# penn-graphics-research/DOT

Measured on AMD Instinct MI355X. Metric: ms_per_time_step, lower is better.
Workload: dtype f64; 1 GPU; bar17K_twist; nV=17315, nT=86058, energy=SNH, subdomains=32, script=twist, parallelism=32 subdomains on 1 GPU

## Files before the change

dot_amd/csrc/dotmi_api.hip:

```cpp
#include "dotmi_handle.hpp"

extern "C" {

int dotmi_set_state(dotmi_handle *h, const double *x, const double *v, const double *x_n)
{
    if (!h || !x || !v) return DOTMI_E_INVALID;
    HIPCHECK(h, hipSetDevice(h->device));
    if (resolve_refresh(h) == DOTMI_E_DEVICE) return DOTMI_E_DEVICE;
    const size_t bytes = sizeof(double) * h->n;
    HIPCHECK(h, hipMemcpyAsync(h->x, x, bytes, hipMemcpyHostToDevice, h->st));
    HIPCHECK(h, hipMemcpyAsync(h->v, v, bytes, hipMemcpyHostToDevice, h->st));
    HIPCHECK(h, hipMemcpyAsync(h->xn, x_n ? x_n : x, bytes, hipMemcpyHostToDevice, h->st));
    HIPCHECK(h, hipStreamSynchronize(h->st));
    std::vector<double> xt(h->n);
    const double *xn_h = x_n ? x_n : x;
    for (int i = 0; i < h->nV; ++i)
        for (int d = 0; d < 3; ++d) {
            const int k = 3 * i + d;
            xt[k] = h->fixed[i] ? xn_h[k] : xn_h[k] + (v[k] * h->dt + h->gdtsq[d]);
        }
    HIPCHECK(h, hipMemcpy(h->xt, xt.data(), bytes, hipMemcpyHostToDevice));
    return 0;
}

int dotmi_get_state(dotmi_handle *h, double *x, double *v, double *x_tilde)
{
    if (!h) return DOTMI_E_INVALID;
    HIPCHECK(h, hipSetDevice(h->device));
    if (resolve_refresh(h) == DOTMI_E_DEVICE) return DOTMI_E_DEVICE;
    const size_t bytes = sizeof(double) * h->n;
    HIPCHECK(h, hipStreamSynchronize(h->st));
    if (x) HIPCHECK(h, hipMemcpy(x, h->x, bytes, hipMemcpyDeviceToHost));
    if (v) HIPCHECK(h, hipMemcpy(v, h->v, bytes, hipMemcpyDeviceToHost));
    if (x_tilde) HIPCHECK(h, hipMemcpy(x_tilde, h->xt, bytes, hipMemcpyDeviceToHost));
    return 0;
}

int dotmi_set_dirichlet(dotmi_handle *h, int32_t n, const int32_t *idx, const double *pos)
{
    if (!h || n < 0 || (n > 0 && (!idx || !pos))) return DOTMI_E_INVALID;
    if (n == 0) return 0;
    HIPCHECK(h, hipSetDevice(h->device));
    for (int i = 0; i < n; ++i)
        if (idx[i] < 0 || idx[i] >= h->nV) {
            h->err = "dirichlet index out of range";
            return DOTMI_E_INVALID;
        }
    if ((size_t)n > h->dcap) {
        if (int rc = dalloc(h, &h->didx, (size_t)n)) return rc;
        if (int rc = dalloc(h, &h->dpos, (size_t)3 * n)) return rc;
        h->dcap = n;
    }
    if (h->didxHost.size() != (size_t)n || memcmp(h->didxHost.data(), idx, sizeof(int32_t) * n) != 0) {
        HIPCHECK(h, hipStreamSynchronize(h->st));
        h->didxHost.assign(idx, idx + n);
        if (h->dposPinned) hipHostFree(h->dposPinned);
        h->dposPinned = nullptr;
        HIPCHECK(h, hipHostMalloc((void **)&h->dposPinned, sizeof(double) * 3 * n));
        HIPCHECK(h, hipMemcpyAsync(h->didx, h->didxHost.data(), sizeof(int) * n, hipMemcpyHostToDevice, h->st));
    }
    if (!h->evDir) HIPCHECK(h, hipEventCreateWithFlags(&h->evDir, hipEventDisableTiming));
    else HIPCHECK(h, hipEventSynchronize(h->evDir));
    memcpy(h->dposPinned, pos, sizeof(double) * 3 * n);
    HIPCHECK(h, hipMemcpyAsync(h->dpos, h->dposPinned, sizeof(double) * 3 * n, hipMemcpyHostToDevice, h->st));
    HIPCHECK(h, hipEventRecord(h->evDir, h->st));
    launch_scatter_rows(n, h->didx, h->dpos, h->x, h->st);
    return 0;
}

int dotmi_refix(dotmi_handle *h, const uint8_t *fixed)
{
    if (!h || !fixed) return DOTMI_E_INVALID;
    HIPCHECK(h, hipSetDevice(h->device));
    if (resolve_refresh(h) == DOTMI_E_DEVICE) return DOTMI_E_DEVICE;
    h->fixed.assign(fixed, fixed + h->nV);
    HIPCHECK(h, hipMemcpy(h->M.fixed, fixed, h->nV, hipMemcpyHostToDevice));
    if (h->VP.orec) {
        refix_vpatch_records(h->vpRecGid, fixed, h->vpRec);
        HIPCHECK(h, hipMemcpy(const_cast<VpOwnRec *>(h->VP.orec), h->vpRec.data(), sizeof(VpOwnRec) * h->vpRec.size(), hipMemcpyHostToDevice));
    }
    if (h->pd) return pd_factor(h);
    return refactor(h, h->x, nullptr, nullptr);
}

int dotmi_operand_records(const dotmi_handle *h) { return h && h->vpFits ? (h->VP.orec ? 1 : 0) : -1; }

int dotmi_loop_forms(const dotmi_handle *h)
{
    if (!h) return DOTMI_E_INVALID;
    const long long nv = h->owner ? h->nHeld : h->nV;
    int forms = 0;
    if (h->devLoop) {
        if (gather_is_wide(3 * nv, h->tune.wideForms)) forms |= FORM_WIDE_GATHER;
        if (h->earlyBs && merge_early_is_wide(3 * nv, h->tune.wideForms)) forms |= FORM_WIDE_MERGE;
        if (h->earlyBs && (h->owner || h->tune.fuseDir) && spmv_zp_is_wide(nv, h->tune.wideForms)) forms |= FORM_WIDE_SPMV;
    }
    if (h->P.splitMerge) forms |= FORM_SPLIT_MERGE;
    if (h->P.tl.on && h->P.tl.nPanels > 0) forms |= twolevel_backward_code(h->P.tl.maxCols) << FORM_TWOLEVEL_CW_SHIFT;
    return forms;
}

double dotmi_target_gres(const dotmi_handle *h) { return h ? h->targetGRes : 0.0; }

int dotmi_last_iter_log(const dotmi_handle *h, int32_t cap, double *alpha, double *E, double *g2)
{
    if (!h) return DOTMI_E_INVALID;
    if (h->logPending > 0) {
        dotmi_handle *hm = const_cast<dotmi_handle *>(h);
        const int nlog = h->logPending;
        hm->logPending = 0;
        hm->log_alpha.resize(nlog);
        hm->log_E.resize(nlog);
        hm->log_g2.resize(nlog);
        if (hipSetDevice(h->device) != hipSuccess ||
            hipMemcpy(hm->log_alpha.data(), h->dlog, sizeof(double) * nlog, hipMemcpyDeviceToHost) != hipSuccess ||
            hipMemcpy(hm->log_E.data(), h->dlog + h->logCap, sizeof(double) * nlog, hipMemcpyDeviceToHost) != hipSuccess ||
            hipMemcpy(hm->log_g2.data(), h->dlog + 2 * (size_t)h->logCap, sizeof(double) * nlog, hipMemcpyDeviceToHost) !=
                hipSuccess)
            return DOTMI_E_DEVICE;
    }
    const int n = std::min<int>(cap, (int)h->log_alpha.size());
    for (int i = 0; i < n; ++i) {
        if (alpha) alpha[i] = h->log_alpha[i];
        if (E) E[i] = h->log_E[i];
        if (g2) g2[i] = h->log_g2[i];
    }
    return (int)h->log_alpha.size();
}

static int upload_tmp(dotmi_handle *h, const double *x, double *dst)
{
    HIPCHECK(h, hipMemcpyAsync(dst, x, sizeof(double) * h->n, hipMemcpyHostToDevice, h->st));
    return 0;
}

int dotmi_eval_energy(dotmi_handle *h, const double *x, double *E)
{
    if (!h || !x || !E) return DOTMI_E_INVALID;
    HIPCHECK(h, hipSetDevice(h->device));
    if (resolve_refresh(h) == DOTMI_E_DEVICE) return DOTMI_E_DEVICE;
    if (int rc = upload_tmp(h, x, h->x_trial)) return rc;
    const int nb = eval_all_elements(h, h->x_trial, 0);
    HIPCHECK(h, hipMemcpyAsync(h->h_partE, h->partE, sizeof(double) * 2 * nb, hipMemcpyDeviceToHost, h->st));
    HIPCHECK(h, hipStreamSynchronize(h->st));
    double se = 0, si = 0;
    for (int b = 0; b < nb; ++b) {
        se += h->h_partE[2 * b];
        si += h->h_partE[2 * b + 1];
    }
    *E = h->dtSq * se + si;
    return 0;
}

int dotmi_eval_gradient(dotmi_handle *h, const double *x, double *g)
{
    if (!h || !x || !g) return DOTMI_E_INVALID;
    HIPCHECK(h, hipSetDevice(h->device));
    if (resolve_refresh(h) == DOTMI_E_DEVICE) return DOTMI_E_DEVICE;
    if (int rc = upload_tmp(h, x, h->x_trial)) return rc;
    eval_all_elements(h, h->x_trial, 1);
    HIPCHECK(h, hipMemcpyAsync(g, h->g_trial, sizeof(double) * h->n, hipMemcpyDeviceToHost, h->st));
    HIPCHECK(h, hipStreamSynchronize(h->st));
    return 0;
}

int dotmi_eval_elem_hessians(dotmi_handle *h, const double *x, double *H)
{
    if (!h || !x || !H) return DOTMI_E_INVALID;
    HIPCHECK(h, hipSetDevice(h->device));
    if (resolve_refresh(h) == DOTMI_E_DEVICE) return DOTMI_E_DEVICE;
    if (int rc = upload_tmp(h, x, h->x_trial)) return rc;
    double *tmp = nullptr;
    HIPCHECK(h, hipMalloc((void **)&tmp, sizeof(double) * 144 * (size_t)h->nT));
    launch_elem_hessians(h->M, h->mat, h->dtSq, h->x_trial, tmp, h->st);
    hipError_t e = hipMemcpyAsync(H, tmp, sizeof(double) * 144 * (size_t)h->nT, hipMemcpyDeviceToHost, h->st);
    hipStreamSynchronize(h->st);
    hipFree(tmp);
    HIPCHECK(h, e);
    return 0;
}

int dotmi_refactor(dotmi_handle *h, const double *x)
{
    if (!h) return DOTMI_E_INVALID;
    if (h->pd) {
        h->err = "dotmi_refactor: an LBFGS-PD handle has no Hessian block solve";
        return DOTMI_E_INVALID;
    }
    HIPCHECK(h, hipSetDevice(h->device));
    if (resolve_refresh(h) == DOTMI_E_DEVICE) return DOTMI_E_DEVICE;
    const double *xd = h->x;
    if (x) {
        if (int rc = upload_tmp(h, x, h->x_trial)) return rc;
        xd = h->x_trial;
    }
    return refactor(h, xd, nullptr, nullptr);
}

int dotmi_apply_precond(dotmi_handle *h, const double *r, double *p)
{
    if (!h || !r || !p) return DOTMI_E_INVALID;
    HIPCHECK(h, hipSetDevice(h->device));
    if (int rc = enter_with_factors(h)) return rc;
    if (int rc = dot_coarse_refresh(h)) return rc;
    if (int rc = upload_tmp(h, r, h->q)) return rc;
    if (h->pd) {
        if (int rc = pd_apply(h, h->q, h->z, NO_HISTORY)) return rc;
    } else if (h->hi) {
        if (int rc = ic_apply(h, h->q, h->z, NO_HISTORY)) return rc;
    } else if (int rc = apply_precond(h, h->q, h->z, NO_HISTORY)) return rc;
    HIPCHECK(h, hipMemcpyAsync(p, h->z, sizeof(double) * h->n, hipMemcpyDeviceToHost, h->st));
    HIPCHECK(h, hipStreamSynchronize(h->st));
    return 0;
}

int dotmi_probe_direction(dotmi_handle *h, const double *x, int32_t m, const double *S, const double *Y, double *g_out,
                          double *q_out, double *z_out, double *p_out, double *alpha0, double *E_trial)
{
    if (!h || !x || m < 0 || m > h->hist || (m > 0 && (!S || !Y))) return DOTMI_E_INVALID;
    if (h->pd) {
        h->err = "dotmi_probe_direction: an LBFGS-PD handle has no Hessian block solve";
        return DOTMI_E_INVALID;
    }
    if (h->hi) {
        h->err = "dotmi_probe_direction: an LBFGS-HI handle has no Hessian block solve";
        return DOTMI_E_INVALID;
    }
    if (h->dist) {
        h->err = "dotmi_probe_direction: single-GPU handles only";
        return DOTMI_E_INVALID;
    }
    HIPCHECK(h, hipSetDevice(h->device));
    if (int rc = enter_with_factors(h)) return rc;
    if (int rc = dot_coarse_refresh(h)) return rc;
    const int n = h->n;
    const size_t bytes = sizeof(double) * n;
    HIPCHECK(h, hipMemcpyAsync(h->tmpn, x, bytes, hipMemcpyHostToDevice, h->st));
    for (int i = 0; i < m; ++i) {
// ... 169 lines not shown
    for (int i = 0; i < reps; ++i) one();
    HIPCHECK(h, hipEventRecord(h->ev1, h->st));
    HIPCHECK(h, hipEventSynchronize(h->ev1));
    float ms = 0;
    HIPCHECK(h, hipEventElapsedTime(&ms, h->ev0, h->ev1));
    if (ms_per_launch) *ms_per_launch = ms / reps;
    if (bytes_per_launch) *bytes_per_launch = h->precond_bytes;
    return 0;
}

int dotmi_bench_kernel(dotmi_handle *h, int32_t kind, int32_t reps, double *ms_per_launch, int64_t *bytes_per_launch)
{
    if (!h || reps < 1) return DOTMI_E_INVALID;
    if (h->pd) {
        h->err = "dotmi_bench_kernel: an LBFGS-PD handle has no Hessian block solve";
        return DOTMI_E_INVALID;
    }
    if (h->hi) {
        switch (kind) {
        case DOTMI_BENCH_BACKSOLVE:
        case DOTMI_BENCH_MERGE:
        case DOTMI_BENCH_BUILD_QPAD:
        case DOTMI_BENCH_SPMV_ZP:
        case DOTMI_BENCH_MERGE_EARLY:
        case DOTMI_BENCH_ELEM_STEP:
        case DOTMI_BENCH_GATHER_EARLY:
        case DOTMI_BENCH_DIRSTEP:
        case DOTMI_BENCH_ELEM_VERTEX:
            h->err = "dotmi_bench_kernel: an LBFGS-HI handle has no Hessian block solve";
            return DOTMI_E_INVALID;
        default:
            break;
        }
    }
    HIPCHECK(h, hipSetDevice(h->device));
    if (int rc = enter_with_factors(h)) return rc;
    const int n = h->n, nV = h->nV;
    const int64_t nTo = h->PT.nElem, nVo = h->v1 - h->v0, m = h->m > 0 ? h->m : h->hist;
    LbfgsArgs L = lbfgs_args(h);
    L.m = (int)std::min<int64_t>(m, h->hist);
    for (int i = 0; i < L.m; ++i) {
        L.s[i] = h->S[i];
        L.y[i] = h->Y[i];
        if (L.ys[i] == 0.0) L.ys[i] = 1.0;
    }
    int64_t bytes = 0;
    bool live = false;
    std::function<void()> run;
    StepElemPass e = step_elem_pass(h, h->x, 1, false);
    const StepArgs sa{h->p, h->partS, h->alpha_dev, h->alphaMin};
    GatherArgs a = gather_args(h);
    a.x = h->x;
    a.g_old = h->g;
    a.p = h->p;
    a.alpha_dev = h->alpha_dev;
    a.g_new = h->g_trial;
    a.s_new = h->S[h->hist];
    a.y_new = h->Y[h->hist];
    a.make_pair = 1;
    double xi[HIST_MAX] = {0, 0, 0, 0, 0, 0};
    switch (kind) {
    case DOTMI_BENCH_ELEM_ENERGY_GRAD:
        bytes = 112 * nTo + 56 * nVo;
        run = [&] { launch_elem_pass(e.M, h->PT, h->mat, h->dtSq, e.a, h->st); };
        break;
    case DOTMI_BENCH_ELEM_ENERGY:
        bytes = 112 * nTo + 56 * nVo;
        e.a.grad = 0;
        run = [&] { launch_elem_pass(e.M, h->PT, h->mat, h->dtSq, e.a, h->st); };
        break;
    case DOTMI_BENCH_VERTEX_GATHER:
        bytes = 80 * (int64_t)nV + (int64_t)(4 + 2 * L.m) * 8 * n;
        run = [&] { launch_vertex_gather(h->M, h->PT, a, L, h->partR, h->st); };
        break;
    case DOTMI_BENCH_SPMV_DOTS:
        bytes = 72 * (int64_t)h->M.nnzb + 2 * 8 * (int64_t)n;
        run = [&] { launch_spmv_dots(h->M, h->Hval, h->p, h->g, nullptr, h->v0, h->v1, h->partS, h->st); };
        break;
    case DOTMI_BENCH_BACKSOLVE:
        bytes = h->precond_bytes;
        run = [&] { launch_gemv(h->P, h->q, h->st); };
        break;
    case DOTMI_BENCH_MERGE:
        bytes = 8 * (int64_t)n * (2 + L.m) + 8 * (int64_t)h->mergeEntries;
        run = [&] {
            if (!h->P.mt_ptr) launch_reduce_partial(h->P, h->st);
            launch_merge(h->M, h->P, L, {.z = h->z, .partials = h->partC, .dots = true, .divide = true}, h->st);
        };
        break;
    case DOTMI_BENCH_BUILD_QPAD:
        bytes = 8 * (int64_t)n * (1 + L.m) + 8 * (int64_t)h->P.nParts * h->P.nmax;
        run = [&] { launch_build_qpad(h->P, h->g, L, xi, h->st); };
        break;
    case DOTMI_BENCH_BUILD_P:
        bytes = 8 * (int64_t)n * (2 + L.m);
        run = [&] { launch_build_p(n, h->z, L, h->partC, xi, h->p, h->st); };
        break;
    case DOTMI_BENCH_STEP_FORWARD:
        bytes = 8 * (int64_t)n * 3;
        run = [&] { launch_step_forward(n, step_forward_args(h, h->partS), h->st); };
        break;
    case DOTMI_BENCH_ELEM_HESSIAN:
        if (h->world > 1) return DOTMI_E_INVALID;
        bytes = (int64_t)(112 + 1152) * h->nHessElems;
        run = [&] {
            if (h->shardHess) launch_elem_hessians(h->M, h->mat, h->dtSq, h->x, h->He, h->st, h->hessElems, h->nHessElems);
            else launch_elem_hessians(h->M, h->mat, h->dtSq, h->x, h->He, h->st);
        };
        break;
    case DOTMI_BENCH_ASSEMBLE:
        if (h->world > 1) return DOTMI_E_INVALID;
        bytes = (int64_t)1152 * h->nHessElems + 72 * (int64_t)(h->shardHess ? h->nHessBlk : h->M.nnzb);
        run = [&] {
            if (h->shardHess) launch_assemble(h->M, h->He, h->Hval, h->st, h->hessBlk, h->nHessBlk, h->hessBlkPtr, h->hessBlkEnt);
            else launch_assemble(h->M, h->He, h->Hval, h->st);
        };
        break;
    case DOTMI_BENCH_SPMV_ZP:
        bytes = 72 * (int64_t)h->M.nnzb + 8 * (int64_t)n * (4 + 2 * L.m);
        live = true;
        run = [&] { launch_spmv_zp(h->M, spmv_zp_args(h, false), h->st, h->ctl); };
        break;
    case DOTMI_BENCH_MERGE_EARLY:
        bytes = 8 * (int64_t)h->mergeEntries + 8 * (int64_t)n * (4 + 2 * L.m);
        live = true;
        run = [&] {
            if (!h->P.mt_ptr) launch_reduce_partial(h->P, h->st, h->ctl);
            launch_merge_early(h->M, h->P, {.z = h->z, .partials = h->partC, .partialsT = h->dist ? nullptr : h->partCT, .wide = h->tune.wideForms}, h->st, h->ctl);
        };
        break;
    case DOTMI_BENCH_ELEM_STEP: {
        bytes = 112 * nTo + 56 * nVo + 48 * (int64_t)nV;
        live = true;
        e.a.x = h->x_trial;
        if (h->tune.fuseStep) e.a.step = &sa;
        run = [&] { launch_elem_pass(e.M, h->PT, h->mat, h->dtSq, e.a, h->st, h->ctl); };
        break;
    }
    case DOTMI_BENCH_GATHER_EARLY: {
        long long held = 0;
        for (int v = 0; v < nV; ++v) held += h->dup[v];
        bytes = 80 * (int64_t)nV + (int64_t)(6 + 2 * L.m) * 8 * n + 24 * held;
        live = true;
        a = early_gather_args(h);
        run = [&] { launch_vertex_gather(h->M, h->PT, a, L, h->partR, h->st, h->ctl); };
        break;
    }
    case DOTMI_BENCH_ELEM_VERTEX: {
        if (!h->vpFits) return DOTMI_E_INVALID;
        long long held = 0;
        for (int v = 0; v < nV; ++v) held += h->dup[v];
        bytes = 112 * nTo + 56 * nVo + 48 * (int64_t)nV + 80 * (int64_t)nV + (int64_t)(6 + 2 * L.m) * 8 * n + 24 * held;
        live = true;
        run = [&] {
            launch_elem_vertex(h->VP, h->mat, elem_vertex_args(h), h->st, h->ctl);
        };
        break;
    }
    case DOTMI_BENCH_DIRSTEP: {
        if (h->dist || !h->specFits) return DOTMI_E_INVALID;
        bytes = 72 * (int64_t)h->M.nnzb + 8 * (int64_t)n * (4 + 2 * L.m) + 112 * nTo + 56 * nVo + 24 * (int64_t)nV;
        live = true;
        e.a.x = h->x_trial;
        e.a.step = &sa;
        run = [&] { launch_dirstep(e.M, h->PTspec, h->mat, h->dtSq, spmv_zp_args(h, false), e.a, h->st, h->ctl); };
        break;
    }
    default:
        return DOTMI_E_INVALID;
    }
    DevLoop saved;
    if (live) {
        if (!h->earlyBs || h->prevSlots < 0 || !h->P.vp_ptr) {
            h->err = "the in-loop kernel forms need a handle that has run a step of the device loop's early order";
            return DOTMI_E_INVALID;
        }
        HIPCHECK(h, hipMemcpy(&saved, h->ctl, sizeof(DevLoop), hipMemcpyDeviceToHost));
        DevLoop live_ctl = saved;
        live_ctl.status = 0;
        live_ctl.phase = 0;
        HIPCHECK(h, hipMemcpy(h->ctl, &live_ctl, sizeof(DevLoop), hipMemcpyHostToDevice));
    }
    run();
    HIPCHECK(h, hipEventRecord(h->ev0, h->st));
    for (int i = 0; i < reps; ++i) run();
    HIPCHECK(h, hipEventRecord(h->ev1, h->st));
    HIPCHECK(h, hipEventSynchronize(h->ev1));
    HIPCHECK(h, hipGetLastError());
    if (live) HIPCHECK(h, hipMemcpy(h->ctl, &saved, sizeof(DevLoop), hipMemcpyHostToDevice));
    float ms = 0;
    HIPCHECK(h, hipEventElapsedTime(&ms, h->ev0, h->ev1));
    if (kind == DOTMI_BENCH_ELEM_HESSIAN || kind == DOTMI_BENCH_ASSEMBLE) {
        if (int rc = refactor(h, h->x, nullptr, nullptr)) return rc;
    }
    if (ms_per_launch) *ms_per_launch = ms / reps;
    if (bytes_per_launch) *bytes_per_launch = bytes;
    return 0;
}

int dotmi_bench_energy(dotmi_handle *h, int32_t reps, double *ms_per_launch, int64_t *bytes_per_launch)
{
    if (!h || reps < 1) return DOTMI_E_INVALID;
    HIPCHECK(h, hipSetDevice(h->device));
    if (resolve_refresh(h) == DOTMI_E_DEVICE) return DOTMI_E_DEVICE;
    const StepElemPass e = step_elem_pass(h, h->x, 0, false);
    launch_elem_pass(e.M, h->PT, h->mat, h->dtSq, e.a, h->st);
    HIPCHECK(h, hipEventRecord(h->ev0, h->st));
    for (int i = 0; i < reps; ++i) launch_elem_pass(e.M, h->PT, h->mat, h->dtSq, e.a, h->st);
    HIPCHECK(h, hipEventRecord(h->ev1, h->st));
    HIPCHECK(h, hipEventSynchronize(h->ev1));
    float ms = 0;
    HIPCHECK(h, hipEventElapsedTime(&ms, h->ev0, h->ev1));
    if (ms_per_launch) *ms_per_launch = ms / reps;
    if (bytes_per_launch) *bytes_per_launch = (int64_t)112 * h->nOwnElem + (int64_t)56 * (h->v1 - h->v0);
    return 0;
}

int dotmi_comm_unique_id(void *out128)
{
    ncclUniqueId id;
    if (ncclGetUniqueId(&id) != ncclSuccess) return DOTMI_E_DEVICE;
    static_assert(sizeof(ncclUniqueId) == 128, "ncclUniqueId size");
    memcpy(out128, &id, 128);
    return 0;
}

int32_t dotmi_factor_kind(const dotmi_handle *h)
{
    if (!h) return DOTMI_E_INVALID;
    return h->tileFlow ? 2 : h->tileSplit ? 3 : 1;
}

int32_t dotmi_factor_groups(const dotmi_handle *h)
{
    if (!h) return DOTMI_E_INVALID;
    return h->tgroupLevel.size() > 2 ? (int32_t)h->tgroupLevel.size() - 1 : 1;
}

int32_t dotmi_backsolve_form(const dotmi_handle *h)
{
    if (!h) return DOTMI_E_INVALID;
    return h->twoLevel ? 1 : 0;
}

int32_t dotmi_comm_ranks(const dotmi_handle *h)
{
    if (!h) return DOTMI_E_INVALID;
    if (h->comm) {
        int n = 0;
        if (ncclCommCount(h->comm, &n) != ncclSuccess) return DOTMI_E_DEVICE;
        return n;
    }
    return h->arCb ? -h->world : 1;
}

}
```

dot_amd/csrc/dotmi_create.hip:

```cpp
#include "dotmi_handle.hpp"
#include "block_plan.hpp"

namespace dotmi {
std::string g_create_error;
}

namespace dotmi {

void host_features(dotmi_handle *h)
{
    const int nV = h->nV, nT = h->nT;
    h->A.assign((size_t)9 * nT, 0.0);
    h->vol.assign(nT, 0.0);
    h->mass.assign(nV, 0.0);
    for (int e = 0; e < nT; ++e) {
        const int *t = &h->T[4 * e];
        const double *p0 = &h->Xrest[3 * t[0]], *p1 = &h->Xrest[3 * t[1]], *p2 = &h->Xrest[3 * t[2]],
                     *p3 = &h->Xrest[3 * t[3]];
        Mat3 X0;
        for (int i = 0; i < 3; ++i) {
            X0.m[i][0] = p1[i] - p0[i];
            X0.m[i][1] = p2[i] - p0[i];
            X0.m[i][2] = p3[i] - p0[i];
        }
        const double d = det3(X0), id = 1.0 / d;
        const double(*m)[3] = X0.m;
        double *R = &h->A[(size_t)9 * e];
        R[0] = (m[1][1] * m[2][2] - m[1][2] * m[2][1]) * id;
        R[1] = (m[0][2] * m[2][1] - m[0][1] * m[2][2]) * id;
        R[2] = (m[0][1] * m[1][2] - m[0][2] * m[1][1]) * id;
        R[3] = (m[1][2] * m[2][0] - m[1][0] * m[2][2]) * id;
        R[4] = (m[0][0] * m[2][2] - m[0][2] * m[2][0]) * id;
        R[5] = (m[0][2] * m[1][0] - m[0][0] * m[1][2]) * id;
        R[6] = (m[1][0] * m[2][1] - m[1][1] * m[2][0]) * id;
        R[7] = (m[0][1] * m[2][0] - m[0][0] * m[2][1]) * id;
        R[8] = (m[0][0] * m[1][1] - m[0][1] * m[1][0]) * id;
        h->vol[e] = d / 3.0 / 2.0;
        double a[3], b[3], c[3];
        for (int i = 0; i < 3; ++i) {
            a[i] = p0[i] - p3[i];
            b[i] = p1[i] - p3[i];
            c[i] = p2[i] - p3[i];
        }
        const double vv = std::fabs(a[0] * (b[1] * c[2] - b[2] * c[1]) + a[1] * (b[2] * c[0] - b[0] * c[2]) +
                                    a[2] * (b[0] * c[1] - b[1] * c[0])) / 6.0;
        for (int k = 0; k < 4; ++k) h->mass[t[k]] += vv / 4.0;
    }
    for (int v = 0; v < nV; ++v) h->mass[v] *= h->density;
}

double host_target_gres(const dotmi_handle *h)
{
    Mat3 Aw;
    double Bw[3][4];
    const double S1[3] = {1, 1, 1};
#define TG_BLOCKS(MATV) spectral_blocks<MATV>(S1, h->mu[0], h->lam[0], 1.0, false, Aw, Bw)
    DM_DISPATCH_MAT(h->mat, TG_BLOCKS)
#undef TG_BLOCKS
    double sqH = 0;
    for (int i = 0; i < 3; ++i)
        for (int j = 0; j < 3; ++j) sqH += Aw.m[i][j] * Aw.m[i][j];
    for (int c = 0; c < 3; ++c)
        for (int k = 0; k < 4; ++k) sqH += Bw[c][k] * Bw[c][k];
    std::vector<double> ls(h->nV, 0.0);
    for (int e = 0; e < h->nT; ++e) {
        const int *t = &h->T[4 * e];
        for (int i = 0; i < 4; ++i) {
            const double *a = &h->Xrest[3 * t[(i + 1) % 4]], *b = &h->Xrest[3 * t[(i + 2) % 4]],
                         *c = &h->Xrest[3 * t[(i + 3) % 4]];
            const double u[3] = {b[0] - a[0], b[1] - a[1], b[2] - a[2]};
            const double w[3] = {c[0] - a[0], c[1] - a[1], c[2] - a[2]};
            const double cx = u[1] * w[2] - u[2] * w[1], cy = u[2] * w[0] - u[0] * w[2],
                         cz = u[0] * w[1] - u[1] * w[0];
            ls[t[i]] += 0.5 * std::sqrt(cx * cx + cy * cy + cz * cz);
        }
    }
    double sql = 0;
    for (int v = 0; v < h->nV; ++v) sql += ls[v] * ls[v];
    const double cn = h->relTol * h->relTol * sqH * sql * (double)(h->nV - 1) / (double)h->nV;
    return cn * h->dtSq * h->dtSq;
}

int upload_vpatches(dotmi_handle *h, const HostVPatches &H, DevVPatches &D, dotmi_handle::SlotMap &SM)
{
    D.nPatches = H.nPatches;
    D.PE = H.PE;
    D.PV = H.PV;
    D.PO = H.PO;
    D.RUN = H.RUN;
    const size_t ns = (size_t)H.nPatches * H.PE;
    std::vector<ushort4> tl(ns), ep(ns);
    std::vector<double> A(9 * ns, 0.0), mu(ns, 1.0), lam(ns, 1.0), vol(ns, 0.0), volE(ns, 0.0);
    D.nSlotsUsed = 0;
    for (size_t s = 0; s < ns; ++s) {
        tl[s] = make_ushort4(H.tl[4 * s], H.tl[4 * s + 1], H.tl[4 * s + 2], H.tl[4 * s + 3]);
        ep[s] = make_ushort4(H.epos[4 * s], H.epos[4 * s + 1], H.epos[4 * s + 2], H.epos[4 * s + 3]);
        const int e = H.elem[s];
        if (e < 0) continue;
        D.nSlotsUsed++;
        for (int k = 0; k < 9; ++k) A[(size_t)k * ns + s] = h->A[(size_t)9 * e + k];
        mu[s] = h->mu[e];
        lam[s] = h->lam[e];
        vol[s] = h->vol[e];
        volE[s] = H.eown[s] ? h->vol[e] : 0.0;
    }
    if (int rc = upload(h, &D.tl, tl)) return rc;
    if (int rc = upload(h, &D.epos, ep)) return rc;
    if (int rc = upload(h, &D.A, A)) return rc;
    bool uniform = !h->mu.empty();
    for (size_t e = 1; e < h->mu.size() && uniform; ++e) uniform = h->mu[e] == h->mu[0] && h->lam[e] == h->lam[0];
    D.mu = D.lam = nullptr;
    if (uniform) {
        D.mu0 = h->mu[0];
        D.lam0 = h->lam[0];
    } else {
        if (int rc = upload(h, &D.mu, mu)) return rc;
        if (int rc = upload(h, &D.lam, lam)) return rc;
    }
    if (int rc = upload(h, &SM.elem, H.elem)) return rc;
    SM.nSlots = ns;
    SM.mu = D.mu;
    SM.lam = D.lam;
    if (int rc = upload(h, &D.vol, vol)) return rc;
    if (int rc = upload(h, &D.volE, volE)) return rc;
    if (int rc = upload(h, &D.pv_gid, H.pv_gid)) return rc;
    if (int rc = upload(h, &D.pv_cnt, H.pv_cnt)) return rc;
    if (int rc = upload(h, &D.po_cnt, H.po_cnt)) return rc;
    if (int rc = upload(h, &D.c_ptr, H.c_ptr)) return rc;
    return 0;
}

int upload_patches(dotmi_handle *h, const HostPatches &H, DevPatches &D, dotmi_handle::SlotMap &SM)
{
    D.nPatches = H.nPatches;
    D.PE = H.PE;
    D.PV = H.PV;
    D.nSlots = H.nSlots;
    const size_t ns = (size_t)H.nPatches * H.PE;
    std::vector<ushort4> tl(ns);
    std::vector<double> A(9 * ns, 0.0), mu(ns, 1.0), lam(ns, 1.0), vol(ns, 0.0);
    D.nElem = 0;
    for (size_t s = 0; s < ns; ++s) {
        tl[s] = make_ushort4(H.tl[4 * s], H.tl[4 * s + 1], H.tl[4 * s + 2], H.tl[4 * s + 3]);
        const int e = H.elem[s];
        if (e < 0) continue;
        D.nElem++;
        for (int k = 0; k < 9; ++k) A[(size_t)k * ns + s] = h->A[(size_t)9 * e + k];
        mu[s] = h->mu[e];
        lam[s] = h->lam[e];
        vol[s] = h->vol[e];
    }
    if (int rc = upload(h, &D.tl, tl)) return rc;
    if (int rc = upload(h, &D.A, A)) return rc;
    bool uniform = !h->mu.empty();
    for (size_t e = 1; e < h->mu.size() && uniform; ++e) uniform = h->mu[e] == h->mu[0] && h->lam[e] == h->lam[0];
    D.mu = D.lam = nullptr;
    if (uniform) {
        D.mu0 = h->mu[0];
        D.lam0 = h->lam[0];
    } else {
        if (int rc = upload(h, &D.mu, mu)) return rc;
        if (int rc = upload(h, &D.lam, lam)) return rc;
    }
    if (int rc = upload(h, &SM.elem, H.elem)) return rc;
    SM.nSlots = ns;
    SM.mu = D.mu;
    SM.lam = D.lam;
    if (int rc = upload(h, &D.vol, vol)) return rc;
    if (int rc = upload(h, &D.pv_gid, H.pv_gid)) return rc;
    if (int rc = upload(h, &D.pv_slot, H.pv_slot)) return rc;
    if (int rc = upload(h, &D.pv_cnt, H.pv_cnt)) return rc;
    if (int rc = upload(h, &D.c_ptr, H.c_ptr)) return rc;
    {
        std::vector<ushort4> ep(ns);
        for (size_t s2 = 0; s2 < ns; ++s2) ep[s2] = make_ushort4(H.epos[4 * s2], H.epos[4 * s2 + 1], H.epos[4 * s2 + 2], H.epos[4 * s2 + 3]);
        if (int rc = upload(h, &D.epos, ep)) return rc;
    }
    {
        std::vector<int2> rng(H.pp_rng.size() / 2);
        for (size_t v = 0; v < rng.size(); ++v) rng[v] = make_int2(H.pp_rng[2 * v], H.pp_rng[2 * v + 1]);
        if (int rc = upload(h, &D.pp_rng, rng)) return rc;
    }
    if (int rc = dalloc(h, &D.gpart, (size_t)3 * std::max(H.nSlots, 1))) return rc;
    HIPCHECK(h, hipMemset(D.gpart, 0, sizeof(double) * 3 * (size_t)std::max(H.nSlots, 1)));
    return 0;
}

static int build_element_side(dotmi_handle *h, const std::vector<int> &adj_ptr, const std::vector<int> &blk_ptr,
                              const std::vector<int> &blk_ent)
{
    const int nV = h->nV, nT = h->nT;
    if (h->shardElems) {
        std::vector<int> el;
        for (int e = 0; e < nT; ++e)
            if (h->epart[e] >= h->p0 && h->epart[e] < h->p1) el.push_back(e);
        h->nOwnElem = (int)el.size();
        if (int rc = upload(h, &h->elist, el)) return rc;
        h->v0 = (int)((long long)nV * h->rank / h->world);
        h->v1 = (int)((long long)nV * (h->rank + 1) / h->world);
    } else {
        h->elist = nullptr;
        h->nOwnElem = nT;
        h->v0 = 0;
        h->v1 = nV;
    }
    h->shardHess = h->shardElems && (h->owner || (h->tune.shardHess >= 0 ? h->tune.shardHess != 0 : true));
    h->nHessElems = nT;
    if (h->shardHess) {
        std::vector<uint8_t> needV(nV, 0);
        for (int pI = h->p0; pI < h->p1; ++pI)
            for (int v : h->partVerts[pI]) needV[v] = 1;
        if (!h->owner)
            for (int v = h->v0; v < h->v1; ++v) needV[v] = 1;
        std::vector<int> el, e2c(nT, -1);
        for (int e = 0; e < nT; ++e)
            if (needV[h->T[4 * e]] || needV[h->T[4 * e + 1]] || needV[h->T[4 * e + 2]] || needV[h->T[4 * e + 3]]) {
                e2c[e] = (int)el.size();
                el.push_back(e);
            }
        std::vector<int> bl, bptr(1, 0), bent, optr(1, 0), oent;
        for (int v = 0; v < nV; ++v) {
            if (!needV[v]) continue;
            for (int k = adj_ptr[v]; k < adj_ptr[v + 1]; ++k) {
                bl.push_back(k);
                for (int i = blk_ptr[k]; i < blk_ptr[k + 1]; ++i) {
                    const int e = blk_ent[i] >> 4;
                    bent.push_back((e2c[e] << 4) | (blk_ent[i] & 15));
                    if (h->owner && h->epart[e] >= h->p0 && h->epart[e] < h->p1) oent.push_back(bent.back());
                }
                bptr.push_back((int)bent.size());
                optr.push_back((int)oent.size());
            }
        }
        if (h->owner) {
            if (oent.empty()) oent.push_back(-1);
            if (int rc = upload(h, &h->ownBlkPtr, optr)) return rc;
            if (int rc = upload(h, &h->ownBlkEnt, oent)) return rc;
        }
        h->nHessElems = (int)el.size();
        h->nHessBlk = (int)bl.size();
        if (int rc = upload(h, &h->hessElems, el)) return rc;
        if (int rc = upload(h, &h->hessBlk, bl)) return rc;
        if (int rc = upload(h, &h->hessBlkPtr, bptr)) return rc;
        if (int rc = upload(h, &h->hessBlkEnt, bent)) return rc;
    }
    {
        int PE = h->tune.patchElems > 0 ? (h->tune.patchElems <= 256 ? 256 : 512) : 256;
        std::vector<int> all(nT);
        for (int e = 0; e < nT; ++e) all[e] = e;
        if (int rc = upload_patches(h, build_patches(nV, h->T.data(), h->Xrest.data(), all, PE), h->PTall, h->smAll)) return rc;
        if (h->shardElems) {
            std::vector<int> own;
            for (int e = 0; e < nT; ++e)
                if (h->epart[e] >= h->p0 && h->epart[e] < h->p1) own.push_back(e);
            if (int rc = upload_patches(h, build_patches(nV, h->T.data(), h->Xrest.data(), own, PE), h->PT, h->smOwn)) return rc;
        } else {
            h->PT = h->PTall;
        }
        h->specFits = false;
        if (!h->dist && h->world == 1 && h->tune.specStep != 0) {
            const int nbv = (nV + 255) / 256, room = 512 - NB_RED - nbv;
            if (std::max(h->PT.nPatches, nbv) <= room) {
                h->PTspec = h->PT;
                h->specFits = true;
            } else if (h->tune.patchElems == 0 && PE == 256) {
                const HostPatches H2 = build_patches(nV, h->T.data(), h->Xrest.data(), all, 512);
                if (std::max(H2.nPatches, nbv) <= room) {
                    if (int rc = upload_patches(h, H2, h->PTspec, h->smSpec)) return rc;
                    h->specFits = true;
                }
            }
        }
    }
    if (h->owner) {
        std::vector<int> holders(nV, 0), last(nV, -1), ownerR(nV, -1);
        for (int r = 0; r < h->world; ++r)
            for (int pI = h->firstPart[r]; pI < h->firstPart[r + 1]; ++pI)
// ... 472 lines not shown
{
    h->nV = mesh->nV;
    h->nT = mesh->nT;
    h->n = 3 * mesh->nV;
    h->mat = prm->energy;
    h->hist = prm->history;
    h->iterCap = prm->iterCap > 0 ? prm->iterCap : 10000;
    h->dt = prm->dt;
    h->dtSq = prm->dt * prm->dt;
    for (int d = 0; d < 3; ++d) {
        h->grav[d] = prm->gravity[d];
        h->gdtsq[d] = h->dtSq * prm->gravity[d];
    }
    h->relTol = prm->relTol;
    h->alphaMin = prm->alphaMin;
    h->device = prm->device;
    h->rank = prm->rank;
    h->world = prm->world;
    h->flags = prm->flags;
    h->tune = Tuning::from_env();
#ifdef DOTMI_TEST_HOOKS
    h->testIterDelta = Tuning::geti("DOTMI_TEST_ITER_DELTA", 0);
    h->testFailRefresh = Tuning::geti("DOTMI_TEST_FAIL_REFRESH", 0);
#endif
    h->density = mesh->density;
    h->nPartsAll = mesh->nParts;
    h->T.assign(mesh->T, mesh->T + 4 * (size_t)h->nT);
    h->pd = (h->flags & DOTMI_FLAG_LBFGS_PD) != 0;
    h->hi = (h->flags & DOTMI_FLAG_LBFGS_HI) != 0;
    h->newtonPcg = (h->flags & DOTMI_FLAG_NEWTON_PCG) != 0;
    if (h->newtonPcg) {
        const int bad = DOTMI_FLAG_FORCE_DIST | DOTMI_FLAG_OWNER_EXCHANGE | DOTMI_FLAG_GSDD | DOTMI_FLAG_NEWTON | DOTMI_FLAG_LBFGS_PD |
                        DOTMI_FLAG_LBFGS_HI | DOTMI_FLAG_ASYNC_REFRESH;
        if (prm->world > 1 || (h->flags & bad) || mesh->vpart) {
            h->err = "DOTMI_FLAG_NEWTON_PCG: single GPU, host loop, not with DOTMI_FLAG_FORCE_DIST / OWNER_EXCHANGE / GSDD / NEWTON / "
                     "LBFGS_PD / LBFGS_HI / ASYNC_REFRESH or a vertex partition";
            return DOTMI_E_INVALID;
        }
    }
    if (h->flags & DOTMI_FLAG_NEWTON_PCG_DIST) {
        const char *why = (h->flags & DOTMI_FLAG_OWNER_EXCHANGE) ? "not with DOTMI_FLAG_OWNER_EXCHANGE (the vectors of the recurrences are replicated)"
                          : (h->flags & DOTMI_FLAG_GSDD)         ? "not with DOTMI_FLAG_GSDD (a GSDD handle solves one subdomain at a time)"
                          : (h->flags & DOTMI_FLAG_NEWTON)       ? "not with DOTMI_FLAG_NEWTON (a Newton handle factorises H as one subdomain)"
                          : (h->flags & DOTMI_FLAG_LBFGS_PD)     ? "not with DOTMI_FLAG_LBFGS_PD (no Hessian block solve)"
                          : (h->flags & DOTMI_FLAG_LBFGS_HI)     ? "not with DOTMI_FLAG_LBFGS_HI (no Hessian block solve)"
                          : (h->flags & DOTMI_FLAG_ASYNC_REFRESH)
                              ? "not with DOTMI_FLAG_ASYNC_REFRESH (a Newton iteration factorises at its own iterate)"
                          : (h->flags & DOTMI_FLAG_DOT_COARSE) ? "not with DOTMI_FLAG_DOT_COARSE (the sharded PCG has no coarse space)"
                          : mesh->vpart                        ? "not with a vertex partition (vpart): it is single-GPU only"
                                                               : nullptr;
        if (why) {
            h->err = std::string("DOTMI_FLAG_NEWTON_PCG_DIST: ") + why;
            return DOTMI_E_INVALID;
        }
        h->newtonPcg = true;
    }
    if (h->hi) {
        const int bad = DOTMI_FLAG_FORCE_DIST | DOTMI_FLAG_OWNER_EXCHANGE | DOTMI_FLAG_GSDD | DOTMI_FLAG_NEWTON | DOTMI_FLAG_LBFGS_PD |
                        DOTMI_FLAG_ASYNC_REFRESH;
        if (prm->world > 1 || (h->flags & bad) || mesh->vpart) {
            h->err = "DOTMI_FLAG_LBFGS_HI: single GPU, host loop, not with DOTMI_FLAG_FORCE_DIST / OWNER_EXCHANGE / GSDD / NEWTON / "
                     "LBFGS_PD / ASYNC_REFRESH or a vertex partition";
            return DOTMI_E_INVALID;
        }
        h->nPartsAll = 1;
        h->epart.assign(h->nT, 0);
    } else if (h->pd) {
        const int bad = DOTMI_FLAG_FORCE_DIST | DOTMI_FLAG_OWNER_EXCHANGE | DOTMI_FLAG_GSDD | DOTMI_FLAG_NEWTON | DOTMI_FLAG_ASYNC_REFRESH;
        if (prm->world > 1 || (h->flags & bad) || mesh->vpart) {
            h->err = "DOTMI_FLAG_LBFGS_PD: single GPU, host loop, not with DOTMI_FLAG_FORCE_DIST / OWNER_EXCHANGE / GSDD / NEWTON / "
                     "ASYNC_REFRESH or a vertex partition";
            return DOTMI_E_INVALID;
        }
        h->nPartsAll = 1;
        h->epart.assign(h->nT, 0);
    } else if (mesh->vpart) {
        if (prm->world > 1 || (prm->flags & DOTMI_FLAG_FORCE_DIST)) {
            h->err = "a vertex partition (vpart) is single-GPU only";
            return DOTMI_E_INVALID;
        }
        for (int v = 0; v < mesh->nV; ++v)
            if (mesh->vpart[v] < 0 || mesh->vpart[v] >= mesh->nParts) {
                h->err = "vpart out of range";
                return DOTMI_E_INVALID;
            }
        h->vpart.assign(mesh->vpart, mesh->vpart + h->nV);
        h->epart.assign(h->nT, 0);
    } else if (mesh->epart) {
        h->epart.assign(mesh->epart, mesh->epart + h->nT);
    } else {
        h->epart.resize(h->nT);
        partition_elements(mesh->nV, mesh->nT, mesh->T, mesh->X_rest, mesh->nParts, h->epart.data());
    }
    if (h->flags & DOTMI_FLAG_DOT_COARSE) {
        const char *why = (h->flags & DOTMI_FLAG_OWNER_EXCHANGE)
                              ? "not with DOTMI_FLAG_OWNER_EXCHANGE (its merge in front of the exchange forms z before the coarse solution y exists)"
                          : (h->flags & DOTMI_FLAG_GSDD)       ? "not with DOTMI_FLAG_GSDD (a GSDD handle solves one subdomain at a time)"
                          : (h->flags & DOTMI_FLAG_NEWTON_PCG) ? "not with DOTMI_FLAG_NEWTON_PCG (its coarse term is dotmi_set_pcg_coarse)"
                          : (h->flags & DOTMI_FLAG_NEWTON)     ? "not with DOTMI_FLAG_NEWTON (a Newton handle factorises H as one subdomain)"
                          : (h->flags & DOTMI_FLAG_LBFGS_PD)   ? "not with DOTMI_FLAG_LBFGS_PD (no Hessian block solve)"
                          : (h->flags & DOTMI_FLAG_LBFGS_HI)   ? "not with DOTMI_FLAG_LBFGS_HI (no Hessian block solve)"
                          : (h->flags & DOTMI_FLAG_ASYNC_REFRESH)
                              ? "not with DOTMI_FLAG_ASYNC_REFRESH (the build is judged with the refresh)"
                          : mesh->vpart ? "not with a vertex partition (vpart): the coarse plan works on an element partition"
                                        : nullptr;
        if (why) {
            h->err = std::string("DOTMI_FLAG_DOT_COARSE: ") + why;
            return DOTMI_E_INVALID;
        }
        if (h->nPartsAll > COARSE_MAX_PARTS) {
            h->err = "DOTMI_FLAG_DOT_COARSE: at most " + std::to_string(COARSE_MAX_PARTS) + " subdomains (the coarse matrix is applied "
                     "through a dense inverse factor); " + std::to_string(h->nPartsAll) + " were asked for";
            return DOTMI_E_INVALID;
        }
        h->coarse.dotMode = 1;
    }
    h->fixed.assign(mesh->fixed, mesh->fixed + h->nV);
    h->Xrest.assign(mesh->X_rest, mesh->X_rest + h->n);
    h->mu.assign(mesh->mu, mesh->mu + h->nT);
    h->lam.assign(mesh->lambda, mesh->lambda + h->nT);
    return 0;
}

static int choose_loop_form(dotmi_handle *h)
{
    h->gsdd = (h->flags & DOTMI_FLAG_GSDD) != 0;
    h->newton = (h->flags & (DOTMI_FLAG_NEWTON | DOTMI_FLAG_NEWTON_PCG | DOTMI_FLAG_NEWTON_PCG_DIST)) != 0;
    if (h->newton && ((h->dist && !(h->flags & DOTMI_FLAG_NEWTON_PCG_DIST)) || h->gsdd)) {
        h->err = "DOTMI_FLAG_NEWTON: single GPU, not together with DOTMI_FLAG_GSDD";
        return DOTMI_E_INVALID;
    }
    if (h->gsdd && h->dist) {
        h->err = "DOTMI_FLAG_GSDD: single GPU only";
        return DOTMI_E_INVALID;
    }
    h->devLoop = !h->gsdd && !h->newton && !h->pd && !h->hi && !(h->flags & (DOTMI_FLAG_HOST_LOOP | DOTMI_FLAG_TIME_PHASES));
    h->earlyBs = h->devLoop && h->tune.earlyBs != 0 &&
                 (h->P.mt_ptr != nullptr || h->P.splitMerge);
    if (h->owner && !(h->earlyBs && h->tune.fuseDir)) {
        h->err = "DOTMI_FLAG_OWNER_EXCHANGE needs the device loop's early order with the fused direction kernel";
        return DOTMI_E_INVALID;
    }
    if (h->earlyBs && h->tune.fuseStep && (!h->shardElems || h->owner)) h->PT.wgCap = h->PTspec.wgCap = 512;
    h->vpFits = false;
    const bool closedForm = h->mat == DOTMI_ENERGY_SNH || h->mat == DOTMI_ENERGY_SNH_LOG;
    if (h->earlyBs && !h->dist && h->world == 1 && h->tune.fuseStep && h->tune.fuseDir && h->tune.vertexPatches != 0 &&
        (closedForm || h->tune.vertexPatches > 0) &&
        h->P.ntiles - h->P.ntilesWide + h->P.nquad > 0 && !(h->flags & (DOTMI_FLAG_GSDD | DOTMI_FLAG_NEWTON | DOTMI_FLAG_NEWTON_PCG | DOTMI_FLAG_NEWTON_PCG_DIST | DOTMI_FLAG_HOST_LOOP))) {
        const HostVPatches HV = build_vpatches(h->nV, h->nT, h->T.data(), h->Xrest.data(), 512, 85);
        const bool rec = h->tune.operandRecords != 0 && HV.nPatches > 0 &&
                         elem_vertex_dyn_lds(HV.PV, HV.RUN, HV.PO, true) + ELEM_VERTEX_STATIC_LDS <= 64 * 1024;
        const size_t shm = HV.nPatches > 0 ? elem_vertex_dyn_lds(HV.PV, HV.RUN, HV.PO, rec) + ELEM_VERTEX_STATIC_LDS : 0;
        if (HV.nPatches > 0 && HV.nPatches <= 512 && HV.nPatches <= ELEM_NB_MAX && shm <= 64 * 1024 && HV.PO + 1 <= 256) {
            if (int rc = upload_vpatches(h, HV, h->VP, h->smVP)) return rc;
            if (rec) {
                std::vector<int> vpp((size_t)h->nV + 1), vpo;
                HIPCHECK(h, hipMemcpy(vpp.data(), h->P.vp_ptr, sizeof(int) * vpp.size(), hipMemcpyDeviceToHost));
                vpo.resize((size_t)std::max(vpp[h->nV], 1));
                HIPCHECK(h, hipMemcpy(vpo.data(), h->P.vp_off, sizeof(int) * (size_t)vpp[h->nV], hipMemcpyDeviceToHost));
                h->vpRec = build_vpatch_records(HV, h->mass.data(), h->fixed.data(), vpp.data(), vpo.data());
                h->vpRecGid = vpatch_own_gid(HV);
                VpOwnRec *d = nullptr;
                if (int rc = upload(h, &d, h->vpRec)) return rc;
                h->VP.orec = d;
            }
            h->vpFits = true;
            if (h->tune.fuseLog)
                fprintf(stderr, "dotmi: vertex patches: %d patches, %.2f x the elements, up to %d owned / %d touched vertices, runs %d, %zu B LDS, operand records %s\n",
                        HV.nPatches, (double)h->VP.nSlotsUsed / std::max(1, h->nT), HV.PO, HV.PV, HV.RUN, shm, rec ? "on" : "off");
        }
    }
    return 0;
}

static int alloc_loop_state(dotmi_handle *h)
{
    if (h->dist) {
        const size_t nz = (size_t)h->n + dot_coarse_tail(h);
        if (int rc = dalloc(h, &h->zstage, nz)) return rc;
        HIPCHECK(h, hipMemsetAsync(h->zstage, 0, sizeof(double) * nz, h->st));
    }
    if (h->vpFits && h->VP.orec) {
        const size_t nrec = (size_t)2 * (HIST_MAX + 1) * h->n;
        if (int rc = dalloc(h, &h->hrec, nrec)) return rc;
        HIPCHECK(h, hipMemsetAsync(h->hrec, 0, sizeof(double) * nrec, h->st));
    }
    if (h->earlyBs) {
        if (int rc = dalloc(h, &h->u_old, (size_t)h->n)) return rc;
        for (int sl = 0; sl <= h->hist; ++sl) {
            if (int rc = dalloc(h, &h->MY[sl], (size_t)h->n)) return rc;
            if (int rc = dalloc(h, &h->HS[sl], (size_t)h->n)) return rc;
        }
    }
    h->logCap = std::min(h->iterCap, 10001) + 1;
    h->kindCap = 4096;
    HIPCHECK(h, hipHostMalloc((void **)&h->h_ctl, sizeof(DevLoop)));
    HIPCHECK(h, hipHostMalloc((void **)&h->h_flags, sizeof(int) * 4));
    HIPCHECK(h, hipMalloc((void **)&h->ctl, sizeof(DevLoop)));
    h->allocs.push_back(h->ctl);
    if (int rc = dalloc(h, &h->dlog, (size_t)3 * h->logCap)) return rc;
    HIPCHECK(h, hipMalloc((void **)&h->dkind, sizeof(int) * h->kindCap));
    h->allocs.push_back(h->dkind);
    return 0;
}

static int create_impl(dotmi_handle *h, const dotmi_mesh *mesh, const dotmi_params *prm, const double *x_init)
{
    int ndev = 0;
    if (hipGetDeviceCount(&ndev) != hipSuccess || ndev <= 0) {
        h->err = "no HIP device available: libdotmi has no CPU fallback";
        return DOTMI_E_NOGPU;
    }
    if (!mesh || !prm || !x_init || mesh->nV <= 0 || mesh->nT <= 0 || !mesh->X_rest || !mesh->T || !mesh->mu ||
        !mesh->lambda || !mesh->fixed || mesh->nParts < 1 || prm->dt <= 0 ||
        prm->history < 1 || prm->history > HIST_MAX || prm->world < 1 || prm->rank < 0 ||
        prm->rank >= prm->world || (prm->world > 1 && !prm->comm_id && !prm->allreduce) ||
        (prm->energy != DOTMI_ENERGY_FCR && prm->energy != DOTMI_ENERGY_SNH && prm->energy != DOTMI_ENERGY_SNH_LOG)) {
        h->err = "invalid argument";
        return DOTMI_E_INVALID;
    }
    for (int e = 0; e < mesh->nT; ++e) {
        if (mesh->epart && !mesh->vpart && (mesh->epart[e] < 0 || mesh->epart[e] >= mesh->nParts)) {
            h->err = "epart out of range";
            return DOTMI_E_INVALID;
        }
        for (int k = 0; k < 4; ++k)
            if (mesh->T[4 * e + k] < 0 || mesh->T[4 * e + k] >= mesh->nV) {
                h->err = "tet index out of range";
                return DOTMI_E_INVALID;
            }
    }
    if (int rc = take_arguments(h, mesh, prm)) return rc;

    HIPCHECK(h, hipSetDevice(h->device));
    HIPCHECK(h, hipStreamCreate(&h->st));
    HIPCHECK(h, hipEventCreate(&h->ev0));
    HIPCHECK(h, hipEventCreate(&h->ev1));
    HIPCHECK(h, hipEventCreate(&h->ev2));
    HIPCHECK(h, hipEventCreate(&h->evA));
    h->timePhases = (h->flags & DOTMI_FLAG_TIME_PHASES) != 0;
    if (h->timePhases)
        for (auto &e : h->evP) HIPCHECK(h, hipEventCreate(&e));
    h->dist = h->world > 1 || (h->flags & DOTMI_FLAG_FORCE_DIST);
    h->shardElems = h->dist && (h->tune.shardElems >= 0 ? h->tune.shardElems != 0 : h->nT >= 400000);
    h->owner = h->dist && (h->flags & DOTMI_FLAG_OWNER_EXCHANGE);
    if (h->owner) {
        if (h->flags & (DOTMI_FLAG_HOST_LOOP | DOTMI_FLAG_TIME_PHASES | DOTMI_FLAG_GSDD | DOTMI_FLAG_NEWTON)) {
            h->err = "DOTMI_FLAG_OWNER_EXCHANGE: device loop only";
            return DOTMI_E_INVALID;
        }
        h->shardElems = true;
    }
    h->arCb = prm->allreduce;
    h->arCtx = prm->allreduce_ctx;
    if (h->dist && !h->arCb) {
        ncclUniqueId id;
        if (h->world > 1) memcpy(&id, prm->comm_id, 128);
        else NCCLCHECK(h, ncclGetUniqueId(&id));
        NCCLCHECK(h, ncclCommInitRank(&h->comm, h->world, id, h->rank));
    }
    {
        void *cd = nullptr;
        HIPCHECK(h, hipMalloc(&cd, sizeof(double) * (RED_K + 8)));
        h->allocs.push_back(cd);
        h->ctrlDev = (double *)cd;
    }

    h->timeStride = h->tune.timeStride;
    if (h->flags & DOTMI_FLAG_TIME_BACKSOLVE) {
        h->evPre.resize(2 * 512);
        for (auto &e : h->evPre) HIPCHECK(h, hipEventCreate(&e));
        if (h->dist) {
            h->evAr.resize(2 * 512);
            for (auto &e : h->evAr) HIPCHECK(h, hipEventCreate(&e));
        }
    }
    host_features(h);
    h->targetGRes = host_target_gres(h);
    if (int rc = build_device_mesh(h)) return rc;
    if (!h->pd && !h->hi)
        if (int rc = pcg_build_scaling(h)) return rc;
    const int n = h->n;
    double **vecs[] = {&h->x, &h->x_trial, &h->xn, &h->v, &h->xt, &h->g, &h->g_trial, &h->p, &h->q, &h->z,
                       &h->Hp, &h->tmpn};
    const size_t nvec = (size_t)n + 8 + dot_coarse_tail(h);
    for (double **pp : vecs) {
        if (int rc = dalloc(h, pp, nvec)) return rc;
        HIPCHECK(h, hipMemsetAsync(*pp, 0, sizeof(double) * nvec, h->st));
    }
    for (int s = 0; s <= h->hist; ++s) {
        if (int rc = dalloc(h, &h->S[s], (size_t)n)) return rc;
        if (int rc = dalloc(h, &h->Y[s], (size_t)n)) return rc;
    }
    if (int rc = dalloc(h, &h->He, (size_t)144 * std::max(h->nHessElems, 1))) return rc;
    if (int rc = dalloc(h, &h->Hval, hval_size(h->M.nnzb))) return rc;
    if (h->owner) {
        if (int rc = dalloc(h, &h->HvalOwn, hval_size(h->M.nnzb))) return rc;
        HIPCHECK(h, hipMemsetAsync(h->HvalOwn, 0, sizeof(double) * hval_size(h->M.nnzb), h->st));
    }
    if (int rc = dalloc(h, &h->partE, (size_t)4 * ELEM_NB_MAX)) return rc;
    double **parts[] = {&h->partR, &h->partC, &h->partS, &h->partG, &h->partGR, &h->partGC, &h->partCT, &h->partST};
    for (double **pp : parts) {
        const size_t rows = pp == &h->partR ? 512 : NB_RED;
        if (int rc = dalloc(h, pp, rows * RED_K)) return rc;
        HIPCHECK(h, hipMemsetAsync(*pp, 0, sizeof(double) * rows * RED_K, h->st));
    }
    if (int rc = dalloc(h, &h->alpha_dev, 8)) return rc;
    if (int rc = dalloc(h, &h->gstage, (size_t)n + 2)) return rc;
    HIPCHECK(h, hipMemsetAsync(h->gstage, 0, sizeof(double) * ((size_t)n + 2), h->st));
    HIPCHECK(h, hipHostMalloc((void **)&h->h_partE, sizeof(double) * 2 * ELEM_NB_MAX));
    HIPCHECK(h, hipHostMalloc((void **)&h->h_partR, sizeof(double) * NB_RED * RED_K));
    HIPCHECK(h, hipHostMalloc((void **)&h->h_alpha, sizeof(double) * 8));
    if (int rc = choose_loop_form(h)) return rc;
    if (int rc = alloc_loop_state(h)) return rc;

    HIPCHECK(h, hipMemcpyAsync(h->x, x_init, sizeof(double) * n, hipMemcpyHostToDevice, h->st));
    HIPCHECK(h, hipMemcpyAsync(h->xn, h->x, sizeof(double) * n, hipMemcpyDeviceToDevice, h->st));
    launch_be_update(h->nV, h->M.fixed, h->x, h->xn, h->v, h->xt, h->dt, h->gdtsq, h->st);
    HIPCHECK(h, hipStreamSynchronize(h->st));
    if (h->pd) return pd_factor(h);
    return refactor(h, h->x, nullptr, nullptr);
}

int dotmi_create(const dotmi_mesh *mesh, const dotmi_params *prm, const double *x_init, dotmi_handle **out)
{
    if (!out) return DOTMI_E_INVALID;
    *out = nullptr;
    dotmi_handle *h = new dotmi_handle();
    int rc = create_impl(h, mesh, prm, x_init);
    if (rc != 0) {
        g_create_error = h->err;
        dotmi_destroy(h);
        return rc;
    }
    *out = h;
    return 0;
}

// ... 2 lines not shown
```

dot_amd/csrc/dotmi_devloop.hip:

```cpp
#include "dotmi_handle.hpp"

namespace dotmi {

struct Slot {
    int nb = 0;
    const double *spart = nullptr;
    const double *ctlE = nullptr;
};

static int slot_direction(dotmi_handle *h, Slot &s)
{
    if (h->specNow) {
        const StepArgs sa{h->p, h->partS, h->alpha_dev, h->alphaMin};
        StepElemPass e = step_elem_pass(h, h->x_trial, 1);
        e.a.step = &sa;
        s.nb = launch_dirstep(e.M, h->PTspec, h->mat, h->dtSq, spmv_zp_args(h), e.a, h->st, h->ctl);
    } else if (h->owner || h->tune.fuseDir) {
        launch_spmv_zp(h->M, spmv_zp_args(h), h->st, h->ctl);
    } else {
        launch_build_p(h->n, h->z, NO_HISTORY, h->partC, nullptr, h->p, h->st, h->ctl);
        launch_spmv_dots(h->M, h->Hval, h->p, h->g, nullptr, h->v0, h->v1, h->partS, h->st, h->ctl);
    }
    return reduce_step_dots(h, &s.spart);
}
// ... 27 lines not shown
    const GatherArgs a = early_gather_args(h);
    s.ctlE = h->partE;
    if (h->vpNow) {
    } else if (!h->shardElems) {
        launch_vertex_gather(h->M, h->stepPT(), a, NO_HISTORY, h->partR, h->st, h->ctl);
    } else if (h->owner) {
        GatherArgs ag = a;
        ag.ownMask = h->ownMask;
        ag.vlist = h->heldList;
        ag.nlist = h->nHeld;
        ag.kind = h->vkind;
        ag.pre = 1;
        ag.gshare = h->gstage;
        launch_vertex_gather(h->M, h->PT, ag, NO_HISTORY, h->partR, h->st, h->ctl);
        if (int rc = exchange_gradient_packed(h, n, s.nb, h->partR, RED_K)) return rc;
        ag.vlist = h->sharedList;
        ag.nlist = h->nShared;
        ag.pre = 0;
        if (h->nShared > 0) launch_pair_stats(n, ag, NO_HISTORY, nullptr, h->st, h->gstage, h->ctl);
        s.ctlE = h->gstage + n;
        s.nb = 1;
    } else {
        if (int rc = gradient_over_ranks(h, s.nb, a)) return rc;
        s.ctlE = h->gstage + n;
        s.nb = 1;
    }
    return 0;
}

static void slot_coarse(dotmi_handle *h)
{
    if (!dot_coarse(h)) return;
    if (h->dist) dot_coarse_restrict(h, h->zstage + h->n, h->ctl, 1);
    else dot_coarse_restrict_solve(h, h->ctl, 1);
}

static void slot_backsolve(dotmi_handle *h, const Slot &s)
{
    const double *ctlR = h->owner ? h->partGR : h->partR;
    const Bracket br = backsolve_bracket(h);
    h->slotTimed.push_back(br.at);
    CtlLaunch ca{{h->ctl, s.ctlE, ctlR, h->alpha_dev, h->h_flags, s.nb, h->pairNow ? 2 : 0}, h->ctlForm};
    launch_gemv(h->P, nullptr, h->st, h->ctl, br.ev0, br.ev1, &ca, (int)h->slotTimed.size() );
}

static int slot_merge(dotmi_handle *h)
{
    if (!h->dist) {
        launch_merge_early(h->M, h->P, {.z = h->z, .partials = h->partC, .partialsT = h->partCT, .co = dot_coarse(h), .wide = h->tune.wideForms}, h->st, h->ctl);
    } else if (!h->owner) {
        return merge_over_ranks(h, NO_HISTORY, h->zstage, RANKSUM_EARLY, h->ctl, h->held());
    } else {
        launch_merge_early(h->M, h->P, {.z = h->z, .partials = h->partC, .ownMask = h->ownMask, .vl = h->held(), .kind = h->vkind, .pre = 1,
                                        .zshare = h->zstage, .wide = h->tune.wideForms}, h->st, h->ctl);
        if (int rc = exchange_solve_packed(h)) return rc;
        if (h->nShared > 0)
            launch_merge_early(h->M, h->P, {.z = h->z, .zsum = h->zstage, .ownMask = h->ownMask, .vl = h->shared(), .wide = h->tune.wideForms}, h->st, h->ctl);
    }
    return 0;
}

static int enqueue_loop_slot_early(dotmi_handle *h)
{
    Slot s;
    if (int rc = slot_direction(h, s)) return rc;
    slot_trial(h, s);
    if (int rc = slot_gradient(h, s)) return rc;
    slot_coarse(h);
    slot_backsolve(h, s);
    return slot_merge(h);
}

static int enqueue_loop_slot(dotmi_handle *h)
{
    if (h->earlyNow) return enqueue_loop_slot_early(h);
    const int n = h->n;
    const CoarseMerge *bal = dot_coarse_balanced(h);
    const double *r1 = nullptr;
    if (bal) {
        launch_build_q(n, h->g, NO_HISTORY, nullptr, h->q, h->st, h->ctl);
        r1 = dot_coarse_deflate(h, h->q, h->ctl);
    } else {
        launch_build_qpad(h->P, h->g, NO_HISTORY, nullptr, h->st, h->ctl);
    }
    const CoarseMerge *co = dot_coarse(h);
    if (co && h->dist) dot_coarse_restrict(h, h->z + n, h->ctl, 0);
    else if (co) dot_coarse_restrict_solve(h, h->ctl, 0);
    const Bracket br = backsolve_bracket(h);
    h->slotTimed.push_back(br.at);
    launch_gemv(h->P, r1, h->st, h->ctl, br.ev0, br.ev1);
    if (bal) {
        launch_merge(h->M, h->P, NO_HISTORY, {.z = h->z}, h->st, h->ctl);
        dot_coarse_balance(h, h->z, NO_HISTORY, h->ctl);
    } else if (!h->dist) {
        launch_merge(h->M, h->P, NO_HISTORY, {.z = h->z, .partials = h->partC, .dots = true, .divide = true, .co = co}, h->st, h->ctl);
    } else {
        if (int rc = merge_over_ranks(h, NO_HISTORY, h->z, RANKSUM_ZFINISH, h->ctl)) return rc;
    }
    launch_build_p(n, h->z, NO_HISTORY, h->partC, nullptr, h->p, h->st, h->ctl);
    launch_spmv_dots(h->M, h->Hval, h->p, h->g, nullptr, h->v0, h->v1, h->partS, h->st, h->ctl);
    const double *spart = nullptr;
    if (int rc = reduce_step_dots(h, &spart)) return rc;
    launch_step_forward(n, step_forward_args(h, spart), h->st, h->ctl);
    const StepElemPass e = step_elem_pass(h, h->x_trial, 1);
    const int nb = launch_elem_pass(e.M, h->PT, h->mat, h->dtSq, e.a, h->st, h->ctl);
    GatherArgs a = gather_args(h);
    a.p = h->p;
    a.alpha_dev = h->alpha_dev;
    a.make_pair = 1;
    if (!h->shardElems) {
        launch_vertex_gather(h->M, h->PT, a, NO_HISTORY, h->partR, h->st, h->ctl);
        launch_loop_control(h->ctl, h->partE, nb, h->partR, h->alpha_dev, h->h_flags, h->st);
        return 0;
    }
    if (int rc = gradient_over_ranks(h, nb, a)) return rc;
    launch_loop_control(h->ctl, h->gstage + n, 1, h->partR, h->alpha_dev, h->h_flags, h->st);
    return 0;
}

static void choose_step_forms(dotmi_handle *h)
{
    h->earlyNow = h->earlyBs && !dot_coarse_balanced(h);
    h->pairNow = h->earlyNow && !h->dist && h->tune.fuseStep && h->tune.fuseDir && h->tune.earlyHold &&
                 (h->tune.pairTrials > 0 || (h->tune.pairTrials < 0 && h->prevIters > 0 && 4 * h->prevHalv >= h->prevIters));
    h->specNow = h->earlyNow && !h->dist && !h->pairNow && h->tune.fuseStep && h->tune.fuseDir &&
                 h->specFits && h->coarse.dotMode == 0 &&
                 (h->tune.specStep > 0 || (h->tune.specStep < 0 && h->prevFirst > 0 && 10 * h->prevUnit >= 9 * h->prevFirst));
    h->vpNow = h->vpFits && h->earlyNow && !h->dist && !h->specNow && !(h->pairNow && h->tune.vertexPatches < 0);
    h->ctlForm = h->pairNow ? (h->vpNow ? CTL_PAIR_VP : CTL_PAIR) : h->specNow ? CTL_SPEC : h->vpNow ? CTL_VP : CTL_PLAIN;
}

static int init_devloop(dotmi_handle *h, int *notifyFrom)
{
    DevLoop &C = *h->h_ctl;
    memset(&C, 0, sizeof(C));
    C.specPartials = h->partS;
    C.alphaMin = h->alphaMin;
    C.iterCap = h->iterCap;
    C.hist = h->hist;
    C.tol = h->targetGRes;
    C.dtSq = h->dtSq;
    C.x_cur = h->x;
    C.x_trial = h->x_trial;
    C.g_cur = h->g;
    C.g_trial = h->g_trial;
    for (int s = 0; s <= h->hist; ++s) {
        C.S[s] = h->S[s];
        C.Y[s] = h->Y[s];
        C.MY[s] = h->MY[s];
        C.HS[s] = h->HS[s];
    }
    C.u_old = h->u_old;
    C.hrec = h->hrec;
    devloop_resolve(C);
    C.holdEnable = h->tune.earlyHold ? 1 : 0;
    memcpy(C.predHist, h->predState, sizeof(int) * 2);
    memcpy(&C.predCtr[0][0], h->predState + 2, sizeof(int) * 8);
    memcpy(C.pairCtr, h->pairState, sizeof(int) * 3);
    C.log_alpha = h->dlog;
    C.log_E = h->dlog + h->logCap;
    C.log_g2 = h->dlog + 2 * (size_t)h->logCap;
    C.slot_kind = h->dkind;
    C.logCap = h->logCap;
    C.kindCap = h->kindCap;
    volatile int *flags = h->h_flags;
    flags[0] = 0;
    flags[1] = 0;
    C.notifyFrom = std::max(0, std::min(h->prevSlots - 3, h->prevSlots * 3 / 4));
    if (h->dist) C.notifyFrom = 1 << 30;
    *notifyFrom = C.notifyFrom;
    HIPCHECK(h, hipMemcpyAsync(h->ctl, h->h_ctl, sizeof(DevLoop), hipMemcpyHostToDevice, h->st));
    return 0;
}

static int step_start_sharded(dotmi_handle *h, int nb)
{
    const int n = h->n;
    const double *ctlR = h->partR;
    if (!h->owner) {
        stage_energy(h, nb, h->gstage + n + 1);
        if (int rc = allreduce_sum(h, h->gstage, (size_t)n + 2)) return rc;
    } else {
        launch_masked_norm2(n, h->gstage, h->vkind, h->partR, h->st, 1);
        if (int rc = exchange_gradient_packed(h, n, nb, h->partR, 1)) return rc;
        ctlR = h->partGR;
    }
    HIPCHECK(h, hipMemcpyAsync(h->g, h->gstage, sizeof(double) * n, hipMemcpyDeviceToDevice, h->st));
    if (!h->owner) {
        const double *vecs[1] = {h->g};
        launch_multidot(n, h->g, vecs, 1, h->partR, h->st);
    }
    if (!h->earlyNow) {
        launch_loop_control(h->ctl, h->gstage + n, 1, ctlR, h->alpha_dev, h->h_flags, h->st, 1);
        return 0;
    }
    launch_build_qpad(h->P, h->g, NO_HISTORY, nullptr, h->st, nullptr);
    const CoarseMerge *co = dot_coarse(h);
    if (co) dot_coarse_restrict(h, h->zstage + n);
    CtlLaunch ca{{h->ctl, h->gstage + n, ctlR, h->alpha_dev, h->h_flags, 1, 1}, CTL_PLAIN};
    launch_gemv(h->P, nullptr, h->st, h->ctl, nullptr, nullptr, &ca, 1 << 30);
    if (!h->owner) return merge_over_ranks(h, NO_HISTORY, h->zstage, RANKSUM_EARLY_FIRST, h->ctl, h->held());
    launch_merge(h->M, h->P, NO_HISTORY, {.z = h->zstage, .vl = h->held()}, h->st, h->ctl);
    if (int rc = exchange_iface(h, h->zstage, nullptr, 0)) return rc;
    launch_merge_early(h->M, h->P, {.z = h->z, .first = 1, .zsum = h->zstage, .ownMask = h->ownMask, .vl = h->held(), .wide = h->tune.wideForms}, h->st, h->ctl);
    HIPCHECK(h, hipMemsetAsync(h->partGC, 0, sizeof(double) * HIST_MAX, h->st));
    return 0;
}

static int enqueue_step_start(dotmi_handle *h)
{
    int nb = h->VP.nPatches;
    if (h->vpNow) {
        ElemVertArgs ea = elem_vertex_args(h);
        ea.x0 = h->x;
        ea.g0 = h->g;
        launch_elem_vertex(h->VP, h->mat, ea, h->st, nullptr);
    } else {
        const StepElemPass e = step_elem_pass(h, h->x, 1);
        nb = launch_elem_pass(e.M, h->stepPT(), h->mat, h->dtSq, e.a, h->st);
    }
    GatherArgs a = gather_args(h);
    a.x = h->x;
    a.g_new = h->shardElems ? h->gstage : h->g;
    a.make_pair = 0;
    a.ownMask = h->owner ? h->ownMask : nullptr;
    a.vlist = h->owner ? h->heldList : nullptr;
    a.nlist = h->owner ? h->nHeld : 0;
    if (h->owner) HIPCHECK(h, hipMemcpyAsync(h->x_trial, h->x, sizeof(double) * h->n, hipMemcpyDeviceToDevice, h->st));
    if (h->earlyNow && !h->shardElems) {
        a.vp_ptr = h->P.vp_ptr;
        a.vp_off = h->P.vp_off;
        a.rpad = h->P.rpad;
    }
    if (!h->vpNow) launch_vertex_gather(h->M, h->stepPT(), a, NO_HISTORY, h->partR, h->st);
    if (h->shardElems) return step_start_sharded(h, nb);
    if (!h->earlyNow) {
        launch_loop_control(h->ctl, h->partE, nb, h->partR, h->alpha_dev, h->h_flags, h->st, 1);
        return 0;
    }
    const CoarseMerge *co = dot_coarse(h);
    if (co && h->dist) dot_coarse_restrict(h, h->zstage + h->n);
    else if (co) dot_coarse_restrict_solve(h);
    CtlLaunch ca{{h->ctl, h->partE, h->partR, h->alpha_dev, h->h_flags, nb, 1}, h->vpNow ? CTL_VP : CTL_PLAIN};
    launch_gemv(h->P, nullptr, h->st, h->ctl, nullptr, nullptr, &ca, 1 << 30);
    if (h->dist) return merge_over_ranks(h, NO_HISTORY, h->zstage, RANKSUM_EARLY_FIRST, h->ctl);
    launch_merge_early(h->M, h->P, {.z = h->z, .partials = h->partC, .partialsT = h->partCT, .first = 1, .co = co, .wide = h->tune.wideForms}, h->st, h->ctl);
    return 0;
}

static int follow_progress(dotmi_handle *h, int notifyFrom, int *enq)
{
    const int AHEAD = 2;
    volatile int *flags = h->h_flags;
    const double tStart = now_ms();
    long spins = 0;
    while (flags[0] == 0) {
        if (*enq < std::max(notifyFrom, (int)flags[1]) + AHEAD) {
            if (int rc = enqueue_loop_slot(h)) return rc;
            ++*enq;
        } else if ((++spins & 0xfffff) == 0) {
            if (hipStreamQuery(h->st) != hipErrorNotReady && flags[0] == 0) {
                HIPCHECK(h, hipStreamSynchronize(h->st));
                HIPCHECK(h, hipGetLastError());
                if (flags[0] == 0 && *enq >= std::max(notifyFrom, (int)flags[1]) + AHEAD) {
                    h->err = "device loop made no progress";
                    return DOTMI_E_DEVICE;
                }
            }
            if (now_ms() - tStart > 600000.0) {
                h->err = "device loop timed out";
                return DOTMI_E_DEVICE;
            }
        }
    }
    return 0;
}

static int enqueue_batches(dotmi_handle *h, int *enq)
{
    const DevLoop &C = *h->h_ctl;
    const double tStart = now_ms();
    int target = std::max(h->prevSlots + 1, 4);
    for (;;) {
        while (*enq < target) {
            if (int rc = enqueue_loop_slot(h)) return rc;
            ++*enq;
        }
        HIPCHECK(h, hipMemcpyAsync(h->h_ctl, h->ctl, sizeof(DevLoop), hipMemcpyDeviceToHost, h->st));
        HIPCHECK(h, hipStreamSynchronize(h->st));
        HIPCHECK(h, hipGetLastError());
        double mine[4] = {(double)C.status, (double)C.slots, (double)C.iter, (double)C.halvings}, red[9];
#ifdef DOTMI_TEST_HOOKS
        mine[2] += (double)h->testIterDelta;
#endif
        for (int i = 0; i < 4; ++i) {
            red[i] = mine[i];
            red[4 + i] = mine[i] * mine[i];
        }
        red[8] = 0.0;
        if (h->world > 1) {
            HIPCHECK(h, hipMemcpyAsync(h->ctrlDev, red, sizeof(red), hipMemcpyHostToDevice, h->st));
            if (int rc = allreduce_sum(h, h->ctrlDev, 9)) return rc;
            HIPCHECK(h, hipMemcpyAsync(red, h->ctrlDev, sizeof(red), hipMemcpyDeviceToHost, h->st));
            HIPCHECK(h, hipStreamSynchronize(h->st));
        }
        const double w = h->world > 1 ? (double)h->world : 1.0;
// ... 75 lines not shown
```

dot_amd/csrc/dotmi_internal.hpp:

```cpp
#pragma once
#include <hip/hip_runtime.h>

#include "bs_forms.hpp"
#include "lbfgs_history.hpp"
#include "merge_sum.hpp"
#include "nd_layout.hpp"
#include "tile_factor.hpp"
#include <stdint.h>
#include <stdio.h>
#include <stdlib.h>

namespace dotmi {

inline int elem_wg_cap(int mat) { return mat == 1 ? 768 : 512; }
#define DM_DISPATCH_MAT(mat, CASE)              \
    switch (mat) {                              \
    case 0: CASE(0); break;                     \
    case 1: CASE(1); break;                     \
    case 2: CASE(2); break;                     \
    default: ::dotmi::unknown_material(mat);    \
    }
[[noreturn]] inline void unknown_material(int mat)
{
    fprintf(stderr, "dotmi: no kernel for material id %d\n", mat);
    abort();
}
constexpr int NB_RED = 256;
constexpr int RED_K = 3 * HIST_MAX + 3;
constexpr int BS_WAVE = bs_family_capacity(BSF_PACK);
constexpr int BS_NARROW = bs_family_capacity(BSF_NARROW);
constexpr int BS_LONG = bs_family_capacity(BSF_WIDE);
constexpr int ELEM_NB_MAX = 8192;
constexpr int CHOL_NB = 64;

__host__ __device__ inline size_t hval_idx(int blk, int e) { return (size_t)(blk >> 3) * 72 + (size_t)(8 * e + (blk & 7)); }
inline size_t hval_size(int nnzb) { return (size_t)72 * (((size_t)nnzb + 7) / 8); }

struct DevMesh {
    int nV, nT, nTp;
    int4 *T;
    double *A;
    double *mu, *lam, *vol;
    double *mass;
    uint8_t *fixed;
    int *adj_ptr, *adj_idx;
    int nnzb;
    int *blk_ptr, *blk_ent;
    int *blk_row;
};

struct DevPatches {
    int nPatches = 0, PE = 0, PV = 0, nSlots = 0, nElem = 0;
    int wgCap = 0;
    ushort4 *tl = nullptr;
    double *A = nullptr;
    double *mu = nullptr, *lam = nullptr, *vol = nullptr;
    double mu0 = 0.0, lam0 = 0.0;
    int *pv_gid = nullptr, *pv_slot = nullptr, *pv_cnt = nullptr;
    unsigned short *c_ptr = nullptr;
    ushort4 *epos = nullptr;
    int2 *pp_rng = nullptr;
    double *gpart = nullptr;
};

struct VpOwnRec;
struct DevVPatches {
    int nPatches = 0, PE = 0, PV = 0, PO = 0, RUN = 0, nSlotsUsed = 0;
    ushort4 *tl = nullptr, *epos = nullptr;
    double *A = nullptr;
    double *vol = nullptr, *volE = nullptr;
    double *mu = nullptr, *lam = nullptr;
    double mu0 = 0.0, lam0 = 0.0;
    int *pv_gid = nullptr, *pv_cnt = nullptr, *po_cnt = nullptr;
    unsigned short *c_ptr = nullptr;
    const VpOwnRec *orec = nullptr;
};
inline size_t elem_vertex_dyn_lds(int PV, int RUN, int PO, bool rec)
{
    return sizeof(double) * ((size_t)3 * PV + (size_t)3 * RUN + (rec ? (size_t)6 * PO : 0)) + 2 * (size_t)((PO + 1 + 3) & ~3);
}
constexpr size_t ELEM_VERTEX_STATIC_LDS = sizeof(double) * (4 * RED_K + 8 + 1);
struct ElemVertArgs {
    const double *mass, *xt, *p, *hp;
    const double *spmv_partials;
    const uint8_t *fixed;
    const int *vp_ptr, *vp_off;
    double *rpad;
    double *partE, *partR, *alpha_out;
    double dtSq, alpha_min;
    const double *x0;
    double *g0;
};

struct RowTile {
    long long off;
    int ld, c0;
};

struct DevTwoLevel {
    int on;
    int nPanels;
    int maxRows, maxCols;
    int nItems;
    const int2 *item;
    const int4 *panel;
    const long long *rowSrc;
    const long long *rowBase;
    double *packed;
    const int *rowPos;
    double *cbuf;
    const int *gPtr, *gIdx;
    double *rpad2;
};

struct DevParts {
    DevTwoLevel tl;
    int nParts;
    int nmax;
    int *dofmap;
    double *W;
    RowTile *rt;
    int ntiles;
    int4 *tile;
    int nquad;
    int ntilesWide;
    int maxTileLen;
    int nltiles, nlwork;
    int4 *ltile;
    int2 *lwork;
    int maxChunks;
    double *tdots;
    int4 *tileByPart;
    int4 *ltileByPart;
    int2 *lworkByPart;
    int nbmax;
    int2 *trange;
    int *rp_ptr, *rp_idx;
    double *ppart;
    double *psub;
    double *rpad;
    int *vp_ptr, *vp_off;
    int *mt_ptr, *mt_ent;
    int2 *mt_wave;
    int *mt_il;
    int splitMerge;
    int *dup;
    int nfill;
    long long *fill_dst;
    int *fill_src;
    int npad;
    long long *pad_dst;
};

constexpr int PD_KC = 8;
struct PdItem {
    int blk;
    int cs, ce;
    int nch, first;
    long long pbase;
};
struct DevPD {
    int nmax = 0;
    int *cvert = nullptr;
    double *W = nullptr;
    RowTile *rt = nullptr;
    double *Lval = nullptr;
    int *inc_ptr = nullptr, *inc = nullptr;
    long long *fill_dst = nullptr;
    long long *pad_dst = nullptr;
    int npad = 0;
    PdItem *items = nullptr;
    int nOne = 0, nLong = 0;
    double *ppart = nullptr, *tdots = nullptr;
    int *mptr = nullptr;
    long long *ment = nullptr;
};

struct DevIC {
    int nV = 0, nL = 0;
    int *vert = nullptr;
    int *lptr = nullptr, *lidx = nullptr;
    int *lsrc = nullptr, *dsrc = nullptr;
    int *pptr = nullptr, *pa = nullptr, *pb = nullptr;
    int *uptr = nullptr, *ublk = nullptr, *uvert = nullptr;
    double *F = nullptr;
    double *yw = nullptr;
    int *flag = nullptr;
};

struct CoarseMerge;
struct LbfgsArgs {
    int m;
    const double *s[HIST_MAX];
    const double *y[HIST_MAX];
    double ys[HIST_MAX];
    double sy[HIST_MAX][HIST_MAX];
};

constexpr int SUM_CHUNKS = 16;
template <class Get>
__host__ __device__ inline double chunked_sum(int n, Get get)
{
    const int L = (n + SUM_CHUNKS - 1) / SUM_CHUNKS;
    double tot = 0.0;
    for (int c = 0; c < SUM_CHUNKS; ++c) {
        double acc = 0.0;
        const int e = (c + 1) * L < n ? (c + 1) * L : n;
        for (int k = c * L; k < e; ++k) acc += get(k);
        tot += acc;
    }
    return tot;
}

__host__ __device__ inline int pair_band(double a0) { return a0 < 0.7 ? 0 : (a0 < 0.9 ? 1 : 2); }

struct XiArgs {
    double xi[HIST_MAX];
};

struct DevLoop {
    int status;
    int phase;
    int iter, iterCap, hist, halvings, evals, slots;
    int notifyFrom;
    int pad0;
    double tol, dtSq;
    double alpha;
    double E_cur, g2_cur;
    double E0, g2_0;
    double *x_cur, *x_trial, *g_cur, *g_trial;
    int slot;
    int order[HIST_MAX + 1];
    double b[HIST_MAX];
    LbfgsArgs L;
    XiArgs X;
    double *S[HIST_MAX + 1], *Y[HIST_MAX + 1];
    double *log_alpha, *log_E, *log_g2;
    int *slot_kind;
    int logCap, kindCap;
    int pairNew;
    int abortEpoch;
    int holdEnable, holdNext, holdVerdict;
    int redo;
    int heldSlots, heldRejected;
    int pairSlots, pairRedo;
    int pairCtr[3], pairPad;
    int predHist[2], predCtr[2][4];
    const double *specPartials;
    double alphaMin;
    int specSlots, specRedo, firstTrials, unitFirst;
    double *u_old, *MY[HIST_MAX + 1];
    double *HS[HIST_MAX + 1];
    double *s_new, *y_new, *hs_new;
    double *hrec, *rec_new;
    const double *Lrec[HIST_MAX];
    double *my_new;
    const double *Lmy[HIST_MAX], *Lhs[HIST_MAX];
};
template <class DL>
__host__ __device__ inline void devloop_resolve(DL &C)
{
    C.s_new = C.S[C.slot];
    C.y_new = C.Y[C.slot];
    C.hs_new = C.HS[C.slot];
    const int m = C.L.m;
    for (int i = 0; i < HIST_MAX; ++i) {
        C.Lmy[i] = i < m ? C.MY[C.order[i]] : nullptr;
        C.Lhs[i] = i < m ? C.HS[C.order[i]] : nullptr;
    }
    C.my_new = m > 0 ? C.MY[C.order[m - 1]] : nullptr;
    C.rec_new = C.hrec ? C.hrec + 6 * C.slot : nullptr;
    for (int i = 0; i < HIST_MAX; ++i) C.Lrec[i] = (i < m && C.hrec) ? C.hrec + 6 * C.order[i] : nullptr;
}
struct VList {
    const int *v = nullptr;
    int n = 0;
};
constexpr int CTL_PLAIN = 0, CTL_PAIR = 1, CTL_SPEC = 2, CTL_VP = 3, CTL_PAIR_VP = 4;
struct CtlArgs {
    DevLoop *ctl;
    const double *partE, *partR, *alpha_dev;
    int *flags_host;
    int nbE;
    int init;
};
struct CtlLaunch {
    CtlArgs a;
    int form;
};

struct StepForwardArgs {
    const double *x0 = nullptr, *p = nullptr;
    double *x = nullptr;
    const double *spmv_partials = nullptr;
    double alpha = 0.0, alpha_min = 0.0;
    double *alpha_out = nullptr, *alpha_out_host = nullptr;
    VList vl;
};
void launch_step_forward(int n, const StepForwardArgs &a, hipStream_t st, const DevLoop *ctl = nullptr);
struct StepArgs {
    const double *p, *spmv_partials;
    double *alpha_out;
    double alpha_min;
};
struct ElemPassArgs {
    const double *x = nullptr, *xt = nullptr;
    int v0 = 0, v1 = 0;
    int grad = 0;
    double *partials = nullptr;
    const StepArgs *step = nullptr;
    bool pair = false;
};
int launch_elem_pass(const DevMesh &M, const DevPatches &PT, int mat, double dtSq, const ElemPassArgs &a, hipStream_t st,
                     const DevLoop *ctl = nullptr);
struct GatherArgs {
    const double *x, *xt, *g_old, *p, *alpha_dev;
    double *g_new, *s_new, *y_new;
    int make_pair;
    int iv0, iv1;
    int stage;
    const int *vp_ptr, *vp_off;
    double *rpad;
    const double *hp;
    const uint8_t *ownMask;
    const int *vlist;
    int nlist;
    const uint8_t *kind;
    int pre;
    double *gshare;
    int wide = -1;
};
void launch_vertex_gather(const DevMesh &M, const DevPatches &PT, const GatherArgs &a, const LbfgsArgs &L,
                          double *partials, hipStream_t st, const DevLoop *ctl = nullptr);
void launch_pair_stats(int n, const GatherArgs &a, const LbfgsArgs &L, double *partials, hipStream_t st,
                       const double *gsrc = nullptr, const DevLoop *ctl = nullptr);
void launch_multidot(int n, const double *v, const double *const *vecs, int m, double *partials,
                     hipStream_t st);
void launch_build_q(int n, const double *g, const LbfgsArgs &L, const double *xi_host, double *q,
                    hipStream_t st, const DevLoop *ctl = nullptr);
void launch_gemv(const DevParts &P, const double *q, hipStream_t st, const DevLoop *ctl = nullptr,
                 hipEvent_t ev0 = nullptr, hipEvent_t ev1 = nullptr, const CtlLaunch *ca = nullptr, int spec = 0);
void launch_elem_vertex(const DevVPatches &VP, int mat, const ElemVertArgs &a, hipStream_t st, const DevLoop *ctl);
bool dirstep_fits(const DevPatches &PT);
void launch_build_qpad(const DevParts &P, const double *g, const LbfgsArgs &L, const double *xi_host, hipStream_t st,
                       const DevLoop *ctl = nullptr, int spec = 0);
void launch_reduce_partial(const DevParts &P, hipStream_t st, const DevLoop *ctl = nullptr);
void launch_twolevel_pack(const DevParts &P, hipStream_t st);
struct MergeEarlyArgs {
    double *z = nullptr;
    double *partials = nullptr;
    double *partialsT = nullptr;
    int first = 0;
    const double *zsum = nullptr;
    const uint8_t *ownMask = nullptr;
    VList vl;
    const uint8_t *kind = nullptr;
    int pre = 0;
    double *zshare = nullptr;
    const CoarseMerge *co = nullptr;
    int wide = -1;
};
void launch_merge_early(const DevMesh &M, const DevParts &P, const MergeEarlyArgs &a, hipStream_t st, const DevLoop *ctl);
struct PackRed {
    const double *part;
    int rows, stride, cols, combine, dst;
    double s0, s1;
};
void launch_pack_iface(int nI, const int *idx, const double *src, double *pack, const double *tailp, int ntail, hipStream_t st,
                       const PackRed *red0 = nullptr, const PackRed *red1 = nullptr);
void launch_unpack_iface(int nI, const int *idx, const double *pack, const uint8_t *heldMask, double *dst, double *tailp, int ntail,
                         hipStream_t st, double *dst2 = nullptr, int ntail2 = 0);
void launch_masked_norm2(int n, const double *v, const uint8_t *ownMask, double *partials, hipStream_t st, int exact = 0);
void launch_mask_owned(int n, double *v, const uint8_t *ownMask, hipStream_t st);
void launch_gemv_part(const DevParts &P, int ls, const int4 *job, int njobs, const int2 *lwork, int nlwork, const double *q,
                      int n, double *p, hipStream_t st);
struct MergeArgs {
    double *z = nullptr;
    double *partials = nullptr;
    bool dots = false;
    bool divide = false;
    VList vl;
    const CoarseMerge *co = nullptr;
};
void launch_merge(const DevMesh &M, const DevParts &P, const LbfgsArgs &L, const MergeArgs &a, hipStream_t st,
                  const DevLoop *ctl = nullptr);
void launch_build_p(int n, const double *z, const LbfgsArgs &L, const double *c_partials,
                    const double *xi_host, double *p, hipStream_t st, const DevLoop *ctl = nullptr);
struct SpmvZpArgs {
    const double *Hval = nullptr, *z = nullptr;
    const double *c_partials = nullptr;
    bool ctrans = false;
    double *p = nullptr, *Hp = nullptr;
    double *partials = nullptr;
    double *partialsT = nullptr;
    int v0 = 0, v1 = -1;
    const uint8_t *rowMask = nullptr, *ownMask = nullptr;
    VList vl;
    int wide = -1;
};
void launch_spmv_zp(const DevMesh &M, const SpmvZpArgs &a, hipStream_t st, const DevLoop *ctl);
int launch_dirstep(const DevMesh &M, const DevPatches &PT, int mat, double dtSq, const SpmvZpArgs &d, const ElemPassArgs &e, hipStream_t st,
                   const DevLoop *ctl);
void launch_spmv_dots(const DevMesh &M, const double *Hval, const double *p, const double *g, double *Hp,
                      int v0, int v1, double *partials, hipStream_t st, const DevLoop *ctl = nullptr);
void launch_loop_control(DevLoop *ctl, const double *partE, int nbE, const double *partR,
                         const double *alpha_dev, int *flags_host, hipStream_t st, int init = 0);
void launch_elem_hessians(const DevMesh &M, int mat, double dtSq, const double *x, double *He,
                          hipStream_t st, const int *elist = nullptr, int nList = 0);
void launch_assemble(const DevMesh &M, const double *He, double *Hval, hipStream_t st, const int *blist = nullptr,
                     int nList = 0, const int *blk_ptr = nullptr, const int *blk_ent = nullptr, const double *mass = nullptr);
void launch_dense_fill(const DevParts &P, const double *Hval, hipStream_t st);
void launch_tile_level(const TileTask *tasks, int ntasks, const TileProd *prods, int *info, hipStream_t st, bool fastDiag = true,
                       const TileFillEntry *fill = nullptr, const double *Hval = nullptr);
void launch_tile_gemm(const TileTask *tasks, int ntasks, const TileProd *prods, hipStream_t st, const TileFillEntry *fill = nullptr,
                      const double *Hval = nullptr);
void launch_tile_flow(const TileTask *tasks, int ntasks, const TileProd *prods, const int *depPtr, const int *depIdx, int *done,
                      int *next, int epoch, int *info, int nwg, hipStream_t st, double waitMs, bool fastDiag = true,
                      const TileFillEntry *fill = nullptr, const double *Hval = nullptr);
void launch_clear_tiles(double *const *tiles, const int *lds_, int ntiles, hipStream_t st);
void launch_pd_assemble(const DevMesh &M, const DevPD &D, double dtSq, hipStream_t st);
void launch_pd_fill(const DevPD &D, int nnz, double *W2, hipStream_t st);
void launch_pd_apply(const DevPD &D, int nV, const double *q, double *z, hipStream_t st);
void launch_ic_fill(const DevIC &D, const double *Hval, double sigma, hipStream_t st);
void launch_ic_factor_colour(const DevIC &D, int c0, int c1, hipStream_t st);
void launch_ic_forward_colour(const DevIC &D, int c0, int c1, const double *b, hipStream_t st);
void launch_ic_backward_colour(const DevIC &D, int c0, int c1, double *x, hipStream_t st);
void launch_init_x(int nV, const uint8_t *fixed, const double *v, double dt, const double *gdtsq,
                   double *x, hipStream_t st);
void launch_be_update(int nV, const uint8_t *fixed, double *x, double *xn, double *v, double *xt,
                      double dt, const double *gdtsq, hipStream_t st);
void launch_scatter_rows(int n, const int *idx, const double *pos, double *x, hipStream_t st);
void launch_copy(int n, const double *src, double *dst, hipStream_t st);
void launch_zfinish(int nV, const int *dup, const LbfgsArgs &L, double *z, double *partials, hipStream_t st,
                    const DevLoop *ctl = nullptr, const CoarseMerge *co = nullptr);
void launch_gather_lame(const int *slotElem, size_t nSlots, const double *mu, const double *lam, double *mu_s, double *lam_s,
                        hipStream_t st);
void launch_x_tilde(int nV, const uint8_t *fixed, const double *xn, const double *v, double dt, const double *gdtsq, double *xt,
                    hipStream_t st);

enum { PCG_RUNNING = 0, PCG_CONVERGED = 1, PCG_BREAKDOWN = 2 };
struct PcgRec {
    double gamma, alpha;
    double rr;
    double bb;
    int iter;
    int state;
    int pad[6];
};
static_assert(sizeof(PcgRec) == 64, "two records and the |r|^2 columns are read back as one block");
struct DevPcg {
    PcgRec *rec = nullptr;
    double *partBT = nullptr;
    double *partAT = nullptr;
    double *partA = nullptr, *partB = nullptr;
    double *isd = nullptr;
    double *r = nullptr, *d = nullptr, *Hd = nullptr, *w = nullptr, *s = nullptr;
    double *pkt = nullptr;
};
constexpr int PCG_READBACK = 2 * (int)(sizeof(PcgRec) / sizeof(double)) + 2 * NB_RED;
void launch_pcg_init(const DevPcg &C, int n, const double *b, double *u, double *q, hipStream_t st);
void launch_pcg_spmv(const DevMesh &M, const DevPcg &C, const double *Hval, const double *zsum, int it, hipStream_t st);
void launch_pcg_update(const DevPcg &C, int n, double *u, double *q, int it, double rel_tol, hipStream_t st);
void launch_pcg_spmv_rows(const DevMesh &M, const DevPcg &C, const double *Hval, const double *zsum, int v0, int v1, int it, hipStream_t st);
void launch_pcg_update_packet(const DevPcg &C, int n, double *u, double *q, int it, double rel_tol, hipStream_t st);

constexpr int COARSE_MAX_PARTS = 256;
constexpr int COARSE_NC_MAX = 6 * COARSE_MAX_PARTS;
struct DevCoarse {
    int nParts = 0, nc = 0, ncp = 0, nPairs = 0;
    int *vsPtr = nullptr, *vsIdx = nullptr;
    int *svPtr = nullptr, *svIdx = nullptr;
    int2 *pair = nullptr;
    int *pairPtr = nullptr, *pairBlk = nullptr;
    int *pairAt = nullptr;
    int *live = nullptr;
    double *wgt = nullptr;
    double *xf = nullptr, *cen = nullptr;
    double *pairA = nullptr;
    double *W = nullptr, *W2 = nullptr;
    double *c = nullptr, *y = nullptr;
    int *info = nullptr;
    int nmax = 0;
    const int *dofmap = nullptr;
    double4 *rtab = nullptr;
    int p0 = 0, nOwn = 0;
    int as0 = 0, as1 = 0;
    int nHz = 0;
    int *hzPtr = nullptr, *hzSub = nullptr;
    int *hzVert = nullptr;
    int *hzBlkPtr = nullptr, *hzBlk = nullptr;
    int *hzTPtr = nullptr, *hzTEnt = nullptr;
    double *hz = nullptr;
    double *cd = nullptr;
    double *r1 = nullptr;
};
// ... 24 lines not shown
```

dot_amd/csrc/dotmi_plan.cpp:

```cpp
#include <algorithm>
#include <vector>

#include "../../include/dotmi.h"
#include "block_plan.hpp"
#include "coarse_plan.hpp"
#include "ic_plan.hpp"
#include "loop_forms.hpp"
#include "partition.hpp"
#include "pd_plan.hpp"
#include "tuning.hpp"
#include "vpatches.hpp"

using namespace dotmi;

namespace {

double *offset_base() { return reinterpret_cast<double *>(1ull << 40); }

long long row_block_table(int n_blocks, int nt, const uint8_t *live, const int32_t *c0, RowTileArrays &rt)
{
    const size_t rows = (size_t)n_blocks * nt;
    rt = RowTileArrays{std::vector<long long>(rows, -1), std::vector<int>(rows, 0), std::vector<int>(rows, 0)};
    long long at = 0;
    for (int b = 0; b < n_blocks; ++b)
// ... 27 lines not shown
            B.rtM.off[j] = B.storage;
            B.storage += 64ll * B.rtM.ld[j];
        }
    double *const W = offset_base();
    const std::vector<uint8_t> lv(live, live + nt), pat(pattern, pattern + (size_t)nt * nt);
    TileSchedule S;
    size_t sn = 0;
    plan_subdomain_tiles(0, nt, W, B.rt.off.data(), B.rt.ld.data(), B.rt.c0.data(), lv, pat, W + B.storage, sn, B.tasks, S.clearTiles,
                         S.clearLd, S.flops, S.qTiles, std::max(1, eager_min), std::max(1, eager_chunk), 0, true, -1,
                         leaf_tile ? B.rtM.off.data() : nullptr, leaf_tile ? B.rtM.ld.data() : nullptr,
                         leaf_tile ? B.rtM.c0.data() : nullptr, leaf_tile);
    std::stable_sort(B.tasks.begin(), B.tasks.end(), [](const TileTaskL &a, const TileTaskL &b) { return a.level < b.level; });
    return B;
}

long long plan_blocks(int n_blocks, int nt, const uint8_t *live, const uint8_t *pattern, int eager_min, int eager_chunk, int groups,
                      bool hfill, RowTileArrays &rt, TileSchedule &S)
{
    const long long tot = row_block_table(n_blocks, nt, nullptr, nullptr, rt);
    double *const W = offset_base(), *const W2 = W + (long long)n_blocks * tot;
    std::vector<SubdomainTiles> subs(n_blocks);
    size_t sn = 0;
    for (int b = 0; b < n_blocks; ++b) {
        std::vector<uint8_t> lv(live + (size_t)b * nt, live + (size_t)(b + 1) * nt);
        std::vector<uint8_t> pat(pattern + (size_t)b * nt * nt, pattern + (size_t)(b + 1) * nt * nt);
        plan_subdomain_tiles(b, nt, W, &rt.off[(size_t)b * nt], &rt.ld[(size_t)b * nt], &rt.c0[(size_t)b * nt], lv, pat, W2, sn,
                             subs[b].tasks, subs[b].clearTiles, subs[b].clearLd, S.flops, S.qTiles, std::max(1, eager_min),
                             std::max(1, eager_chunk), 0, true, -1, nullptr, nullptr, nullptr, nullptr, hfill);
    }
    finish_grouped_schedule(subs, groups, S);
    return tot;
}

void out(int32_t *dst, const std::vector<int> &src)
{
    if (dst) std::copy(src.begin(), src.end(), dst);
}

void vpatch_header(const HostVPatches &H, int32_t *hdr)
{
    const int32_t h[5] = {H.nPatches, H.PE, H.PV, H.PO, H.RUN};
    std::copy(h, h + 5, hdr);
}

}

extern "C" {

int dotmi_plan_shards(int32_t nParts, const int32_t *part_scalar_size, int32_t world, int32_t *first_part)
{
    if (nParts < 0 || world < 1 || !first_part || (nParts > 0 && !part_scalar_size)) return DOTMI_E_INVALID;
    std::vector<double> cost(nParts + 1, 0.0);
    for (int p = 0; p < nParts; ++p) cost[p + 1] = cost[p] + (double)part_scalar_size[p] * part_scalar_size[p];
    first_part[0] = 0;
    first_part[world] = nParts;
    for (int r = 1; r < world; ++r) {
        const double target = cost[nParts] * r / world;
        int c = (int)(std::lower_bound(cost.begin(), cost.end(), target) - cost.begin());
        if (c > 0 && target - cost[c - 1] < cost[c] - target) --c;
        c = std::min(std::max(c, first_part[r - 1]), nParts);
        first_part[r] = c;
    }
    return 0;
}

int dotmi_plan_loop_forms(int64_t ndof_gather, int64_t ndof_merge, int64_t nrows_spmv, int32_t force, int32_t *out)
{
    if (ndof_gather < 0 || ndof_merge < 0 || nrows_spmv < 0 || !out) return DOTMI_E_INVALID;
    *out = loop_forms_mask(ndof_gather, ndof_merge, nrows_spmv, force);
    return 0;
}

int dotmi_plan_backsolve_forms(int32_t cap, int32_t *forms, int32_t *counts)
{
    if (!counts || cap < 0 || (cap > 0 && !forms)) return DOTMI_E_INVALID;
    int n = 0;
    for (int fam : {BSF_PACK, BSF_NARROW, BSF_WIDE})
        for (int i = 0; i < bs_form_count(fam); ++i, ++n) {
            if (!forms) continue;
            if (n >= cap) return DOTMI_E_INVALID;
            const BsForm f = bs_form(fam, i);
            const int32_t row[6] = {fam, BSF_LANES[fam], f.chunks, f.sub, f.rlds, bs_form_capacity(fam, i)};
            if (bs_form_index(fam, row[5]) != i || bs_form_index(fam, row[5] + 1) != i + 1) return DOTMI_E_INVALID;
            std::copy(row, row + 6, forms + 6 * (size_t)n);
        }
    const int32_t c[4] = {n, BSL_THREADS, BSL_SUB, BS_LONG_CHUNK};
    std::copy(c, c + 4, counts);
    return 0;
}

int dotmi_plan_patches(int32_t nV, int32_t nT, const int32_t *T, const double *X, int32_t PE, int32_t *n_patches, int32_t *pv,
                       int32_t *n_slots, int32_t *elem, uint16_t *tl, uint16_t *epos, int32_t *pv_gid, int32_t *pv_slot,
                       int32_t *pv_cnt, uint16_t *c_ptr, int32_t *pp_rng)
{
    if (nV < 1 || nT < 1 || !T || !X || (PE != 256 && PE != 512) || !n_patches || !pv || !n_slots) return DOTMI_E_INVALID;
    std::vector<int> all(nT);
    for (int e = 0; e < nT; ++e) all[e] = e;
    const HostPatches H = build_patches(nV, T, X, all, PE);
    *n_patches = H.nPatches;
    *pv = H.PV;
    *n_slots = H.nSlots;
    if (!elem) return 0;
    std::copy(H.elem.begin(), H.elem.end(), elem);
    std::copy(H.tl.begin(), H.tl.end(), tl);
    std::copy(H.epos.begin(), H.epos.end(), epos);
    std::copy(H.pv_gid.begin(), H.pv_gid.end(), pv_gid);
    std::copy(H.pv_slot.begin(), H.pv_slot.end(), pv_slot);
    std::copy(H.pv_cnt.begin(), H.pv_cnt.end(), pv_cnt);
    std::copy(H.c_ptr.begin(), H.c_ptr.end(), c_ptr);
    std::copy(H.pp_rng.begin(), H.pp_rng.end(), pp_rng);
    return 0;
}

int dotmi_plan_vpatches(int32_t nV, int32_t nT, const int32_t *T, const double *X, int32_t PE, int32_t max_own, int32_t *hdr,
                        int32_t *owner, int32_t *elem, int32_t *eown, int32_t *runlen)
{
    if (nV < 1 || nT < 1 || !T || !X || PE < 1 || max_own < 1 || !hdr) return DOTMI_E_INVALID;
    const HostVPatches H = build_vpatches(nV, nT, T, X, PE, max_own);
    vpatch_header(H, hdr);
    if (!owner || H.nPatches == 0) return 0;
    for (int p = 0; p < H.nPatches; ++p) {
        const uint16_t *cp = &H.c_ptr[(size_t)p * (H.PO + 1)];
        for (int lv = 0; lv < H.po_cnt[p]; ++lv) {
            const int v = H.pv_gid[(size_t)p * H.PV + lv];
            owner[v] = p;
            if (runlen) runlen[v] = cp[lv + 1] - cp[lv];
        }
    }
    if (elem) std::copy(H.elem.begin(), H.elem.end(), elem);
    if (eown)
        for (size_t s = 0; s < H.eown.size(); ++s) eown[s] = H.eown[s];
    return 0;
}

int dotmi_plan_vpatch_records(int32_t nV, int32_t nT, const int32_t *T, const double *X, int32_t PE, int32_t max_own, const double *mass,
                              const uint8_t *fixed, const int32_t *vp_ptr, const int32_t *vp_off, const uint8_t *fixed2, int32_t *hdr,
                              int32_t *pv_gid, int32_t *po_cnt, double *rec_mass, int32_t *rec_fixed, int32_t *rec_cnt, int32_t *rec_off)
{
    if (nV < 1 || nT < 1 || !T || !X || PE < 1 || max_own < 1 || !mass || !fixed || !vp_ptr || !vp_off || !hdr) return DOTMI_E_INVALID;
    const HostVPatches H = build_vpatches(nV, nT, T, X, PE, max_own);
    vpatch_header(H, hdr);
    if (!pv_gid || H.nPatches == 0) return 0;
    if (!po_cnt || !rec_mass || !rec_fixed || !rec_cnt || !rec_off) return DOTMI_E_INVALID;
    std::vector<VpOwnRec> R = build_vpatch_records(H, mass, fixed, vp_ptr, vp_off);
    if (fixed2) refix_vpatch_records(vpatch_own_gid(H), fixed2, R);
    std::copy(H.pv_gid.begin(), H.pv_gid.end(), pv_gid);
    std::copy(H.po_cnt.begin(), H.po_cnt.end(), po_cnt);
    for (size_t i = 0; i < R.size(); ++i) {
        rec_mass[i] = R[i].mass;
        rec_fixed[i] = R[i].fixed;
        rec_cnt[i] = R[i].cnt;
        for (int c = 0; c < 4; ++c) rec_off[4 * i + c] = R[i].off[c];
    }
    return 0;
}

static int plan_tile_schedule_impl(int32_t nt, const uint8_t *live, const uint8_t *pattern, const int32_t *c0, int32_t eager_min,
                                   int32_t eager_chunk, int64_t *tasks, int64_t *prods, int64_t *n_tasks, int64_t *n_prods,
                                   int64_t *n_levels, int64_t *storage, int64_t *scratch_base, int64_t *row_off, int32_t *row_ld,
                                   const uint8_t *leaf_tile, const int32_t *c0m, const int32_t *ntm, int64_t *row_off_m,
                                   int32_t *row_ld_m)
{
    if (nt < 1 || !live || !pattern || !c0 || !n_tasks || !n_prods) return DOTMI_E_INVALID;
    const BlockTasks B = plan_one_block(nt, live, pattern, c0, eager_min, eager_chunk, leaf_tile, c0m, ntm);
    const std::vector<TileTaskL> &all = B.tasks;
    size_t np = 0;
    for (auto &t : all) np += t.prods.size();
    *n_tasks = (int64_t)all.size();
    *n_prods = (int64_t)np;
    if (n_levels) *n_levels = all.empty() ? 0 : all.back().level;
    if (storage) *storage = B.storage;
    if (scratch_base) *scratch_base = B.storage;
    if (row_off) std::copy(B.rt.off.begin(), B.rt.off.end(), row_off);
    if (row_ld) std::copy(B.rt.ld.begin(), B.rt.ld.end(), row_ld);
    if (row_off_m) std::copy(B.rtM.off.begin(), B.rtM.off.end(), row_off_m);
    if (row_ld_m) std::copy(B.rtM.ld.begin(), B.rtM.ld.end(), row_ld_m);
    if (!tasks || !prods) return 0;
    const double *const W = offset_base();
    size_t pi = 0;
    for (size_t k = 0; k < all.size(); ++k) {
        const TileTask &t = all[k].t;
        const int64_t row[11] = {all[k].level, t.form, t.init, t.post, (int64_t)all[k].prods.size(), (int64_t)pi, t.c - W,
                                 t.q ? t.q - W : -1, t.ldc, t.ldq, t.o - W};
        std::copy(row, row + 11, tasks + 11 * k);
        for (auto &pr : all[k].prods) {
            const int64_t q[4] = {pr.a - W, pr.b - W, pr.lda, pr.ldb};
            std::copy(q, q + 4, prods + 4 * pi++);
        }
    }
    return 0;
}

int dotmi_plan_tile_schedule(int32_t nt, const uint8_t *live, const uint8_t *pattern, const int32_t *c0, int32_t eager_min,
                             int32_t eager_chunk, int64_t *tasks, int64_t *prods, int64_t *n_tasks, int64_t *n_prods,
                             int64_t *n_levels, int64_t *storage, int64_t *scratch_base, int64_t *row_off, int32_t *row_ld)
{
    return plan_tile_schedule_impl(nt, live, pattern, c0, eager_min, eager_chunk, tasks, prods, n_tasks, n_prods, n_levels, storage,
                                   scratch_base, row_off, row_ld, nullptr, nullptr, nullptr, nullptr, nullptr);
}
int dotmi_plan_tile_schedule_two_level(int32_t nt, const uint8_t *live, const uint8_t *pattern, const int32_t *c0,
                                       const uint8_t *leaf_tile, const int32_t *c0m, const int32_t *ntm, int32_t eager_min,
                                       int32_t eager_chunk, int64_t *tasks, int64_t *prods, int64_t *n_tasks, int64_t *n_prods,
                                       int64_t *n_levels, int64_t *storage, int64_t *row_off, int32_t *row_ld, int64_t *row_off_m,
                                       int32_t *row_ld_m)
{
    if (!leaf_tile || !c0m || !ntm) return DOTMI_E_INVALID;
    return plan_tile_schedule_impl(nt, live, pattern, c0, eager_min, eager_chunk, tasks, prods, n_tasks, n_prods, n_levels, storage,
                                   nullptr, row_off, row_ld, leaf_tile, c0m, ntm, row_off_m, row_ld_m);
}

int dotmi_plan_tile_groups(int32_t n_parts, const int64_t *weight, int32_t groups, int32_t *group_of)
{
    if (n_parts < 1 || !weight || !group_of) return DOTMI_E_INVALID;
    std::vector<long long> w(weight, weight + n_parts);
    std::vector<int> g(n_parts, 0);
    const int G = plan_tile_groups(n_parts, w.data(), groups, g.data());
    std::copy(g.begin(), g.end(), group_of);
    return G;
}

int dotmi_plan_grouped_tile_schedule(int32_t n_blocks, int32_t nt, const uint8_t *live, const uint8_t *pattern, int32_t eager_min,
                                     int32_t eager_chunk, int32_t groups, int64_t *tasks, int64_t *n_tasks, int32_t *group_of,
                                     int32_t *group_level, int64_t *clear, int64_t *n_clear, int32_t n_fill, const int32_t *fill_sub,
                                     int32_t *fill_perm, int32_t *fill_start)
{
    if (n_blocks < 1 || nt < 1 || !live || !pattern || !n_tasks || !n_clear || n_fill < 0 || (n_fill > 0 && !fill_sub))
        return DOTMI_E_INVALID;
    for (int e = 0; e < n_fill; ++e)
        if (fill_sub[e] < 0 || fill_sub[e] >= n_blocks) return DOTMI_E_INVALID;
    RowTileArrays rt;
    TileSchedule S;
    plan_blocks(n_blocks, nt, live, pattern, eager_min, eager_chunk, groups, false, rt, S);
    const double *const W = offset_base();
    const int G = (int)S.groupLevel.size() - 1;
    *n_tasks = (int64_t)S.tasks.size();
    *n_clear = (int64_t)S.clearTiles.size();
    if (!tasks) return G;
    if (!group_of || !group_level || !clear || !fill_perm || !fill_start) return DOTMI_E_INVALID;
    std::copy(S.groupOf.begin(), S.groupOf.end(), group_of);
    std::copy(S.groupLevel.begin(), S.groupLevel.end(), group_level);
    for (int g = 0; g < G; ++g) {
        for (int l = S.groupLevel[g]; l < S.groupLevel[g + 1]; ++l)
            for (int k = S.levelStart[l]; k < S.levelStart[l + 1]; ++k) {
                const TileTask &t = S.tasks[k];
                const int64_t row[6] = {g, l - S.groupLevel[g] + 1, t.sub, t.o - W, t.post, t.nprod};
                std::copy(row, row + 6, tasks + 6 * (size_t)k);
            }
        for (int k = S.clearStart[g]; k < S.clearStart[g + 1]; ++k) {
            clear[2 * (size_t)k] = g;
            clear[2 * (size_t)k + 1] = S.clearTiles[k] - W;
        }
    }
    std::vector<int> perm, start;
    partition_by_group(fill_sub, (size_t)n_fill, S.groupOf, G, perm, start);
    std::copy(perm.begin(), perm.end(), fill_perm);
    std::copy(start.begin(), start.end(), fill_start);
    return G;
}

static void export_tile_fill(const TileSchedule &S, const double *W, const double *W2, int64_t *tasks, int64_t *clear,
                             int32_t *entry_pos, int32_t *entry_src)
{
    const int G = (int)S.groupLevel.size() - 1;
    for (int g = 0; g < G; ++g) {
        for (int l = S.groupLevel[g]; l < S.groupLevel[g + 1]; ++l)
            for (int k = S.levelStart[l]; k < S.levelStart[l + 1]; ++k) {
                const TileTask &t = S.tasks[k];
                const bool inv = t.form == TF_INV;
                const int64_t row[10] = {g, l - S.groupLevel[g] + 1, t.sub, t.c - (inv ? W : W2),
                                         t.o - (inv || t.post == TP_DIAG ? W : W2), t.init, t.post, t.fillFirst, t.fillCount, t.form};
                std::copy(row, row + 10, tasks + 10 * (size_t)k);
            }
        for (int k = S.clearStart[g]; k < S.clearStart[g + 1]; ++k) {
            const int64_t row[5] = {g, S.clearTiles[k] - W2, S.clearLd[k], S.fillPtr[k], S.fillPtr[k + 1] - S.fillPtr[k]};
            std::copy(row, row + 5, clear + 5 * (size_t)k);
        }
    }
    for (size_t e = 0; e < S.fill.size(); ++e) {
        entry_pos[e] = S.fill[e].pos;
        entry_src[e] = S.fill[e].src;
    }
}

int dotmi_plan_tile_fill(int32_t n_blocks, int32_t nt, const uint8_t *live, const uint8_t *pattern, int32_t eager_min,
                         int32_t eager_chunk, int32_t groups, int64_t n_fill, const int64_t *fill_dst, const int32_t *fill_src,
                         int64_t n_pad, const int64_t *pad_dst, int64_t *counts, int64_t *tasks, int64_t *clear, int32_t *entry_pos,
                         int32_t *entry_src)
{
    if (n_blocks < 1 || nt < 1 || !live || !pattern || !counts || n_fill < 0 || n_pad < 0 || (n_fill > 0 && (!fill_dst || !fill_src)) ||
        (n_pad > 0 && !pad_dst))
        return DOTMI_E_INVALID;
    RowTileArrays rt, rtM;
    TileSchedule S;
    const long long tot = plan_blocks(n_blocks, nt, live, pattern, eager_min, eager_chunk, groups, true, rt, S);
    const double *const W = offset_base(), *const W2 = W + (long long)n_blocks * tot;
    FillLists fill;
    fill.fill_dst.assign(fill_dst, fill_dst + 9 * n_fill);
    fill.fill_src.assign(fill_src, fill_src + n_fill);
    fill.pad_dst.assign(pad_dst, pad_dst + n_pad);
    for (long long d : fill.fill_dst)
        if (d >= (long long)n_blocks * tot) return DOTMI_E_INVALID;
    for (long long d : fill.pad_dst)
        if (d < 0 || d >= (long long)n_blocks * tot) return DOTMI_E_INVALID;
    if (!build_tile_fill(S, W2, fill, rt, rtM).empty()) return DOTMI_E_INVALID;
    const int G = (int)S.groupLevel.size() - 1;
    const int64_t c[8] = {(int64_t)S.tasks.size(), (int64_t)S.clearTiles.size(), (int64_t)S.fill.size(), n_fill, n_pad, G,
// ... 266 lines not shown
```

dot_amd/csrc/k_elemvert.hip:

```cpp
#include "k_device.hpp"
#include "vpatches.hpp"

namespace dotmi {

typedef double ev_pair __attribute__((ext_vector_type(2)));

constexpr int EV_EPT = 2;

#ifdef K_PROFILE
__device__ long long g_evprof[512][8];
extern "C" int dotmi_debug_evprof(long long *out)
{
    return (int)hipMemcpyFromSymbol(out, HIP_SYMBOL(g_evprof), sizeof(long long) * 512 * 8);
}
#define EVSTAMP(i) do { if (threadIdx.x == 0 && blockIdx.x < 512) g_evprof[blockIdx.x][i] = wall_clock64(); } while (0)
#else
#define EVSTAMP(i) do { } while (0)
#endif

template <int MAT, bool PAIR, bool REC>
__global__ __launch_bounds__(256) void elem_vertex_kernel(DevVPatches VP, ElemVertArgs a, const DevLoop *__restrict__ ctl)
{
    extern __shared__ double lds[];
    __shared__ double sm[4 * RED_K];
    __shared__ double sme[8];
    __shared__ double sh_alpha;
    const bool pairedLaunch = PAIR && a.alpha_min < 0.0;
    const double alphaMin = pairedLaunch ? -a.alpha_min : a.alpha_min;
    const bool second = pairedLaunch && (int)blockIdx.x >= VP.nPatches;
    const int tid = threadIdx.x, p = second ? (int)blockIdx.x - VP.nPatches : (int)blockIdx.x;
    long long t_start = 0;
#ifdef K_PROFILE
    t_start = wall_clock64();
#endif
    const double *__restrict__ x = a.x0;
    double *__restrict__ x_out = nullptr, *__restrict__ g_out = a.g0;
    const double *__restrict__ g_old = nullptr;
    double *__restrict__ s_new = nullptr, *__restrict__ y_new = nullptr, *__restrict__ hs_new = nullptr;
    const double *hs[HIST_MAX], *hy[HIST_MAX];
    const ev_pair *hr[HIST_MAX];
    ev_pair *rec_new = nullptr;
    int hm = 0, lphase = 1;
    double lalpha = 0.0;
    const bool loop = ctl != nullptr;
    if (loop) {
        const int status = ctl->status;
        lphase = ctl->phase;
        lalpha = ctl->alpha;
        x = ctl->x_cur;
        x_out = ctl->x_trial;
        g_out = ctl->g_trial;
        g_old = ctl->g_cur;
        s_new = ctl->s_new;
        y_new = ctl->y_new;
        hs_new = ctl->hs_new;
        hm = ctl->L.m;
#pragma unroll
        for (int i = 0; i < HIST_MAX; ++i) {
            if constexpr (REC) {
                hr[i] = reinterpret_cast<const ev_pair *>(ctl->Lrec[i]);
            } else {
                hs[i] = ctl->L.s[i];
                hy[i] = ctl->L.y[i];
            }
        }
        if constexpr (REC) rec_new = reinterpret_cast<ev_pair *>(ctl->rec_new);
        if (status != 0) return;
    }
#ifdef K_PROFILE
    if (threadIdx.x == 0 && blockIdx.x < 512) g_evprof[blockIdx.x][7] = t_start;
#endif
    EVSTAMP(0);
    double pgv[NB_RED / 64], pHpv[NB_RED / 64];
    const bool usePart = loop && lphase == 0;
    if (usePart && tid < 64) {
#pragma unroll
        for (int u = 0; u < NB_RED / 64; ++u) {
            pgv[u] = a.spmv_partials[tid + 64 * u];
            pHpv[u] = a.spmv_partials[NB_RED + tid + 64 * u];
        }
    }
    constexpr int PE = 256 * EV_EPT;
    double *xs = lds, *gs = lds + 3 * VP.PV;
    double *po = gs + 3 * VP.RUN, *xo = po + 3 * VP.PO;
    unsigned short *cptr = reinterpret_cast<unsigned short *>(REC ? xo + 3 * VP.PO : po);
    const int nv = VP.pv_cnt[p], no = VP.po_cnt[p];
    const size_t vb = (size_t)p * VP.PV;
    const int gid = tid < VP.PV ? VP.pv_gid[vb + tid] : -1;
    const unsigned short cp_reg = tid <= VP.PO ? VP.c_ptr[(size_t)p * (VP.PO + 1) + tid] : (unsigned short)0;
    const int ov = tid / 3, od = tid - 3 * ov;
    const int ogid_raw = ov < VP.PV ? VP.pv_gid[vb + ov] : -1;
    const bool vlane = tid < 3 * no;
    const int ogid = vlane ? ogid_raw : -1;
    double2 rq0 = make_double2(0.0, 0.0);
    int4 rq1 = make_int4(0, 0, 0, 0);
    if constexpr (REC) {
        if (ov < VP.PO) {
            const VpOwnRec *r = VP.orec + ((size_t)p * VP.PO + ov);
            rq0 = *reinterpret_cast<const double2 *>(r);
            rq1 = *reinterpret_cast<const int4 *>(&r->off[0]);
        }
    }
    ushort4 tl[EV_EPT], ep[EV_EPT];
    double Ai[EV_EPT][9], mu_[EV_EPT], la_[EV_EPT], vo[EV_EPT], voE[EV_EPT];
    const size_t strideA = (size_t)VP.nPatches * PE;
#pragma unroll
    for (int u = 0; u < EV_EPT; ++u) {
        const size_t s = (size_t)p * PE + u * 256 + tid;
        tl[u] = VP.tl[s];
        ep[u] = VP.epos[s];
#pragma unroll
        for (int k = 0; k < 9; ++k) Ai[u][k] = VP.A[(size_t)k * strideA + s];
        mu_[u] = VP.mu ? VP.mu[s] : VP.mu0;
        la_[u] = VP.mu ? VP.lam[s] : VP.lam0;
        vo[u] = VP.vol[s];
        voE[u] = VP.volE[s];
    }
    double xv[3] = {0, 0, 0}, pv[3] = {0, 0, 0};
    if (gid >= 0) {
#pragma unroll
        for (int d = 0; d < 3; ++d) {
            xv[d] = x[3 * gid + d];
            if (loop) pv[d] = a.p[3 * gid + d];
        }
    }
    const int ok = 3 * ogid + od;
    bool fx = true;
    double gold = 0.0, pk = 0.0, hpk = 0.0, ms = 0.0, xt_own = 0.0, xtv[3] = {0, 0, 0}, si[HIST_MAX], yi[HIST_MAX];
    int cb = 0, ce = 0;
#pragma unroll
    for (int i = 0; i < HIST_MAX; ++i) si[i] = yi[i] = 0.0;
    if constexpr (REC) {
        if (vlane) {
            fx = __double2hiint(rq0.y) != 0;
            ms = rq0.x;
            ce = __double2loint(rq0.y);
            xt_own = a.xt[ok];
            if (loop) {
                gold = g_old[ok];
                hpk = a.hp[ok];
                const size_t rk = (size_t)(3 * (HIST_MAX + 1)) * ogid + od;
#pragma unroll
                for (int i = 0; i < HIST_MAX; ++i) {
                    ev_pair sy = {0.0, 0.0};
                    if (i < hm) sy = hr[i][rk];
                    si[i] = sy.x;
                    yi[i] = sy.y;
                }
            }
        }
    } else if (vlane) {
        fx = a.fixed[ogid] != 0;
        ms = a.mass[ogid];
        xt_own = a.xt[ok];
        if (od == 0) {
#pragma unroll
            for (int d = 0; d < 3; ++d) xtv[d] = a.xt[3 * ogid + d];
        }
        cb = a.vp_ptr[ogid];
        ce = a.vp_ptr[ogid + 1];
        if (loop) {
            gold = g_old[ok];
            pk = a.p[ok];
            hpk = a.hp[ok];
#pragma unroll
            for (int i = 0; i < HIST_MAX; ++i) {
                si[i] = (i < hm) ? hs[i][ok] : 0.0;
                yi[i] = (i < hm) ? hy[i][ok] : 0.0;
            }
        }
    }
    if (tid <= VP.PO) cptr[tid] = cp_reg;
    EVSTAMP(1);
    if (tid < 64) {
        double al = loop ? lalpha : 0.0;
        if (usePart) {
            double pg = 0.0, pHp = 0.0;
#pragma unroll
            for (int u = 0; u < NB_RED / 64; ++u) {
                pg += pgv[u];
                pHp += pHpv[u];
            }
            pg = __shfl(wave_sum(pg), 0, 64);
            pHp = __shfl(wave_sum(pHp), 0, 64);
            al = ls_first_step(pg, pHp, alphaMin);
        }
        if (tid == 0) {
            if constexpr (PAIR) {
                const bool pair = pairedLaunch && usePart && al < 1.0 && al / 2.0 > 0.0 && ctl->pairCtr[pair_band(al)] >= 3;
                sh_alpha = pair ? (second ? al : al / 2.0) : (second ? -1.0 : al);
                if (blockIdx.x == 0) {
                    a.alpha_out[0] = pair ? al / 2.0 : al;
                    if (pairedLaunch) a.alpha_out[1] = pair ? al : 0.0;
                }
            } else {
                sh_alpha = al;
                if (p == 0 && loop) *a.alpha_out = al;
            }
        }
    }
    __syncthreads();
    const double alpha = sh_alpha;
    if (second && alpha < 0.0) return;
    EVSTAMP(2);
    if (gid >= 0) {
#pragma unroll
        for (int d = 0; d < 3; ++d) xs[3 * tid + d] = loop ? xv[d] + alpha * pv[d] : xv[d];
        if constexpr (REC) {
            if (loop && tid < no) {
#pragma unroll
                for (int d = 0; d < 3; ++d) po[3 * tid + d] = pv[d];
            }
        }
    }
    for (int lv = tid + 256; lv < nv; lv += 256) {
        const int g2 = VP.pv_gid[vb + lv];
#pragma unroll
        for (int d = 0; d < 3; ++d) xs[3 * lv + d] = loop ? x[3 * g2 + d] + alpha * a.p[3 * g2 + d] : x[3 * g2 + d];
    }
    __syncthreads();
    EVSTAMP(3);
    constexpr int VC = 4;
    int vof[VC];
    if constexpr (REC) {
        vof[0] = rq1.x;
        vof[1] = rq1.y;
        vof[2] = rq1.z;
        vof[3] = rq1.w;
    } else {
#pragma unroll
        for (int c = 0; c < VC; ++c) vof[c] = (cb + c < ce) ? a.vp_off[cb + c] : 0;
    }
    double acc = 0.0;
#pragma unroll
    for (int u = 0; u < EV_EPT; ++u) {
        if (tl[u].x == 0xFFFF) continue;
        const double *p0 = xs + 3 * tl[u].x, *p1 = xs + 3 * tl[u].y, *p2 = xs + 3 * tl[u].z, *p3 = xs + 3 * tl[u].w;
        Mat3 F;
#pragma unroll
        for (int r = 0; r < 3; ++r) {
            const double d0 = p1[r] - p0[r], d1 = p2[r] - p0[r], d2 = p3[r] - p0[r];
#pragma unroll
            for (int c = 0; c < 3; ++c) F.m[r][c] = d0 * Ai[u][c] + d1 * Ai[u][3 + c] + d2 * Ai[u][6 + c];
        }
        const double w = a.dtSq * vo[u];
        double P[3][3];
        if constexpr (MAT == 1) {
            const double J = det3(F);
            const double ic = F.m[0][0] * F.m[0][0] + F.m[0][1] * F.m[0][1] + F.m[0][2] * F.m[0][2] +
                              F.m[1][0] * F.m[1][0] + F.m[1][1] * F.m[1][1] + F.m[1][2] * F.m[1][2] +
                              F.m[2][0] * F.m[2][0] + F.m[2][1] * F.m[2][1] + F.m[2][2] * F.m[2][2];
            const double JmA = J - (1.0 + mu_[u] / la_[u]);
            acc += (mu_[u] * (ic - 3.0) + la_[u] * JmA * JmA) / 2.0 * voE[u];
            const double t = la_[u] * JmA;
#pragma unroll
            for (int r = 0; r < 3; ++r) {
                const int r1 = (r + 1) % 3, r2 = (r + 2) % 3;
#pragma unroll
                for (int c = 0; c < 3; ++c) {
                    const int c1 = (c + 1) % 3, c2 = (c + 2) % 3;
                    const double cof = F.m[r1][c1] * F.m[r2][c2] - F.m[r1][c2] * F.m[r2][c1];
                    P[r][c] = w * (mu_[u] * F.m[r][c] + t * cof);
                }
            }
        } else if constexpr (MAT == 2) {
            acc += snh_log_energy_stress(F, mu_[u], la_[u], w, true, P) * voE[u];
        } else {
            Mat3 U, V;
            double S[3];
            svd3(F, U, S, V);
            acc += psi<MAT>(S, mu_[u], la_[u]) * voE[u];
            double dd[3];
            dpsi<MAT>(S, mu_[u], la_[u], dd);
#pragma unroll
            for (int r = 0; r < 3; ++r)
#pragma unroll
                for (int c = 0; c < 3; ++c)
                    P[r][c] = w * (U.m[r][0] * dd[0] * V.m[c][0] + U.m[r][1] * dd[1] * V.m[c][1] + U.m[r][2] * dd[2] * V.m[c][2]);
        }
        double g[12];
#pragma unroll
        for (int aa = 0; aa < 3; ++aa)
#pragma unroll
            for (int c = 0; c < 3; ++c)
                g[3 + 3 * aa + c] = Ai[u][3 * aa] * P[c][0] + Ai[u][3 * aa + 1] * P[c][1] + Ai[u][3 * aa + 2] * P[c][2];
#pragma unroll
        for (int c = 0; c < 3; ++c) g[c] = -g[3 + c] - g[6 + c] - g[9 + c];
        const int pkk[4] = {ep[u].x, ep[u].y, ep[u].z, ep[u].w};
#pragma unroll
        for (int k = 0; k < 4; ++k)
            if (pkk[k] != 0xFFFF && !second) {
                gs[pkk[k]] = g[3 * k];
                gs[VP.RUN + pkk[k]] = g[3 * k + 1];
                gs[2 * VP.RUN + pkk[k]] = g[3 * k + 2];
            }
    }
    if constexpr (REC) {
        if (vlane) xo[tid] = xt_own;
    }
    __syncthreads();
    EVSTAMP(4);
    if constexpr (REC) {
        if (vlane) {
            if (loop) pk = po[tid];
            if (od == 0) {
                xtv[0] = xt_own;
                xtv[1] = xo[tid + 1];
                xtv[2] = xo[tid + 2];
            }
        }
    }
    double st[RED_K];
#pragma unroll
    for (int j = 0; j < RED_K; ++j) st[j] = 0.0;
    double ine = 0.0;
    if (vlane && second) {
        if (od == 0) {
            const double dx = xs[3 * ov] - xtv[0], dy = xs[3 * ov + 1] - xtv[1], dz = xs[3 * ov + 2] - xtv[2];
            ine = (dx * dx + dy * dy + dz * dz) * ms / 2.0;
        }
    } else if (vlane) {
        const int kb = cptr[ov], ke = cptr[ov + 1];
        const double *run = gs + od * VP.RUN;
        double sum = 0.0;
        for (int k = kb; k < ke; k += 4) {
            const double w0 = run[k], w1 = k + 1 < ke ? run[k + 1] : 0.0, w2 = k + 2 < ke ? run[k + 2] : 0.0,
                         w3 = k + 3 < ke ? run[k + 3] : 0.0;
            sum += w0;
            if (k + 1 < ke) sum += w1;
            if (k + 2 < ke) sum += w2;
            if (k + 3 < ke) sum += w3;
        }
        const double xt_k = xs[3 * ov + od];
        const double g = fx ? 0.0 : sum + ms * (xt_k - xt_own);
        if (x_out) x_out[ok] = xt_k;
        g_out[ok] = g;
#pragma unroll
        for (int c = 0; c < VC; ++c)
            if (cb + c < ce) a.rpad[vof[c] + od] = -g;
        if constexpr (REC) {
            if (ce > VC) {
                const int c0 = a.vp_ptr[ogid];
                for (int c = c0 + VC; c < c0 + ce; ++c) a.rpad[a.vp_off[c] + od] = -g;
            }
        } else {
            for (int c = cb + VC; c < ce; ++c) a.rpad[a.vp_off[c] + od] = -g;
        }
        st[0] = g * g;
        if (loop) {
            const double sn = alpha * pk;
            const double yn = g - gold;
            s_new[ok] = sn;
            y_new[ok] = yn;
            if constexpr (REC) rec_new[(size_t)(3 * (HIST_MAX + 1)) * ogid + od] = ev_pair{sn, yn};
            hs_new[ok] = alpha * hpk;
            st[1] = yn * sn;
            st[2] = sn * g;
#pragma unroll
            for (int i = 0; i < HIST_MAX; ++i)
                if (i < hm) {
                    st[3 + i] = si[i] * yn;
                    st[3 + HIST_MAX + i] = sn * yi[i];
                    st[3 + 2 * HIST_MAX + i] = si[i] * g;
                }
        }
        if (od == 0) {
            const double dx = xs[3 * ov] - xtv[0], dy = xs[3 * ov + 1] - xtv[1], dz = xs[3 * ov + 2] - xtv[2];
            ine = (dx * dx + dy * dy + dz * dz) * ms / 2.0;
        }
    }
    EVSTAMP(5);
    const double we = wave_sum(acc), wi = wave_sum(ine);
    const int lane = tid & 63, wv = tid >> 6;
    if (lane == 0) {
        sme[wv] = we;
        sme[4 + wv] = wi;
    }
    if (!second) write_partials(st, loop ? RED_K : 1, a.partR, sm);
    else __syncthreads();
    if (tid == 0) {
        double *pe = second ? a.partE + 2 * ELEM_NB_MAX : a.partE;
        pe[2 * p] = (sme[0] + sme[1]) + (sme[2] + sme[3]);
        pe[2 * p + 1] = (sme[4] + sme[5]) + (sme[6] + sme[7]);
    }
    EVSTAMP(6);
}

void launch_elem_vertex(const DevVPatches &VP, int mat, const ElemVertArgs &a, hipStream_t st, const DevLoop *ctl)
{
    const bool rec = VP.orec != nullptr;
    const size_t shm = elem_vertex_dyn_lds(VP.PV, VP.RUN, VP.PO, rec);
    const bool paired = ctl && a.alpha_min < 0.0;
#define EV_LAUNCH(MATV, PAIRV, NWG)                                                                                          \
    do {                                                                                                                     \
        if (rec) hipLaunchKernelGGL((elem_vertex_kernel<MATV, PAIRV, true>), dim3(NWG), dim3(256), shm, st, VP, a, ctl);     \
        else hipLaunchKernelGGL((elem_vertex_kernel<MATV, PAIRV, false>), dim3(NWG), dim3(256), shm, st, VP, a, ctl);        \
    } while (0)
#define EV_LAUNCH_M(MATV)                                      \
    do {                                                       \
        if (paired) EV_LAUNCH(MATV, true, 2 * VP.nPatches);    \
        else EV_LAUNCH(MATV, false, VP.nPatches);              \
    } while (0)
    DM_DISPATCH_MAT(mat, EV_LAUNCH_M)
#undef EV_LAUNCH_M
#undef EV_LAUNCH
}

}
```

dot_amd/csrc/tuning.hpp:

```cpp
#pragma once
#include <algorithm>
#include <cstdlib>

#include "nd_layout.hpp"

struct Tuning {
    int ndLevels = -1;
    int ndMin = dotmi::ND_MIN_SPLIT;
    bool ndMinByUser = false;
    bool wavePacks = true;
    int tilePasses = 4;
    int tileRows = 0;
    int tileRowsLong = 0;
    int twoLevel = -1;
    int splitMerge = -1;
    bool fuseLog = false;
    bool factorGraph = true;
    int shardElems = -1;
    int shardHess = -1;
    int timeStride = 8;
    int patchElems = 0;
    int tileSplit = -1;
    int tileGroups = -1;
    int tileHfill = 1;
    int tileEagerMin = 0;
    int fastDiag = 1;
    int tileFlow = -1;
    int tileFlowWaitMs = 2000;
    int tileEagerMinRmul = -1;
    bool tileEagerMinRmulByUser = false;
    bool fuseDir = true;
    int wideForms = -1;
    bool fuseStep = true;
    int pairTrials = -1;
    int vertexPatches = -1;
    int specStep = 0;
    bool earlyHold = true;
    int earlyBs = 2;
    int operandRecords = 1;
    static int geti(const char *name, int dflt)
    {
        const char *ev = getenv(name);
        return ev ? atoi(ev) : dflt;
    }
    static Tuning from_env()
    {
        Tuning t;
        t.wavePacks = geti("DOTMI_WAVE_PACKS", 1) != 0;
        t.tilePasses = std::min(8, std::max(1, geti("DOTMI_TILE_PASSES", 4)));
        t.ndLevels = geti("DOTMI_ND_LEVELS", -1);
        if (t.ndLevels < -1) t.ndLevels = 0;
        t.ndMin = std::max(128, geti("DOTMI_ND_MIN", dotmi::ND_MIN_SPLIT));
        t.ndMinByUser = getenv("DOTMI_ND_MIN") != nullptr;
        if (const char *ev = getenv("DOTMI_TILE_ROWS")) t.tileRows = std::min(64, std::max(8, atoi(ev) / 8 * 8));
        t.tileRowsLong = geti("DOTMI_TILE_ROWS_LONG", 0);
        if (t.tileRowsLong > 0) t.tileRowsLong = std::min(64, std::max(8, t.tileRowsLong / 8 * 8));
        t.splitMerge = geti("DOTMI_SPLIT_MERGE", -1);
        t.twoLevel = geti("DOTMI_TWO_LEVEL", -1);
        t.fuseLog = getenv("DOTMI_FUSE_LOG") != nullptr;
        t.factorGraph = geti("DOTMI_FACTOR_GRAPH", 1) != 0;
        t.shardElems = geti("DOTMI_SHARD_ELEMS", -1);
        t.shardHess = geti("DOTMI_SHARD_HESS", -1);
        t.timeStride = std::max(1, geti("DOTMI_TIME_STRIDE", 8));
        t.patchElems = std::max(0, geti("DOTMI_PATCH_ELEMS", 0));
        t.tileSplit = geti("DOTMI_TILE_SPLIT", -1);
        t.tileGroups = geti("DOTMI_TILE_GROUPS", -1);
        t.tileHfill = geti("DOTMI_TILE_HFILL", 1) != 0;
        t.tileEagerMin = std::max(0, geti("DOTMI_TILE_EAGER_MIN", 0));
        t.tileFlow = geti("DOTMI_TILE_FLOW", -1);
        t.fastDiag = geti("DOTMI_FAST_DIAG", 1);
        t.tileFlowWaitMs = std::max(1, geti("DOTMI_TILE_FLOW_WAIT_MS", 2000));
        t.tileEagerMinRmul = geti("DOTMI_TILE_EAGER_MIN_RMUL", -1);
        t.tileEagerMinRmulByUser = getenv("DOTMI_TILE_EAGER_MIN_RMUL") != nullptr;
        t.earlyBs = geti("DOTMI_EARLY_BACKSOLVE", 2) != 0 ? 2 : 0;
        t.earlyHold = geti("DOTMI_EARLY_HOLD", 1) != 0;
        t.pairTrials = geti("DOTMI_PAIR_TRIALS", -1);
        t.specStep = geti("DOTMI_SPEC_STEP", 0);
        t.vertexPatches = geti("DOTMI_VERTEX_PATCHES", -1);
        t.fuseStep = geti("DOTMI_FUSE_STEP", 1) != 0;
        t.fuseDir = geti("DOTMI_FUSE_DIR", 1) != 0;
        t.wideForms = geti("DOTMI_WIDE_FORMS", -1);
        if (t.wideForms < -1) t.wideForms = -1;
        t.operandRecords = geti("DOTMI_OPERAND_RECORDS", 1) & 1;
        return t;
    }
};
```

dot_amd/csrc/vpatches.hpp:

```cpp
#pragma once
#include <algorithm>
#include <cstdint>
#include <vector>

#include "patches.hpp"

namespace dotmi {

struct HostVPatches {
    int nPatches = 0, PE = 0, PV = 0, PO = 0, RUN = 0;
    std::vector<int> elem;
    std::vector<uint16_t> tl;
    std::vector<uint16_t> epos;
    std::vector<uint8_t> eown;
    std::vector<int> pv_gid;
    std::vector<int> pv_cnt, po_cnt;
    std::vector<uint16_t> c_ptr;
};

inline HostVPatches build_vpatches(int nV, int nT, const int32_t *T, const double *X, int PE, int maxOwn)
{
    HostVPatches H;
    H.PE = PE;
    double lo[3] = {1e300, 1e300, 1e300}, hi[3] = {-1e300, -1e300, -1e300};
// ... 7 lines not shown
    if (!(ext > 0)) ext = 1.0;
    std::vector<std::pair<uint64_t, int>> key(nV);
    for (int v = 0; v < nV; ++v) {
        uint32_t q[3];
        for (int d = 0; d < 3; ++d) q[d] = (uint32_t)std::min(2097151.0, std::max(0.0, (X[3 * v + d] - lo[d]) / ext * 2097151.0));
        key[v] = {morton3(q[0], q[1], q[2]), v};
    }
    std::sort(key.begin(), key.end());
    std::vector<int> ip(nV + 1, 0), ie((size_t)4 * nT);
    for (int e = 0; e < nT; ++e)
        for (int k = 0; k < 4; ++k) ip[T[4 * e + k] + 1]++;
    for (int v = 0; v < nV; ++v) ip[v + 1] += ip[v];
    {
        std::vector<int> at(ip.begin(), ip.end() - 1);
        for (int e = 0; e < nT; ++e)
            for (int k = 0; k < 4; ++k) ie[at[T[4 * e + k]]++] = e;
    }
    std::vector<int> owner(nV, -1), mark(nT, -1);
    std::vector<std::vector<int>> own, els;
    {
        std::vector<int> curOwn, curEl;
        auto flush = [&]() {
            if (curOwn.empty()) return;
            own.push_back(curOwn);
            els.push_back(curEl);
            curOwn.clear();
            curEl.clear();
        };
        for (int i = 0; i < nV; ++i) {
            const int v = key[i].second, p = (int)own.size();
            int add = 0;
            for (int q = ip[v]; q < ip[v + 1]; ++q) add += mark[ie[q]] != p;
            if (!curOwn.empty() && ((int)curEl.size() + add > PE || (int)curOwn.size() >= maxOwn)) flush();
            const int pp = (int)own.size();
            for (int q = ip[v]; q < ip[v + 1]; ++q)
                if (mark[ie[q]] != pp) {
                    mark[ie[q]] = pp;
                    curEl.push_back(ie[q]);
                }
            curOwn.push_back(v);
            owner[v] = pp;
        }
        flush();
    }
    H.nPatches = (int)own.size();
    int pvmax = 0, pomax = 0, runmax = 0, emax = 0;
    std::vector<std::vector<int>> pverts(H.nPatches);
    for (int p = 0; p < H.nPatches; ++p) {
        std::sort(els[p].begin(), els[p].end());
        std::sort(own[p].begin(), own[p].end());
        std::vector<int> others;
        for (int e : els[p])
            for (int k = 0; k < 4; ++k)
                if (owner[T[4 * e + k]] != p) others.push_back(T[4 * e + k]);
        std::sort(others.begin(), others.end());
        others.erase(std::unique(others.begin(), others.end()), others.end());
        pverts[p] = own[p];
        pverts[p].insert(pverts[p].end(), others.begin(), others.end());
        pvmax = std::max(pvmax, (int)pverts[p].size());
        pomax = std::max(pomax, (int)own[p].size());
        emax = std::max(emax, (int)els[p].size());
        int run = 0;
        for (int v : own[p]) run += ip[v + 1] - ip[v];
        runmax = std::max(runmax, run);
    }
    if (emax > PE) {
        H.nPatches = 0;
        return H;
    }
    H.PV = std::max(8, (pvmax + 7) / 8 * 8);
    H.PO = pomax;
    H.RUN = (runmax + 7) / 8 * 8;
    H.elem.assign((size_t)H.nPatches * PE, -1);
    H.tl.assign((size_t)H.nPatches * PE * 4, 0xFFFF);
    H.epos.assign((size_t)H.nPatches * PE * 4, 0xFFFF);
    H.eown.assign((size_t)H.nPatches * PE, 0);
    H.pv_gid.assign((size_t)H.nPatches * H.PV, -1);
    H.pv_cnt.assign(H.nPatches, 0);
    H.po_cnt.assign(H.nPatches, 0);
    H.c_ptr.assign((size_t)H.nPatches * (H.PO + 1), 0);
    std::vector<int> loc(nV, -1);
    for (int p = 0; p < H.nPatches; ++p) {
        const auto &pv = pverts[p];
        const int no = (int)own[p].size();
        H.pv_cnt[p] = (int)pv.size();
        H.po_cnt[p] = no;
        for (size_t lv = 0; lv < pv.size(); ++lv) {
            H.pv_gid[(size_t)p * H.PV + lv] = pv[lv];
            loc[pv[lv]] = (int)lv;
        }
        uint16_t *cp = &H.c_ptr[(size_t)p * (H.PO + 1)];
        int off = 0;
        for (int lv = 0; lv < no; ++lv) {
            cp[lv] = (uint16_t)off;
            off += ip[pv[lv] + 1] - ip[pv[lv]];
        }
        for (int lv = no; lv <= H.PO; ++lv) cp[lv] = (uint16_t)off;
        std::vector<int> at(no);
        for (int lv = 0; lv < no; ++lv) at[lv] = cp[lv];
        const size_t eb = (size_t)p * PE;
        for (size_t i = 0; i < els[p].size(); ++i) {
            const int e = els[p][i];
            H.elem[eb + i] = e;
            H.eown[eb + i] = owner[T[4 * e]] == p ? 1 : 0;
            for (int k = 0; k < 4; ++k) {
                const int lv = loc[T[4 * e + k]];
                H.tl[(eb + i) * 4 + k] = (uint16_t)lv;
                if (lv < no) H.epos[(eb + i) * 4 + k] = (uint16_t)at[lv]++;
            }
        }
        for (int v : pv) loc[v] = -1;
    }
    return H;
}

struct VpOwnRec {
    double mass;
    int32_t cnt;
    int32_t fixed;
    int32_t off[4];
};
static_assert(sizeof(VpOwnRec) == 32, "two 16-byte loads per lane");

inline std::vector<VpOwnRec> build_vpatch_records(const HostVPatches &H, const double *mass, const uint8_t *fixed, const int *vp_ptr,
                                                  const int *vp_off)
{
    std::vector<VpOwnRec> R((size_t)H.nPatches * H.PO, VpOwnRec{0.0, 0, 0, {0, 0, 0, 0}});
    for (int p = 0; p < H.nPatches; ++p)
        for (int lv = 0; lv < H.po_cnt[p]; ++lv) {
            const int v = H.pv_gid[(size_t)p * H.PV + lv];
            VpOwnRec &r = R[(size_t)p * H.PO + lv];
            r.mass = mass[v];
            r.fixed = fixed[v] != 0;
            r.cnt = vp_ptr[v + 1] - vp_ptr[v];
            for (int c = 0; c < 4 && c < r.cnt; ++c) r.off[c] = vp_off[vp_ptr[v] + c];
        }
    return R;
}

inline std::vector<int> vpatch_own_gid(const HostVPatches &H)
{
    std::vector<int> g((size_t)H.nPatches * H.PO, -1);
    for (int p = 0; p < H.nPatches; ++p)
        for (int lv = 0; lv < H.po_cnt[p]; ++lv) g[(size_t)p * H.PO + lv] = H.pv_gid[(size_t)p * H.PV + lv];
    return g;
}

inline void refix_vpatch_records(const std::vector<int> &own_gid, const uint8_t *fixed, std::vector<VpOwnRec> &R)
{
    for (size_t i = 0; i < own_gid.size(); ++i)
        if (own_gid[i] >= 0) R[i].fixed = fixed[own_gid[i]] != 0;
}

}
```

dot_amd/lib.py:

```python
from __future__ import annotations

import ctypes as C
import os

import numpy as np

_HERE = os.path.dirname(os.path.abspath(__file__))
LIB_PATH = os.environ.get("DOTMI_LIBRARY") or os.path.join(_HERE, "libdotmi.so")

c_dp = C.POINTER(C.c_double)
c_ip = C.POINTER(C.c_int32)
c_up = C.POINTER(C.c_uint8)

ENERGY_FCR = 0
ENERGY_SNH = 1
ENERGY_SNH_LOG = 2
FLAG_TIME_BACKSOLVE = 2
FLAG_FORCE_DIST = 4
FLAG_HOST_LOOP = 8
FLAG_TIME_PHASES = 16
FLAG_GSDD = 32
FLAG_NEWTON = 64
FLAG_ASYNC_REFRESH = 128
FLAG_OWNER_EXCHANGE = 256
FLAG_LBFGS_PD = 512
FLAG_LBFGS_HI = 1024
FLAG_NEWTON_PCG = 2048
FLAG_DOT_COARSE = 4096
DOTMI_FLAG_NEWTON_PCG_DIST = 8192


class Mesh(C.Structure):
    _fields_ = [("nV", C.c_int32), ("nT", C.c_int32), ("X_rest", c_dp), ("T", c_ip), ("mu", c_dp),
                ("lam", c_dp), ("density", C.c_double), ("fixed", c_up), ("epart", c_ip),
                ("nParts", C.c_int32), ("vpart", c_ip)]


class Params(C.Structure):
    _fields_ = [("energy", C.c_int32), ("dt", C.c_double), ("gravity", C.c_double * 3),
                ("relTol", C.c_double), ("history", C.c_int32), ("iterCap", C.c_int32),
                ("alphaMin", C.c_double), ("device", C.c_int32), ("rank", C.c_int32),
                ("world", C.c_int32), ("comm_id", C.c_void_p), ("flags", C.c_int32),
                ("allreduce", C.c_void_p), ("allreduce_ctx", C.c_void_p)]


ALLREDUCE_CB = C.CFUNCTYPE(None, C.c_void_p, C.POINTER(C.c_double), C.c_int64)


class StepStats(C.Structure):
    _fields_ = [("iters", C.c_int32), ("ls_halvings", C.c_int32), ("energy_evals", C.c_int32),
                ("status", C.c_int32), ("E0", C.c_double), ("g2_0", C.c_double), ("E", C.c_double),
                ("g2", C.c_double), ("ms_total", C.c_double), ("ms_loop", C.c_double),
                ("ms_hessian", C.c_double), ("ms_factor", C.c_double), ("ms_precond", C.c_double),
                ("precond_launches", C.c_int64), ("precond_bytes", C.c_int64),
                ("factor_flops", C.c_double), ("ms_phase", C.c_double * 14),
                ("collective_calls", C.c_int64), ("collective_bytes", C.c_int64), ("ms_collective", C.c_double),
                ("collective_timed", C.c_int64), ("collective_timed_bytes", C.c_int64),
                ("backsolve_launches", C.c_int64), ("backsolve_stopped", C.c_int64),
                ("backsolve_held", C.c_int64), ("backsolve_held_rejected", C.c_int64),
                ("paired_slots", C.c_int64), ("paired_redone", C.c_int64),
                ("spec_slots", C.c_int64), ("spec_redone", C.c_int64)]


BENCH_KERNELS = ["elem_energy_grad", "elem_energy", "vertex_gather", "spmv_dots", "backsolve", "merge", "build_qpad",
                 "build_p", "step_forward", "elem_hessian", "assemble",
                 "spmv_zp", "merge_early", "elem_step", "gather_early", "dirstep", "elem_vertex"]

EXPORTS = [
    "dotmi_create", "dotmi_destroy", "dotmi_last_error", "dotmi_comm_unique_id", "dotmi_comm_ranks", "dotmi_set_state",
    "dotmi_get_state", "dotmi_set_dirichlet", "dotmi_refix", "dotmi_step", "dotmi_last_iter_log",
    "dotmi_target_gres", "dotmi_eval_energy", "dotmi_eval_gradient", "dotmi_eval_elem_hessians",
    "dotmi_refactor", "dotmi_apply_precond", "dotmi_spmv", "dotmi_get_features", "dotmi_part_size", "dotmi_padded_size",
    "dotmi_part_matrix", "dotmi_factor_storage_bytes", "dotmi_factor_kind", "dotmi_factor_groups", "dotmi_backsolve_form", "dotmi_plan_backsolve_form", "dotmi_probe_direction", "dotmi_bench_precond", "dotmi_bench_energy", "dotmi_bench_kernel", "dotmi_plan_shards", "dotmi_plan_layout", "dotmi_plan_tile_schedule", "dotmi_plan_tile_schedule_two_level", "dotmi_plan_tile_deps", "dotmi_plan_tile_groups", "dotmi_plan_grouped_tile_schedule", "dotmi_plan_tile_fill", "dotmi_plan_tile_fill_mesh", "dotmi_plan_backsolve_tiles", "dotmi_plan_backsolve_forms", "dotmi_plan_patches", "dotmi_plan_vpatches", "dotmi_plan_vpatch_records", "dotmi_operand_records", "dotmi_loop_forms", "dotmi_plan_loop_forms", "dotmi_plan_rank", "dotmi_partition",
    "dotmi_plan_pd",
    "dotmi_plan_ic", "dotmi_ic_info", "dotmi_ic_factor",
    "dotmi_set_rel_tol", "dotmi_set_time_step", "dotmi_set_lame",
    "dotmi_solve_hessian", "dotmi_set_pcg", "dotmi_pcg_info",
    "dotmi_set_pcg_coarse", "dotmi_pcg_coarse_info", "dotmi_pcg_coarse_matrix", "dotmi_pcg_apply_precond", "dotmi_plan_coarse",
    "dotmi_set_dot_coarse", "dotmi_dot_coarse_info", "dotmi_set_dot_coarse_mode", "dotmi_dot_coarse_mode", "dotmi_plan_coarse_hz",
]

_lib = None


class DotmiError(RuntimeError):
    pass


def load() -> C.CDLL:
    global _lib
    if _lib is not None:
        return _lib
    if not os.path.exists(LIB_PATH):
        raise DotmiError(f"{LIB_PATH} not built: run `python -c 'import __graft_entry__ as g; g.build()'` "
                         "(or make -C dot_amd/csrc). There is no CPU fallback.")
    L = C.CDLL(LIB_PATH)
    H = C.c_void_p
    L.dotmi_create.argtypes = [C.POINTER(Mesh), C.POINTER(Params), c_dp, C.POINTER(H)]
    L.dotmi_create.restype = C.c_int
    L.dotmi_destroy.argtypes = [H]
    L.dotmi_destroy.restype = None
    L.dotmi_last_error.argtypes = [H]
    L.dotmi_last_error.restype = C.c_char_p
    L.dotmi_comm_unique_id.argtypes = [C.c_void_p]
    if hasattr(L, "dotmi_comm_ranks"):
        L.dotmi_comm_ranks.argtypes = [H]
        L.dotmi_comm_ranks.restype = C.c_int32
    L.dotmi_set_state.argtypes = [H, c_dp, c_dp, c_dp]
    L.dotmi_get_state.argtypes = [H, c_dp, c_dp, c_dp]
    L.dotmi_set_dirichlet.argtypes = [H, C.c_int32, c_ip, c_dp]
    L.dotmi_refix.argtypes = [H, c_up]
    L.dotmi_set_rel_tol.argtypes = [H, C.c_double]
    L.dotmi_set_time_step.argtypes = [H, C.c_double]
    L.dotmi_set_lame.argtypes = [H, c_dp, c_dp]
    L.dotmi_step.argtypes = [H, C.POINTER(StepStats)]
    L.dotmi_last_iter_log.argtypes = [H, C.c_int32, c_dp, c_dp, c_dp]
    L.dotmi_target_gres.argtypes = [H]
    L.dotmi_target_gres.restype = C.c_double
    L.dotmi_eval_energy.argtypes = [H, c_dp, c_dp]
    L.dotmi_eval_gradient.argtypes = [H, c_dp, c_dp]
    L.dotmi_eval_elem_hessians.argtypes = [H, c_dp, c_dp]
    L.dotmi_refactor.argtypes = [H, c_dp]
    L.dotmi_apply_precond.argtypes = [H, c_dp, c_dp]
    L.dotmi_spmv.argtypes = [H, c_dp, c_dp]
    L.dotmi_get_features.argtypes = [H, c_dp, c_dp, c_dp]
    L.dotmi_part_size.argtypes = [H, C.c_int32]
    L.dotmi_part_size.restype = C.c_int32
    L.dotmi_padded_size.argtypes = [H]
    L.dotmi_padded_size.restype = C.c_int32
    L.dotmi_part_matrix.argtypes = [H, C.c_int32, C.c_int, c_dp, c_ip]
    L.dotmi_probe_direction.argtypes = [H, c_dp, C.c_int32, c_dp, c_dp, c_dp, c_dp, c_dp, c_dp, c_dp, c_dp]
    L.dotmi_factor_storage_bytes.argtypes = [H]
    L.dotmi_factor_storage_bytes.restype = C.c_int64
    if hasattr(L, "dotmi_backsolve_form"):
        L.dotmi_backsolve_form.argtypes = [H]
        L.dotmi_backsolve_form.restype = C.c_int32
    if hasattr(L, "dotmi_factor_kind"):
        L.dotmi_factor_kind.argtypes = [H]
        L.dotmi_factor_kind.restype = C.c_int32
    if hasattr(L, "dotmi_factor_groups"):
        L.dotmi_factor_groups.argtypes = [H]
        L.dotmi_factor_groups.restype = C.c_int32
    L.dotmi_bench_precond.argtypes = [H, C.c_int32, c_dp, C.POINTER(C.c_int64)]
    L.dotmi_bench_energy.argtypes = [H, C.c_int32, c_dp, C.POINTER(C.c_int64)]
    L.dotmi_bench_kernel.argtypes = [H, C.c_int32, C.c_int32, c_dp, C.POINTER(C.c_int64)]
    L.dotmi_plan_shards.argtypes = [C.c_int32, c_ip, C.c_int32, c_ip]
    L.dotmi_plan_rank.argtypes = [C.c_int32, C.c_int32, c_ip, c_ip, C.c_int32, C.c_int32, C.c_int32, c_ip, c_ip, c_ip, c_ip,
                                  c_ip, c_ip, c_ip]
    L.dotmi_partition.argtypes = [C.c_int32, C.c_int32, c_ip, c_dp, C.c_int32, c_ip]
    if hasattr(L, "dotmi_operand_records"):
        L.dotmi_operand_records.argtypes = [H]
        L.dotmi_operand_records.restype = C.c_int32
    if hasattr(L, "dotmi_loop_forms"):
        L.dotmi_loop_forms.argtypes = [H]
        L.dotmi_loop_forms.restype = C.c_int32
        L.dotmi_plan_loop_forms.argtypes = [C.c_int64, C.c_int64, C.c_int64, C.c_int32, c_ip]
    if hasattr(L, "dotmi_plan_pd"):
        L.dotmi_plan_pd.argtypes = [C.c_int32, C.c_int32, c_ip, c_dp, c_ip, C.POINTER(C.c_int64)]
    if hasattr(L, "dotmi_plan_ic"):
        L.dotmi_plan_ic.argtypes = [C.c_int32, C.c_int32, c_ip] + [c_ip] * 10
        L.dotmi_ic_info.argtypes = [H, c_ip, c_dp, c_ip]
        L.dotmi_ic_factor.argtypes = [H, C.c_int32, c_dp]
    if hasattr(L, "dotmi_solve_hessian"):
        L.dotmi_solve_hessian.argtypes = [H, c_dp, c_dp, C.c_double, C.c_int32, c_ip, c_dp]
        L.dotmi_set_pcg.argtypes = [H, C.c_double, C.c_int32, C.c_int32]
        L.dotmi_pcg_info.argtypes = [H, C.POINTER(C.c_int64), C.POINTER(C.c_int64), c_ip, c_dp]
    if hasattr(L, "dotmi_set_pcg_coarse"):
        L.dotmi_set_pcg_coarse.argtypes = [H, C.c_int32]
        L.dotmi_pcg_coarse_info.argtypes = [H, c_ip, c_ip, c_ip, C.POINTER(C.c_int64)]
        L.dotmi_pcg_coarse_matrix.argtypes = [H, C.c_int32, c_dp]
        L.dotmi_pcg_apply_precond.argtypes = [H, c_dp, c_dp]
        L.dotmi_plan_coarse.argtypes = [C.c_int32, C.c_int32, c_ip, c_ip, C.c_int32] + [c_ip] * 9
    if hasattr(L, "dotmi_set_dot_coarse"):
        L.dotmi_set_dot_coarse.argtypes = [H, C.c_int32]
        L.dotmi_dot_coarse_info.argtypes = [H, c_ip, c_ip, c_ip, C.POINTER(C.c_int64), c_dp]
    if hasattr(L, "dotmi_dot_coarse_mode"):
        L.dotmi_set_dot_coarse_mode.argtypes = [H, C.c_int32]
        L.dotmi_dot_coarse_mode.argtypes = [H]
        L.dotmi_dot_coarse_mode.restype = C.c_int32
        L.dotmi_plan_coarse_hz.argtypes = [C.c_int32, C.c_int32, c_ip, c_ip, C.c_int32] + [c_ip] * 8
    L.dotmi_plan_layout.argtypes = [C.c_int32, C.c_int32, c_ip, c_dp, c_ip, C.c_int32, C.c_int32, C.c_int32,
                                    C.c_int32, C.c_int32, C.c_int32, c_ip, c_ip, c_ip, c_ip]
    if hasattr(L, "dotmi_plan_backsolve_tiles"):
        L.dotmi_plan_backsolve_tiles.argtypes = [C.c_int32, C.c_int32, c_ip, c_dp, c_ip, C.c_int32, C.c_int32, C.c_int32,
                                                 C.c_int32, c_ip, c_ip]
    if hasattr(L, "dotmi_plan_backsolve_forms"):
        L.dotmi_plan_backsolve_forms.argtypes = [C.c_int32, c_ip, c_ip]
    for name in EXPORTS:
        fn = getattr(L, name, None)
        if fn is None:
            continue
        if fn.restype is C.c_int or name in ("dotmi_create",):
            fn.restype = C.c_int
    _lib = L
    return L


def dp(a: np.ndarray):
    return a.ctypes.data_as(c_dp)


def ip(a: np.ndarray):
    return a.ctypes.data_as(c_ip)


def up(a: np.ndarray):
    return a.ctypes.data_as(c_up)
```

include/dotmi.h:

```cpp
#ifndef DOTMI_H
#define DOTMI_H

#include <stdint.h>

#ifdef __cplusplus
extern "C" {
#endif

#define DOTMI_ENERGY_FCR 0
#define DOTMI_ENERGY_SNH 1
#define DOTMI_ENERGY_SNH_LOG 2

#define DOTMI_E_INVALID -1
#define DOTMI_E_DEVICE -2
#define DOTMI_E_NOTSPD -3
#define DOTMI_E_NOGPU -4

typedef struct dotmi_handle dotmi_handle;

typedef struct {
    int32_t nV, nT;
    const double *X_rest;
    const int32_t *T;
    const double *mu;
    const double *lambda;
    double density;
    const uint8_t *fixed;
    const int32_t *epart;
    int32_t nParts;
    const int32_t *vpart;
} dotmi_mesh;

typedef struct {
    int32_t energy;
    double dt;
    double gravity[3];
    double relTol;
    int32_t history;
    int32_t iterCap;
    double alphaMin;
    int32_t device;
    int32_t rank;
    int32_t world;
    const void *comm_id;
    int32_t flags;
    void (*allreduce)(void *ctx, double *buf, int64_t n);
    void *allreduce_ctx;
} dotmi_params;

#define DOTMI_FLAG_FORCE_DIST 4
#define DOTMI_FLAG_TIME_BACKSOLVE 2
#define DOTMI_FLAG_HOST_LOOP 8

#define DOTMI_FLAG_TIME_PHASES 16

enum {
    DOTMI_T_MATRIX_COMPUTATION = 0,
    DOTMI_T_MATRIX_ASSEMBLY = 1,
    DOTMI_T_SYMBOLIC_FACTORIZATION = 2,
    DOTMI_T_NUMERICAL_FACTORIZATION = 3,
    DOTMI_T_BACKSOLVE = 4,
    DOTMI_T_LINESEARCH_OTHER = 5,
    DOTMI_T_MODIFY_GRAD = 6,
    DOTMI_T_MODIFY_SEARCHDIR = 7,
    DOTMI_T_UPDATE_HISTORY = 8,
    DOTMI_T_LINESEARCH_EVAL = 9,
    DOTMI_T_FULLYIMPLICIT_ECOMP = 10,
    DOTMI_T_SOLVE_EXTRACOMP = 11,
    DOTMI_T_COMPGRAD = 12,
    DOTMI_T_CCD = 13,
    DOTMI_T_COUNT = 14
};

#define DOTMI_FLAG_GSDD 32

#define DOTMI_FLAG_ASYNC_REFRESH 128
#define DOTMI_FLAG_NEWTON 64
#define DOTMI_FLAG_OWNER_EXCHANGE 256
#define DOTMI_FLAG_LBFGS_PD 512
#define DOTMI_FLAG_LBFGS_HI 1024
#define DOTMI_FLAG_NEWTON_PCG 2048
#define DOTMI_FLAG_DOT_COARSE 4096
#define DOTMI_FLAG_NEWTON_PCG_DIST 8192

typedef struct {
    int32_t iters;
    int32_t ls_halvings;
    int32_t energy_evals;
    int32_t status;
    double E0, g2_0;
    double E, g2;
    double ms_total;
    double ms_loop;
    double ms_hessian;
    double ms_factor;
    double ms_precond;
    int64_t precond_launches;
    int64_t precond_bytes;
    double factor_flops;
    double ms_phase[DOTMI_T_COUNT];
    int64_t collective_calls;
    int64_t collective_bytes;
    double ms_collective;
    int64_t collective_timed;
    int64_t collective_timed_bytes;
    int64_t backsolve_launches;
    int64_t backsolve_stopped;
    int64_t backsolve_held;
    int64_t backsolve_held_rejected;
    int64_t paired_slots;
    int64_t paired_redone;
    int64_t spec_slots;
    int64_t spec_redone;
} dotmi_step_stats;

int dotmi_create(const dotmi_mesh *mesh, const dotmi_params *params, const double *x_init,
                 dotmi_handle **out);
void dotmi_destroy(dotmi_handle *h);
const char *dotmi_last_error(const dotmi_handle *h);

int dotmi_plan_shards(int32_t nParts, const int32_t *part_scalar_size, int32_t world, int32_t *first_part);

int dotmi_plan_rank(int32_t nV, int32_t nT, const int32_t *T, const int32_t *epart, int32_t nParts, int32_t rank,
                    int32_t world, int32_t *p0, int32_t *p1, int32_t *elems, int32_t *n_elems, int32_t *v0, int32_t *v1,
                    int32_t *part_size);

int dotmi_plan_patches(int32_t nV, int32_t nT, const int32_t *T, const double *X, int32_t PE, int32_t *n_patches, int32_t *pv,
                       int32_t *n_slots, int32_t *elem, uint16_t *tl, uint16_t *epos, int32_t *pv_gid, int32_t *pv_slot,
                       int32_t *pv_cnt, uint16_t *c_ptr, int32_t *pp_rng);
int dotmi_plan_vpatches(int32_t nV, int32_t nT, const int32_t *T, const double *X, int32_t PE, int32_t max_own, int32_t *hdr,
                        int32_t *owner, int32_t *elem, int32_t *eown, int32_t *runlen);
int dotmi_operand_records(const dotmi_handle *h);
int dotmi_loop_forms(const dotmi_handle *h);
int dotmi_plan_loop_forms(int64_t ndof_gather, int64_t ndof_merge, int64_t nrows_spmv, int32_t force, int32_t *out);
int dotmi_plan_vpatch_records(int32_t nV, int32_t nT, const int32_t *T, const double *X, int32_t PE, int32_t max_own, const double *mass,
                              const uint8_t *fixed, const int32_t *vp_ptr, const int32_t *vp_off, const uint8_t *fixed2, int32_t *hdr,
                              int32_t *pv_gid, int32_t *po_cnt, double *rec_mass, int32_t *rec_fixed, int32_t *rec_cnt, int32_t *rec_off);
int dotmi_plan_tile_schedule(int32_t nt, const uint8_t *live, const uint8_t *pattern, const int32_t *c0, int32_t eager_min,
                             int32_t eager_chunk, int64_t *tasks, int64_t *prods, int64_t *n_tasks, int64_t *n_prods,
                             int64_t *n_levels, int64_t *storage, int64_t *scratch_base, int64_t *row_off, int32_t *row_ld);
int dotmi_plan_tile_schedule_two_level(int32_t nt, const uint8_t *live, const uint8_t *pattern, const int32_t *c0,
                                       const uint8_t *leaf_tile, const int32_t *c0m, const int32_t *ntm, int32_t eager_min,
                                       int32_t eager_chunk, int64_t *tasks, int64_t *prods, int64_t *n_tasks, int64_t *n_prods,
                                       int64_t *n_levels, int64_t *storage, int64_t *row_off, int32_t *row_ld, int64_t *row_off_m,
                                       int32_t *row_ld_m);
int dotmi_plan_tile_deps(int32_t nt, const uint8_t *live, const uint8_t *pattern, const int32_t *c0, int32_t eager_min,
                         int32_t eager_chunk, int64_t *dep_ptr, int64_t *dep_idx, int64_t *n_deps);
int dotmi_plan_tile_groups(int32_t n_parts, const int64_t *weight, int32_t groups, int32_t *group_of);
int dotmi_plan_grouped_tile_schedule(int32_t n_blocks, int32_t nt, const uint8_t *live, const uint8_t *pattern, int32_t eager_min,
                                     int32_t eager_chunk, int32_t groups, int64_t *tasks, int64_t *n_tasks, int32_t *group_of,
                                     int32_t *group_level, int64_t *clear, int64_t *n_clear, int32_t n_fill, const int32_t *fill_sub,
                                     int32_t *fill_perm, int32_t *fill_start);
int dotmi_plan_tile_fill(int32_t n_blocks, int32_t nt, const uint8_t *live, const uint8_t *pattern, int32_t eager_min,
                         int32_t eager_chunk, int32_t groups, int64_t n_fill, const int64_t *fill_dst, const int32_t *fill_src,
                         int64_t n_pad, const int64_t *pad_dst, int64_t *counts, int64_t *tasks, int64_t *clear, int32_t *entry_pos,
                         int32_t *entry_src);
int dotmi_plan_tile_fill_mesh(int32_t nV, int32_t nT, const int32_t *T, const double *Xrest, const int32_t *epart, int32_t nParts,
                              int32_t groups, int32_t two_level, int64_t *counts, int64_t *tasks, int64_t *clear, int32_t *entry_pos,
                              int32_t *entry_src, int64_t *fill_dst, int32_t *fill_src, int64_t *pad_dst);
int dotmi_plan_backsolve_tiles(int32_t nV, int32_t nT, const int32_t *T, const double *Xrest, const int32_t *epart, int32_t nParts,
                               int32_t p0, int32_t p1, int32_t cap, int32_t *tiles, int32_t *counts);
int dotmi_plan_backsolve_forms(int32_t cap, int32_t *forms, int32_t *counts);
int dotmi_plan_layout(int32_t nV, int32_t nT, const int32_t *T, const double *Xrest, const int32_t *epart,
                      int32_t nParts, int32_t p0, int32_t p1, int32_t levels, int32_t min_split,
                      int32_t node_cap, int32_t *nodes, int32_t *n_nodes, int32_t *nmax, int32_t *pos);

int dotmi_partition(int32_t nV, int32_t nT, const int32_t *T, const double *X, int32_t nParts, int32_t *epart);

int dotmi_comm_unique_id(void *out128);
int32_t dotmi_comm_ranks(const dotmi_handle *h);

int dotmi_set_state(dotmi_handle *h, const double *x, const double *v, const double *x_n );
int dotmi_get_state(dotmi_handle *h, double *x, double *v, double *x_tilde );
int dotmi_set_dirichlet(dotmi_handle *h, int32_t n, const int32_t *idx, const double *pos);
int dotmi_refix(dotmi_handle *h, const uint8_t *fixed);

int dotmi_set_rel_tol(dotmi_handle *h, double relTol);
int dotmi_set_time_step(dotmi_handle *h, double dt);
int dotmi_set_lame(dotmi_handle *h, const double *mu, const double *lambda);

int dotmi_step(dotmi_handle *h, dotmi_step_stats *stats);
int dotmi_last_iter_log(const dotmi_handle *h, int32_t cap, double *alpha, double *E, double *g2);
double dotmi_target_gres(const dotmi_handle *h);

int dotmi_eval_energy(dotmi_handle *h, const double *x, double *E);
int dotmi_eval_gradient(dotmi_handle *h, const double *x, double *g);
int dotmi_eval_elem_hessians(dotmi_handle *h, const double *x, double *H);
int dotmi_refactor(dotmi_handle *h, const double *x );
int dotmi_apply_precond(dotmi_handle *h, const double *r, double *p);
int dotmi_spmv(dotmi_handle *h, const double *p, double *Hp);
int dotmi_probe_direction(dotmi_handle *h, const double *x, int32_t m, const double *S, const double *Y,
                          double *g, double *q, double *z, double *p, double *alpha0, double *E_trial);
int dotmi_get_features(dotmi_handle *h, double *A, double *vol, double *mass);
int32_t dotmi_part_size(const dotmi_handle *h, int32_t part);
int32_t dotmi_padded_size(const dotmi_handle *h);
int64_t dotmi_factor_storage_bytes(const dotmi_handle *h);
int32_t dotmi_factor_kind(const dotmi_handle *h);
int32_t dotmi_factor_groups(const dotmi_handle *h);
int32_t dotmi_backsolve_form(const dotmi_handle *h);
int dotmi_plan_backsolve_form(int32_t nV, int32_t nT, const int32_t *T, const double *Xrest, const int32_t *epart, int32_t nParts,
                              int32_t *form, int64_t *one_pass_bytes);
int dotmi_part_matrix(dotmi_handle *h, int32_t part, int inverse, double *M, int32_t *l2g);
int dotmi_plan_pd(int32_t nV, int32_t nT, const int32_t *T, const double *Xrest, int32_t *padded, int64_t *apply_bytes);
int dotmi_plan_ic(int32_t nV, int32_t nT, const int32_t *T, int32_t *sizes, int32_t *colour, int32_t *pos, int32_t *lptr,
                  int32_t *lidx, int32_t *lsrc, int32_t *dsrc, int32_t *pptr, int32_t *pa, int32_t *pb);
int dotmi_ic_info(dotmi_handle *h, int32_t *colours, double *shift, int32_t *attempts);
int dotmi_ic_factor(dotmi_handle *h, int32_t cap, double *blocks);
int dotmi_solve_hessian(dotmi_handle *h, const double *b, double *u, double rel_tol, int32_t max_iter, int32_t *iters,
                        double *rel_res);
int dotmi_set_pcg(dotmi_handle *h, double rel_tol, int32_t max_iter, int32_t check_every);
int dotmi_pcg_info(const dotmi_handle *h, int64_t *solves, int64_t *iters_total, int32_t *last_iters, double *last_rel_res);
int dotmi_set_pcg_coarse(dotmi_handle *h, int32_t mode);
int dotmi_pcg_coarse_info(const dotmi_handle *h, int32_t *dim, int32_t *dropped_subdomains, int32_t *active, int64_t *builds);
int dotmi_pcg_coarse_matrix(dotmi_handle *h, int32_t cap, double *A0);
int dotmi_pcg_apply_precond(dotmi_handle *h, const double *r, double *w);
int dotmi_set_dot_coarse(dotmi_handle *h, int32_t mode);
int dotmi_set_dot_coarse_mode(dotmi_handle *h, int32_t mode);
int32_t dotmi_dot_coarse_mode(const dotmi_handle *h);
int dotmi_dot_coarse_info(const dotmi_handle *h, int32_t *dim, int32_t *dropped_subdomains, int32_t *active, int64_t *builds,
                          double *last_build_ms);
int dotmi_plan_coarse(int32_t nV, int32_t nT, const int32_t *T, const int32_t *epart, int32_t nParts, int32_t *sizes, int32_t *pairS,
                      int32_t *pairT, int32_t *pairPtr, int32_t *pairBlk, int32_t *vsPtr, int32_t *vsIdx, int32_t *svPtr,
                      int32_t *svIdx);
int dotmi_plan_coarse_hz(int32_t nV, int32_t nT, const int32_t *T, const int32_t *epart, int32_t nParts, int32_t *sizes, int32_t *hzPtr,
                         int32_t *hzSub, int32_t *hzVert, int32_t *hzBlkPtr, int32_t *hzBlk, int32_t *hzTPtr, int32_t *hzTEnt);

int dotmi_bench_precond(dotmi_handle *h, int32_t reps, double *ms_per_launch, int64_t *bytes_per_launch);
int dotmi_bench_energy(dotmi_handle *h, int32_t reps, double *ms_per_launch, int64_t *bytes_per_launch);
enum dotmi_bench_kind {
    DOTMI_BENCH_ELEM_ENERGY_GRAD = 0,
    DOTMI_BENCH_ELEM_ENERGY = 1,
    DOTMI_BENCH_VERTEX_GATHER = 2,
    DOTMI_BENCH_SPMV_DOTS = 3,
    DOTMI_BENCH_BACKSOLVE = 4,
    DOTMI_BENCH_MERGE = 5,
    DOTMI_BENCH_BUILD_QPAD = 6,
    DOTMI_BENCH_BUILD_P = 7,
    DOTMI_BENCH_STEP_FORWARD = 8,
    DOTMI_BENCH_ELEM_HESSIAN = 9,
    DOTMI_BENCH_ASSEMBLE = 10,
    DOTMI_BENCH_SPMV_ZP = 11,
    DOTMI_BENCH_MERGE_EARLY = 12,
    DOTMI_BENCH_ELEM_STEP = 13,
    DOTMI_BENCH_GATHER_EARLY = 14,
    DOTMI_BENCH_DIRSTEP = 15,
    DOTMI_BENCH_ELEM_VERTEX = 16,
    DOTMI_BENCH_COUNT = 17
};
int dotmi_bench_kernel(dotmi_handle *h, int32_t kind, int32_t reps, double *ms_per_launch, int64_t *bytes_per_launch);

#ifdef __cplusplus
}
#endif
#endif
```

Measured before the change: 3.497 ms.

## Pair element-vertex slot operands and store history records per patch lane

Adds two layout bits to the operand-records form of the element-vertex kernel. Bit 2 interleaves each thread's two slots, so topology, rest-shape, material and volume data load as single wide vector reads, and the separate volE array is dropped in favour of deriving it from epos. Bit 4 stores the L-BFGS s/y history records and xt in patch-lane order, so each patch reads them contiguously instead of gathering by global vertex id. The xt copy is refreshed by a new small kernel, which is only launched in the bench path shown, and the stride change touches the device loop. Both bits are on by default, which adds template variants and a setup-time host permutation, and carries a risk that xtrec goes stale in the step path.

```diff
diff --git a/dot_amd/csrc/dotmi_api.hip b/dot_amd/csrc/dotmi_api.hip
--- a/dot_amd/csrc/dotmi_api.hip
+++ b/dot_amd/csrc/dotmi_api.hip
@@ -84,6 +84,7 @@
 }
 
 int dotmi_operand_records(const dotmi_handle *h) { return h && h->vpFits ? (h->VP.orec ? 1 : 0) : -1; }
+int dotmi_operand_record_bits(const dotmi_handle *h) { return h && h->vpFits ? (h->VP.orec ? h->VP.bits : 0) : -1; }
 
 int dotmi_loop_forms(const dotmi_handle *h)
 {
@@ -559,6 +560,7 @@
         for (int v = 0; v < nV; ++v) held += h->dup[v];
         bytes = 112 * nTo + 56 * nVo + 48 * (int64_t)nV + 80 * (int64_t)nV + (int64_t)(6 + 2 * L.m) * 8 * n + 24 * held;
         live = true;
+        launch_elem_vertex_xtrec(h->VP, h->xt, h->st);
         run = [&] {
             launch_elem_vertex(h->VP, h->mat, elem_vertex_args(h), h->st, h->ctl);
         };
diff --git a/dot_amd/csrc/dotmi_create.hip b/dot_amd/csrc/dotmi_create.hip
--- a/dot_amd/csrc/dotmi_create.hip
+++ b/dot_amd/csrc/dotmi_create.hip
@@ -81,8 +81,10 @@
     return cn * h->dtSq * h->dtSq;
 }
 
-int upload_vpatches(dotmi_handle *h, const HostVPatches &H, DevVPatches &D, dotmi_handle::SlotMap &SM)
-{
+int upload_vpatches(dotmi_handle *h, const HostVPatches &H, DevVPatches &D, dotmi_handle::SlotMap &SM, int bits)
+{
+    D.bits = bits;
+    const bool paired = (bits & 2) != 0;
     D.nPatches = H.nPatches;
     D.PE = H.PE;
     D.PV = H.PV;
@@ -104,6 +106,21 @@
         vol[s] = h->vol[e];
         volE[s] = H.eown[s] ? h->vol[e] : 0.0;
     }
+    std::vector<int> slotElem = H.elem;
+    if (paired) {
+        tl = vpatch_pair_slots(H, tl);
+        ep = vpatch_pair_slots(H, ep);
+        std::vector<double> plane(ns);
+        for (int k = 0; k < 9; ++k) {
+            std::copy(A.begin() + (size_t)k * ns, A.begin() + (size_t)(k + 1) * ns, plane.begin());
+            plane = vpatch_pair_slots(H, plane);
+            std::copy(plane.begin(), plane.end(), A.begin() + (size_t)k * ns);
+        }
+        mu = vpatch_pair_slots(H, mu);
+        lam = vpatch_pair_slots(H, lam);
+        vol = vpatch_pair_slots(H, vol);
+        slotElem = vpatch_pair_slots(H, slotElem);
+    }
     if (int rc = upload(h, &D.tl, tl)) return rc;
     if (int rc = upload(h, &D.epos, ep)) return rc;
     if (int rc = upload(h, &D.A, A)) return rc;
@@ -117,12 +134,14 @@
         if (int rc = upload(h, &D.mu, mu)) return rc;
         if (int rc = upload(h, &D.lam, lam)) return rc;
     }
-    if (int rc = upload(h, &SM.elem, H.elem)) return rc;
+    if (int rc = upload(h, &SM.elem, slotElem)) return rc;
     SM.nSlots = ns;
     SM.mu = D.mu;
     SM.lam = D.lam;
     if (int rc = upload(h, &D.vol, vol)) return rc;
-    if (int rc = upload(h, &D.volE, volE)) return rc;
+    D.volE = nullptr;
+    if (!paired)
+        if (int rc = upload(h, &D.volE, volE)) return rc;
     if (int rc = upload(h, &D.pv_gid, H.pv_gid)) return rc;
     if (int rc = upload(h, &D.pv_cnt, H.pv_cnt)) return rc;
     if (int rc = upload(h, &D.po_cnt, H.po_cnt)) return rc;
@@ -901,7 +920,7 @@
                          elem_vertex_dyn_lds(HV.PV, HV.RUN, HV.PO, true) + ELEM_VERTEX_STATIC_LDS <= 64 * 1024;
         const size_t shm = HV.nPatches > 0 ? elem_vertex_dyn_lds(HV.PV, HV.RUN, HV.PO, rec) + ELEM_VERTEX_STATIC_LDS : 0;
         if (HV.nPatches > 0 && HV.nPatches <= 512 && HV.nPatches <= ELEM_NB_MAX && shm <= 64 * 1024 && HV.PO + 1 <= 256) {
-            if (int rc = upload_vpatches(h, HV, h->VP, h->smVP)) return rc;
+            if (int rc = upload_vpatches(h, HV, h->VP, h->smVP, rec ? h->tune.operandRecords : 0)) return rc;
             if (rec) {
                 std::vector<int> vpp((size_t)h->nV + 1), vpo;
                 HIPCHECK(h, hipMemcpy(vpp.data(), h->P.vp_ptr, sizeof(int) * vpp.size(), hipMemcpyDeviceToHost));
@@ -930,9 +949,14 @@
         HIPCHECK(h, hipMemsetAsync(h->zstage, 0, sizeof(double) * nz, h->st));
     }
     if (h->vpFits && h->VP.orec) {
-        const size_t nrec = (size_t)2 * (HIST_MAX + 1) * h->n;
+        const size_t lanes = (size_t)h->VP.nPatches * 3 * h->VP.PO;
+        const size_t nrec = (h->VP.bits & 4) ? (size_t)2 * (HIST_MAX + 1) * lanes : (size_t)2 * (HIST_MAX + 1) * h->n;
         if (int rc = dalloc(h, &h->hrec, nrec)) return rc;
         HIPCHECK(h, hipMemsetAsync(h->hrec, 0, sizeof(double) * nrec, h->st));
+        if (h->VP.bits & 4) {
+            if (int rc = dalloc(h, &h->VP.xtrec, lanes)) return rc;
+            HIPCHECK(h, hipMemsetAsync(h->VP.xtrec, 0, sizeof(double) * lanes, h->st));
+        }
     }
     if (h->earlyBs) {
         if (int rc = dalloc(h, &h->u_old, (size_t)h->n)) return rc;
diff --git a/dot_amd/csrc/dotmi_devloop.hip b/dot_amd/csrc/dotmi_devloop.hip
--- a/dot_amd/csrc/dotmi_devloop.hip
+++ b/dot_amd/csrc/dotmi_devloop.hip
@@ -203,6 +203,7 @@
     }
     C.u_old = h->u_old;
     C.hrec = h->hrec;
+    C.recStride = (h->VP.bits & 4) ? 6 * h->VP.PO : 6;
     devloop_resolve(C);
     C.holdEnable = h->tune.earlyHold ? 1 : 0;
     memcpy(C.predHist, h->predState, sizeof(int) * 2);
diff --git a/dot_amd/csrc/dotmi_internal.hpp b/dot_amd/csrc/dotmi_internal.hpp
--- a/dot_amd/csrc/dotmi_internal.hpp
+++ b/dot_amd/csrc/dotmi_internal.hpp
@@ -74,6 +74,8 @@
     int *pv_gid = nullptr, *pv_cnt = nullptr, *po_cnt = nullptr;
     unsigned short *c_ptr = nullptr;
     const VpOwnRec *orec = nullptr;
+    int bits = 0;
+    double *xtrec = nullptr;
 };
 inline size_t elem_vertex_dyn_lds(int PV, int RUN, int PO, bool rec)
 {
@@ -256,6 +258,7 @@
     const double *Lrec[HIST_MAX];
     double *my_new;
     const double *Lmy[HIST_MAX], *Lhs[HIST_MAX];
+    int recStride;
 };
 template <class DL>
 __host__ __device__ inline void devloop_resolve(DL &C)
@@ -269,8 +272,9 @@
         C.Lhs[i] = i < m ? C.HS[C.order[i]] : nullptr;
     }
     C.my_new = m > 0 ? C.MY[C.order[m - 1]] : nullptr;
-    C.rec_new = C.hrec ? C.hrec + 6 * C.slot : nullptr;
-    for (int i = 0; i < HIST_MAX; ++i) C.Lrec[i] = (i < m && C.hrec) ? C.hrec + 6 * C.order[i] : nullptr;
+    const size_t rs = (size_t)C.recStride;
+    C.rec_new = C.hrec ? C.hrec + rs * C.slot : nullptr;
+    for (int i = 0; i < HIST_MAX; ++i) C.Lrec[i] = (i < m && C.hrec) ? C.hrec + rs * C.order[i] : nullptr;
 }
 struct VList {
     const int *v = nullptr;
@@ -341,6 +345,7 @@
 void launch_gemv(const DevParts &P, const double *q, hipStream_t st, const DevLoop *ctl = nullptr,
                  hipEvent_t ev0 = nullptr, hipEvent_t ev1 = nullptr, const CtlLaunch *ca = nullptr, int spec = 0);
 void launch_elem_vertex(const DevVPatches &VP, int mat, const ElemVertArgs &a, hipStream_t st, const DevLoop *ctl);
+void launch_elem_vertex_xtrec(const DevVPatches &VP, const double *xt, hipStream_t st);
 bool dirstep_fits(const DevPatches &PT);
 void launch_build_qpad(const DevParts &P, const double *g, const LbfgsArgs &L, const double *xi_host, hipStream_t st,
                        const DevLoop *ctl = nullptr, int spec = 0);
diff --git a/dot_amd/csrc/dotmi_plan.cpp b/dot_amd/csrc/dotmi_plan.cpp
--- a/dot_amd/csrc/dotmi_plan.cpp
+++ b/dot_amd/csrc/dotmi_plan.cpp
@@ -203,6 +203,34 @@
         rec_cnt[i] = R[i].cnt;
         for (int c = 0; c < 4; ++c) rec_off[4 * i + c] = R[i].off[c];
     }
+    return 0;
+}
+
+int dotmi_plan_vpatch_layout(int32_t nV, int32_t nT, const int32_t *T, const double *X, int32_t PE, int32_t max_own, int32_t nslots,
+                             const double *vals, int32_t *hdr, uint16_t *tl, uint16_t *epos, uint8_t *eown, uint16_t *tl2,
+                             uint16_t *epos2, double *vals2, uint8_t *counts, int32_t *pv_gid, int32_t *po_cnt, int64_t *hrec_idx)
+{
+    if (nV < 1 || nT < 1 || !T || !X || PE < 2 || PE % 2 || max_own < 1 || nslots < 1 || !hdr) return DOTMI_E_INVALID;
+    const HostVPatches H = build_vpatches(nV, nT, T, X, PE, max_own);
+    vpatch_header(H, hdr);
+    if (!tl || H.nPatches == 0) return 0;
+    if (!epos || !eown || !tl2 || !epos2 || !vals || !vals2 || !counts || !pv_gid || !po_cnt || !hrec_idx) return DOTMI_E_INVALID;
+    const size_t ns = (size_t)H.nPatches * H.PE;
+    std::copy(H.tl.begin(), H.tl.end(), tl);
+    std::copy(H.epos.begin(), H.epos.end(), epos);
+    std::copy(H.eown.begin(), H.eown.end(), eown);
+    const std::vector<uint16_t> t2 = vpatch_pair_slots(H, H.tl, 4), e2 = vpatch_pair_slots(H, H.epos, 4);
+    std::copy(t2.begin(), t2.end(), tl2);
+    std::copy(e2.begin(), e2.end(), epos2);
+    const std::vector<double> v2 = vpatch_pair_slots(H, std::vector<double>(vals, vals + ns));
+    std::copy(v2.begin(), v2.end(), vals2);
+    for (size_t s = 0; s < ns; ++s) counts[s] = vpatch_counts_energy(H, s) ? 1 : 0;
+    std::copy(H.pv_gid.begin(), H.pv_gid.end(), pv_gid);
+    std::copy(H.po_cnt.begin(), H.po_cnt.end(), po_cnt);
+    for (int p = 0; p < H.nPatches; ++p)
+        for (int l = 0; l < 3 * H.PO; ++l)
+            for (int sl = 0; sl < nslots; ++sl)
+                hrec_idx[((size_t)p * 3 * H.PO + l) * nslots + sl] = (int64_t)vpatch_hrec_index(H.PO, nslots, p, sl, l);
     return 0;
 }
 
diff --git a/dot_amd/csrc/k_elemvert.hip b/dot_amd/csrc/k_elemvert.hip
--- a/dot_amd/csrc/k_elemvert.hip
+++ b/dot_amd/csrc/k_elemvert.hip
@@ -18,9 +18,11 @@
 #define EVSTAMP(i) do { } while (0)
 #endif
 
-template <int MAT, bool PAIR, bool REC>
+template <int MAT, bool PAIR, int RECB>
 __global__ __launch_bounds__(256) void elem_vertex_kernel(DevVPatches VP, ElemVertArgs a, const DevLoop *__restrict__ ctl)
 {
+    constexpr bool REC = (RECB & 1) != 0, ELP = (RECB & 2) != 0, HPO = (RECB & 4) != 0;
+    static_assert(REC || RECB == 0, "bits 1 and 2 are layouts of the records' kernel");
     extern __shared__ double lds[];
     __shared__ double sm[4 * RED_K];
     __shared__ double sme[8];
@@ -104,6 +106,39 @@
     ushort4 tl[EV_EPT], ep[EV_EPT];
     double Ai[EV_EPT][9], mu_[EV_EPT], la_[EV_EPT], vo[EV_EPT], voE[EV_EPT];
     const size_t strideA = (size_t)VP.nPatches * PE;
+    if constexpr (ELP) {
+        static_assert(EV_EPT == 2, "a pair is the thread's two slots");
+        struct us4x2 {
+            ushort4 a, b;
+        };
+        const size_t s2 = (size_t)p * 256 + tid;
+        const us4x2 t2 = __builtin_bit_cast(us4x2, reinterpret_cast<const uint4 *>(VP.tl)[s2]);
+        const us4x2 e2 = __builtin_bit_cast(us4x2, reinterpret_cast<const uint4 *>(VP.epos)[s2]);
+        tl[0] = t2.a;
+        tl[1] = t2.b;
+        ep[0] = e2.a;
+        ep[1] = e2.b;
+#pragma unroll
+        for (int k = 0; k < 9; ++k) {
+            const ev_pair a2 = reinterpret_cast<const ev_pair *>(VP.A + (size_t)k * strideA)[s2];
+            Ai[0][k] = a2.x;
+            Ai[1][k] = a2.y;
+        }
+        ev_pair m2 = {VP.mu0, VP.mu0}, l2 = {VP.lam0, VP.lam0};
+        if (VP.mu) {
+            m2 = reinterpret_cast<const ev_pair *>(VP.mu)[s2];
+            l2 = reinterpret_cast<const ev_pair *>(VP.lam)[s2];
+        }
+        const ev_pair v2 = reinterpret_cast<const ev_pair *>(VP.vol)[s2];
+        mu_[0] = m2.x;
+        mu_[1] = m2.y;
+        la_[0] = l2.x;
+        la_[1] = l2.y;
+        vo[0] = v2.x;
+        vo[1] = v2.y;
+#pragma unroll
+        for (int u = 0; u < EV_EPT; ++u) voE[u] = ep[u].x != 0xFFFF ? vo[u] : 0.0;
+    } else {
 #pragma unroll
     for (int u = 0; u < EV_EPT; ++u) {
         const size_t s = (size_t)p * PE + u * 256 + tid;
@@ -116,6 +151,7 @@
         vo[u] = VP.vol[s];
         voE[u] = VP.volE[s];
     }
+    }
     double xv[3] = {0, 0, 0}, pv[3] = {0, 0, 0};
     if (gid >= 0) {
 #pragma unroll
@@ -130,24 +166,43 @@
     int cb = 0, ce = 0;
 #pragma unroll
     for (int i = 0; i < HIST_MAX; ++i) si[i] = yi[i] = 0.0;
+    if constexpr (HPO) {
+        if (loop && tid < 3 * VP.PO) {
+            const size_t lk = (size_t)p * (3 * VP.PO) + tid;
+            xt_own = VP.xtrec[lk];
+            const size_t rk = lk + (size_t)p * HIST_MAX * (3 * VP.PO);
+#pragma unroll
+            for (int i = 0; i < HIST_MAX; ++i) {
+                ev_pair sy = {0.0, 0.0};
+                if (i < hm) sy = hr[i][rk];
+                si[i] = sy.x;
+                yi[i] = sy.y;
+            }
+        }
+    }
     if constexpr (REC) {
         if (vlane) {
             fx = __double2hiint(rq0.y) != 0;
             ms = rq0.x;
             ce = __double2loint(rq0.y);
-            xt_own = a.xt[ok];
+            if (!HPO || !loop) xt_own = a.xt[ok];
             if (loop) {
                 gold = g_old[ok];
                 hpk = a.hp[ok];
-                const size_t rk = (size_t)(3 * (HIST_MAX + 1)) * ogid + od;
-#pragma unroll
-                for (int i = 0; i < HIST_MAX; ++i) {
-                    ev_pair sy = {0.0, 0.0};
-                    if (i < hm) sy = hr[i][rk];
-                    si[i] = sy.x;
-                    yi[i] = sy.y;
+                if constexpr (!HPO) {
+                    const size_t rk = (size_t)(3 * (HIST_MAX + 1)) * ogid + od;
+#pragma unroll
+                    for (int i = 0; i < HIST_MAX; ++i) {
+                        ev_pair sy = {0.0, 0.0};
+                        if (i < hm) sy = hr[i][rk];
+                        si[i] = sy.x;
+                        yi[i] = sy.y;
+                    }
                 }
             }
+        }
+        if constexpr (HPO) {
+            if (!loop && vlane) VP.xtrec[(size_t)p * (3 * VP.PO) + tid] = xt_own;
         }
     } else if (vlane) {
         fx = a.fixed[ogid] != 0;
@@ -352,7 +407,8 @@
             const double yn = g - gold;
             s_new[ok] = sn;
             y_new[ok] = yn;
-            if constexpr (REC) rec_new[(size_t)(3 * (HIST_MAX + 1)) * ogid + od] = ev_pair{sn, yn};
+            if constexpr (HPO) rec_new[(size_t)p * (HIST_MAX + 1) * (3 * VP.PO) + tid] = ev_pair{sn, yn};
+            else if constexpr (REC) rec_new[(size_t)(3 * (HIST_MAX + 1)) * ogid + od] = ev_pair{sn, yn};
             hs_new[ok] = alpha * hpk;
             st[1] = yn * sn;
             st[2] = sn * g;
@@ -386,15 +442,35 @@
     EVSTAMP(6);
 }
 
+__global__ __launch_bounds__(256) void elem_vertex_xtrec_kernel(DevVPatches VP, const double *__restrict__ xt)
+{
+    const int p = blockIdx.x, tid = threadIdx.x, ov = tid / 3, od = tid - 3 * ov;
+    if (tid >= 3 * VP.po_cnt[p]) return;
+    VP.xtrec[(size_t)p * (3 * VP.PO) + tid] = xt[3 * VP.pv_gid[(size_t)p * VP.PV + ov] + od];
+}
+
+void launch_elem_vertex_xtrec(const DevVPatches &VP, const double *xt, hipStream_t st)
+{
+    if (VP.xtrec) hipLaunchKernelGGL(elem_vertex_xtrec_kernel, dim3(VP.nPatches), dim3(256), 0, st, VP, xt);
+}
+
 void launch_elem_vertex(const DevVPatches &VP, int mat, const ElemVertArgs &a, hipStream_t st, const DevLoop *ctl)
 {
     const bool rec = VP.orec != nullptr;
     const size_t shm = elem_vertex_dyn_lds(VP.PV, VP.RUN, VP.PO, rec);
     const bool paired = ctl && a.alpha_min < 0.0;
-#define EV_LAUNCH(MATV, PAIRV, NWG)                                                                                          \
-    do {                                                                                                                     \
-        if (rec) hipLaunchKernelGGL((elem_vertex_kernel<MATV, PAIRV, true>), dim3(NWG), dim3(256), shm, st, VP, a, ctl);     \
-        else hipLaunchKernelGGL((elem_vertex_kernel<MATV, PAIRV, false>), dim3(NWG), dim3(256), shm, st, VP, a, ctl);        \
+    const int bits = rec ? VP.bits : 0;
+#define EV_LAUNCH_B(MATV, PAIRV, NWG, BITS) \
+    hipLaunchKernelGGL((elem_vertex_kernel<MATV, PAIRV, BITS>), dim3(NWG), dim3(256), shm, st, VP, a, ctl)
+#define EV_LAUNCH(MATV, PAIRV, NWG)                        \
+    do {                                                   \
+        switch (bits) {                                    \
+        case 7: EV_LAUNCH_B(MATV, PAIRV, NWG, 7); break;   \
+        case 5: EV_LAUNCH_B(MATV, PAIRV, NWG, 5); break;   \
+        case 3: EV_LAUNCH_B(MATV, PAIRV, NWG, 3); break;   \
+        case 1: EV_LAUNCH_B(MATV, PAIRV, NWG, 1); break;   \
+        default: EV_LAUNCH_B(MATV, PAIRV, NWG, 0); break;  \
+        }                                                  \
     } while (0)
 #define EV_LAUNCH_M(MATV)                                      \
     do {                                                       \
@@ -404,6 +480,7 @@
     DM_DISPATCH_MAT(mat, EV_LAUNCH_M)
 #undef EV_LAUNCH_M
 #undef EV_LAUNCH
-}
-
-}
+#undef EV_LAUNCH_B
+}
+
+}
diff --git a/dot_amd/csrc/tuning.hpp b/dot_amd/csrc/tuning.hpp
--- a/dot_amd/csrc/tuning.hpp
+++ b/dot_amd/csrc/tuning.hpp
@@ -37,7 +37,7 @@
     int specStep = 0;
     bool earlyHold = true;
     int earlyBs = 2;
-    int operandRecords = 1;
+    int operandRecords = 7;
     static int geti(const char *name, int dflt)
     {
         const char *ev = getenv(name);
@@ -81,7 +81,8 @@
         t.fuseDir = geti("DOTMI_FUSE_DIR", 1) != 0;
         t.wideForms = geti("DOTMI_WIDE_FORMS", -1);
         if (t.wideForms < -1) t.wideForms = -1;
-        t.operandRecords = geti("DOTMI_OPERAND_RECORDS", 1) & 1;
+        t.operandRecords = geti("DOTMI_OPERAND_RECORDS", 7) & 7;
+        if (!(t.operandRecords & 1)) t.operandRecords = 0;
         return t;
     }
 };
diff --git a/dot_amd/csrc/vpatches.hpp b/dot_amd/csrc/vpatches.hpp
--- a/dot_amd/csrc/vpatches.hpp
+++ b/dot_amd/csrc/vpatches.hpp
@@ -183,4 +183,26 @@
         if (own_gid[i] >= 0) R[i].fixed = fixed[own_gid[i]] != 0;
 }
 
-}
+inline size_t vpatch_pair_slot(int PE, size_t s)
+{
+    const size_t half = (size_t)PE / 2, p = s / PE, r = s % PE;
+    return p * PE + 2 * (r % half) + r / half;
+}
+template <class T>
+inline std::vector<T> vpatch_pair_slots(const HostVPatches &H, const std::vector<T> &flat, int width = 1)
+{
+    std::vector<T> out(flat.size());
+    const size_t ns = (size_t)H.nPatches * H.PE;
+    for (size_t s = 0; s < ns; ++s) {
+        const size_t j = vpatch_pair_slot(H.PE, s);
+        for (int k = 0; k < width; ++k) out[j * width + k] = flat[s * width + k];
+    }
+    return out;
+}
+inline bool vpatch_counts_energy(const HostVPatches &H, size_t s) { return H.epos[4 * s] != 0xFFFF; }
+inline size_t vpatch_hrec_index(int PO, int nslots, int patch, int slot, int lane)
+{
+    return ((size_t)patch * nslots + slot) * (size_t)(3 * PO) + lane;
+}
+
+}
diff --git a/dot_amd/lib.py b/dot_amd/lib.py
--- a/dot_amd/lib.py
+++ b/dot_amd/lib.py
@@ -71,7 +71,7 @@
     "dotmi_get_state", "dotmi_set_dirichlet", "dotmi_refix", "dotmi_step", "dotmi_last_iter_log",
     "dotmi_target_gres", "dotmi_eval_energy", "dotmi_eval_gradient", "dotmi_eval_elem_hessians",
     "dotmi_refactor", "dotmi_apply_precond", "dotmi_spmv", "dotmi_get_features", "dotmi_part_size", "dotmi_padded_size",
-    "dotmi_part_matrix", "dotmi_factor_storage_bytes", "dotmi_factor_kind", "dotmi_factor_groups", "dotmi_backsolve_form", "dotmi_plan_backsolve_form", "dotmi_probe_direction", "dotmi_bench_precond", "dotmi_bench_energy", "dotmi_bench_kernel", "dotmi_plan_shards", "dotmi_plan_layout", "dotmi_plan_tile_schedule", "dotmi_plan_tile_schedule_two_level", "dotmi_plan_tile_deps", "dotmi_plan_tile_groups", "dotmi_plan_grouped_tile_schedule", "dotmi_plan_tile_fill", "dotmi_plan_tile_fill_mesh", "dotmi_plan_backsolve_tiles", "dotmi_plan_backsolve_forms", "dotmi_plan_patches", "dotmi_plan_vpatches", "dotmi_plan_vpatch_records", "dotmi_operand_records", "dotmi_loop_forms", "dotmi_plan_loop_forms", "dotmi_plan_rank", "dotmi_partition",
+    "dotmi_part_matrix", "dotmi_factor_storage_bytes", "dotmi_factor_kind", "dotmi_factor_groups", "dotmi_backsolve_form", "dotmi_plan_backsolve_form", "dotmi_probe_direction", "dotmi_bench_precond", "dotmi_bench_energy", "dotmi_bench_kernel", "dotmi_plan_shards", "dotmi_plan_layout", "dotmi_plan_tile_schedule", "dotmi_plan_tile_schedule_two_level", "dotmi_plan_tile_deps", "dotmi_plan_tile_groups", "dotmi_plan_grouped_tile_schedule", "dotmi_plan_tile_fill", "dotmi_plan_tile_fill_mesh", "dotmi_plan_backsolve_tiles", "dotmi_plan_backsolve_forms", "dotmi_plan_patches", "dotmi_plan_vpatches", "dotmi_plan_vpatch_records", "dotmi_operand_records", "dotmi_operand_record_bits", "dotmi_plan_vpatch_layout", "dotmi_loop_forms", "dotmi_plan_loop_forms", "dotmi_plan_rank", "dotmi_partition",
     "dotmi_plan_pd",
     "dotmi_plan_ic", "dotmi_ic_info", "dotmi_ic_factor",
     "dotmi_set_rel_tol", "dotmi_set_time_step", "dotmi_set_lame",
@@ -151,6 +151,9 @@
     if hasattr(L, "dotmi_operand_records"):
         L.dotmi_operand_records.argtypes = [H]
         L.dotmi_operand_records.restype = C.c_int32
+    if hasattr(L, "dotmi_operand_record_bits"):
+        L.dotmi_operand_record_bits.argtypes = [H]
+        L.dotmi_operand_record_bits.restype = C.c_int32
     if hasattr(L, "dotmi_loop_forms"):
         L.dotmi_loop_forms.argtypes = [H]
         L.dotmi_loop_forms.restype = C.c_int32
diff --git a/include/dotmi.h b/include/dotmi.h
--- a/include/dotmi.h
+++ b/include/dotmi.h
@@ -131,11 +131,15 @@
 int dotmi_plan_vpatches(int32_t nV, int32_t nT, const int32_t *T, const double *X, int32_t PE, int32_t max_own, int32_t *hdr,
                         int32_t *owner, int32_t *elem, int32_t *eown, int32_t *runlen);
 int dotmi_operand_records(const dotmi_handle *h);
+int dotmi_operand_record_bits(const dotmi_handle *h);
 int dotmi_loop_forms(const dotmi_handle *h);
 int dotmi_plan_loop_forms(int64_t ndof_gather, int64_t ndof_merge, int64_t nrows_spmv, int32_t force, int32_t *out);
 int dotmi_plan_vpatch_records(int32_t nV, int32_t nT, const int32_t *T, const double *X, int32_t PE, int32_t max_own, const double *mass,
                               const uint8_t *fixed, const int32_t *vp_ptr, const int32_t *vp_off, const uint8_t *fixed2, int32_t *hdr,
                               int32_t *pv_gid, int32_t *po_cnt, double *rec_mass, int32_t *rec_fixed, int32_t *rec_cnt, int32_t *rec_off);
+int dotmi_plan_vpatch_layout(int32_t nV, int32_t nT, const int32_t *T, const double *X, int32_t PE, int32_t max_own, int32_t nslots,
+                             const double *vals, int32_t *hdr, uint16_t *tl, uint16_t *epos, uint8_t *eown, uint16_t *tl2,
+                             uint16_t *epos2, double *vals2, uint8_t *counts, int32_t *pv_gid, int32_t *po_cnt, int64_t *hrec_idx);
 int dotmi_plan_tile_schedule(int32_t nt, const uint8_t *live, const uint8_t *pattern, const int32_t *c0, int32_t eager_min,
                              int32_t eager_chunk, int64_t *tasks, int64_t *prods, int64_t *n_tasks, int64_t *n_prods,
                              int64_t *n_levels, int64_t *storage, int64_t *scratch_base, int64_t *row_off, int32_t *row_ld);
```

New measurement: 3.464 ms (median of 6 runs). No clear change (-0.9%).
